# IndaPlus22/bwidman-raytracer

Hardware: AMD Instinct MI355X
Metric: Msamples/sec (W*H*spp*bounces/t), 1920x1080 8spp 4-bounce, 07_specular_BRDF (higher is better)
Workload: dtype f32; 1 GPU; 07_specular_BRDF 1920x1080 8spp 4-bounce (BASELINE configs[2]); scene=07, width=1920, height=1080, spp=8, max_bounces=4, parallelism=pixel-rows/1

## Files before the change

bwidman-raytracer_amd/bwrt/abi.py:

```python
from __future__ import annotations

import ctypes as C
import os
import re

PKG_DIR = os.path.dirname(os.path.dirname(os.path.abspath(__file__)))
REPO_DIR = os.path.dirname(PKG_DIR)
LIB_PATH = os.path.join(PKG_DIR, "lib", "libbwrt.so")
HEADER_PATH = os.path.join(REPO_DIR, "include", "rt_abi.h")


class Vec3(C.Structure):
    _fields_ = [("x", C.c_float), ("y", C.c_float), ("z", C.c_float)]

    def tolist(self):
        return [self.x, self.y, self.z]


class Material(C.Structure):
    _fields_ = [("albedo", Vec3), ("emittance", C.c_float), ("roughness", C.c_float),
                ("refractive_index", C.c_float)]


class Sphere(C.Structure):
    _fields_ = [("position", Vec3), ("radius", C.c_float), ("mat", Material)]


class Plane(C.Structure):
    _fields_ = [("origin", Vec3), ("directions", Vec3 * 2), ("mat", Material)]


class Triangle(C.Structure):
    _fields_ = [("vertices", Vec3 * 3), ("mat", Material)]


class Quad(C.Structure):
    _fields_ = [("vertices", Vec3 * 4), ("mat", Material)]


class Camera(C.Structure):
    _fields_ = [("position", Vec3), ("angle", C.c_float * 2), ("fov", C.c_float)]


class SceneStruct(C.Structure):
    _fields_ = [("camera", Camera),
                ("spheres", C.POINTER(Sphere)), ("sphere_count", C.c_int),
                ("planes", C.POINTER(Plane)), ("plane_count", C.c_int),
                ("triangles", C.POINTER(Triangle)), ("triangle_count", C.c_int),
                ("quads", C.POINTER(Quad)), ("quad_count", C.c_int)]


class RenderParams(C.Structure):
    _fields_ = [("width", C.c_int), ("height", C.c_int), ("samples", C.c_int),
                ("max_bounces", C.c_int), ("first_frame", C.c_uint),
                ("row_offset", C.c_int), ("row_stride", C.c_int)]


class DenoiseParams(C.Structure):
    _fields_ = [("iterations", C.c_int), ("sigma_color", C.c_float), ("sigma_normal", C.c_float),
                ("sigma_plane", C.c_float)]


class DenoiseVarParams(C.Structure):
    _fields_ = [("iterations", C.c_int), ("sigma_lum", C.c_float), ("sigma_normal", C.c_float),
                ("sigma_plane", C.c_float), ("min_batches", C.c_int)]


class TemporalParams(C.Structure):
    _fields_ = [("max_history", C.c_float), ("normal_cos_min", C.c_float), ("plane_tol", C.c_float)]


RT_OK = 0
RT_ERR_INVALID_ARGUMENT = -1
RT_ERR_NO_DEVICE = -2
RT_ERR_NO_SCENE = -5
RT_ERR_UNSUPPORTED = -6
RT_DENOISE_MAX_ITERATIONS = 6
RT_MAX_BOUNCES = 32
RT_DEFAULT_MAX_BOUNCES = 5
RT_PRECISION_EXACT = 0
RT_PRECISION_REFERENCE_FAST = 1

_lib = None


def _proto(lib):
    P = C.POINTER
    vp = C.c_void_p
    sigs = {
        "rt_version": (C.c_char_p, []),
        "rt_material_default": (Material, []),
        "rt_device_count": (C.c_int, []),
        "rt_create": (C.c_int, [C.c_int, P(vp)]),
        "rt_destroy": (None, [vp]),
        "rt_cpu_threads": (C.c_int, []),
        "rt_create_cpu": (C.c_int, [C.c_int, P(vp)]),
        "rt_context_threads": (C.c_int, [vp]),
        "rt_render_cpu": (C.c_int, [vp, P(RenderParams), C.c_int, vp, vp]),
        "rt_set_scene": (C.c_int, [vp, P(SceneStruct)]),
        "rt_set_camera": (C.c_int, [vp, P(Camera)]),
        "rt_reset_accumulation": (C.c_int, [vp]),
        "rt_frame_counter": (C.c_uint, [vp]),
        "rt_set_max_bounces": (C.c_int, [vp, C.c_int]),
        "rt_set_background": (C.c_int, [vp, C.c_float, C.c_float, C.c_float]),
        "rt_set_precision": (C.c_int, [vp, C.c_int]),
        "rt_get_precision": (C.c_int, [vp]),
        "rt_set_samples_per_pixel": (C.c_int, [vp, C.c_int]),
        "rt_get_camera": (C.c_int, [vp, P(Camera)]),
        "rt_apply_controls": (C.c_int, [P(Camera), C.c_uint, C.c_float]),
        "rt_controls": (C.c_int, [vp, C.c_uint, C.c_float]),
        "rt_init_rand": (C.c_int, [vp, C.c_int, C.c_int, C.c_int, C.c_int]),
        "rt_render": (C.c_int, [vp, C.c_int, C.c_int, C.c_int, vp]),
        "rt_render_ex": (C.c_int, [vp, P(RenderParams), vp, vp]),
        "rt_render_device": (C.c_int, [vp, P(RenderParams), vp, vp]),
        "rt_synchronize": (C.c_int, [vp]),
        "rt_get_stream": (vp, [vp]),
        "rt_render_multi": (C.c_int, [P(vp), C.c_int, C.c_int, C.c_int, C.c_int, vp]),
        "rt_last_kernel_ms": (C.c_float, [vp]),
        "rt_set_kernel_timing": (C.c_int, [vp, C.c_int]),
        "rt_shard_rows": (C.c_int, [C.c_int, C.c_int, C.c_int]),
        "rt_deinterleave_rows_device": (C.c_int, [vp, vp, vp, C.c_int, C.c_int, C.c_int,
                                                  C.c_int, vp]),
        "rt_get_state": (C.c_int, [vp, vp, vp]),
        "rt_set_state": (C.c_int, [vp, vp, vp, C.c_uint]),
        "rt_render_aov": (C.c_int, [vp, P(RenderParams), vp, vp, vp, vp]),
        "rt_denoise_params_default": (DenoiseParams, []),
        "rt_denoise": (C.c_int, [vp, P(DenoiseParams), vp, vp]),
        "rt_denoise_device": (C.c_int, [vp, P(DenoiseParams), vp, vp]),
        "rt_last_denoise_ms": (C.c_float, [vp]),
        "rt_denoise_var_params_default": (DenoiseVarParams, []),
        "rt_denoise_var": (C.c_int, [vp, P(DenoiseVarParams), vp, vp, vp]),
        "rt_denoise_var_device": (C.c_int, [vp, P(DenoiseVarParams), vp, vp]),
        "rt_last_denoise_var_ms": (C.c_float, [vp]),
        "rt_temporal_params_default": (TemporalParams, []),
        "rt_temporal": (C.c_int, [vp, P(TemporalParams), P(DenoiseParams), vp, vp, vp]),
        "rt_temporal_device": (C.c_int, [vp, P(TemporalParams), P(DenoiseParams), vp, vp]),
        "rt_temporal_reset": (C.c_int, [vp]),
        "rt_last_temporal_ms": (C.c_float, [vp]),
        "rt_set_moments": (C.c_int, [vp, C.c_int]),
        "rt_get_moments": (C.c_int, [vp]),
        "rt_moments_batches": (C.c_int, [vp]),
        "rt_get_variance": (C.c_int, [vp, vp, vp]),
        "rt_error_string": (C.c_char_p, [C.c_int]),
        "rt_last_error": (C.c_char_p, [vp]),
        "rt_last_kernel_name": (C.c_char_p, [vp]),
    }
    for name, (res, args) in sigs.items():
        fn = getattr(lib, name)
        fn.restype = res
        fn.argtypes = args
    return lib


def declared_functions(header: str = HEADER_PATH):
    with open(header) as f:
        text = f.read()
    return sorted(set(re.findall(r"RT_API[^;(]*?\b(rt_\w+)\s*\(", text)))


def load(path: str | None = None):
    global _lib
    if _lib is not None and path is None:
        return _lib
    p = path or os.environ.get("BWRT_LIB", LIB_PATH)
    if not os.path.exists(p):
        raise RuntimeError(
            f"libbwrt.so not found at {p}: build it with `python -c 'import __graft_entry__ as g; g.build()'`"
            " (the HIP library is the product; nothing runs without it)")
    lib = _proto(C.CDLL(p))
    if path is None:
        _lib = lib
    return lib


KEYS = {"W": 1 << 0, "A": 1 << 1, "S": 1 << 2, "D": 1 << 3, "SPACE": 1 << 4, "LEFT_SHIFT": 1 << 5,
        "LEFT": 1 << 6, "RIGHT": 1 << 7, "UP": 1 << 8, "DOWN": 1 << 9, "ESCAPE": 1 << 10}
CONTROLS_MOVED = 1
CONTROLS_QUIT = 2


class RTError(RuntimeError):
    pass


def check(lib, status, ctx=None):
    if status != RT_OK:
        msg = lib.rt_error_string(status).decode()
        if ctx:
            last = lib.rt_last_error(ctx)
            if last:
                msg += ": " + last.decode()
        raise RTError(f"rt status {status}: {msg}")
    return status
```

bwidman-raytracer_amd/bwrt/renderer.py:

```python
from __future__ import annotations

import ctypes as C

import numpy as np

from . import abi


class Renderer:
    def __init__(self, device: int = 0, lib=None, _cpu_threads=None):
        self.lib = lib or abi.load()
        self.ctx = C.c_void_p()
        if _cpu_threads is None:
            abi.check(self.lib, self.lib.rt_create(device, C.byref(self.ctx)))
        else:
            abi.check(self.lib, self.lib.rt_create_cpu(_cpu_threads, C.byref(self.ctx)))
        self.device = device if _cpu_threads is None else -1
        self.scene = None

    @classmethod
    def cpu(cls, threads: int = 0, lib=None) -> "Renderer":
        return cls(-1, lib=lib, _cpu_threads=threads)

    @property
    def is_cpu(self) -> bool:
        return self.device < 0

    @property
    def threads(self) -> int:
        return self.lib.rt_context_threads(self.ctx)

    def close(self):
        if self.ctx:
            self.lib.rt_destroy(self.ctx)
            self.ctx = C.c_void_p()

    def __enter__(self):
        return self

    def __exit__(self, *exc):
        self.close()

    def __del__(self):
        try:
            self.close()
        except Exception:
            pass

    def _check(self, status):
        return abi.check(self.lib, status, self.ctx)

    def set_scene(self, scene):
        self.scene = scene
        self._check(self.lib.rt_set_scene(self.ctx, C.byref(scene.struct)))

    def set_camera(self, camera):
        self._check(self.lib.rt_set_camera(self.ctx, C.byref(camera)))

    def reset_accumulation(self):
        self._check(self.lib.rt_reset_accumulation(self.ctx))

    @property
    def frame_counter(self) -> int:
        return self.lib.rt_frame_counter(self.ctx)

    def set_max_bounces(self, mb: int):
        self._check(self.lib.rt_set_max_bounces(self.ctx, mb))

    def set_background(self, r: float, g: float, b: float):
        self._check(self.lib.rt_set_background(self.ctx, r, g, b))

    _PRECISIONS = {"exact": abi.RT_PRECISION_EXACT, "fast": abi.RT_PRECISION_REFERENCE_FAST}

    def set_precision(self, mode: str):
        if mode not in self._PRECISIONS:
            raise ValueError(f"precision {mode!r}: expected 'exact' or 'fast'")
        self._check(self.lib.rt_set_precision(self.ctx, self._PRECISIONS[mode]))

    @property
    def precision(self) -> str:
        return "fast" if self.lib.rt_get_precision(self.ctx) == abi.RT_PRECISION_REFERENCE_FAST else "exact"

    def set_samples_per_pixel(self, n: int):
        self._check(self.lib.rt_set_samples_per_pixel(self.ctx, n))

    def get_camera(self):
        from .abi import Camera
        cam = Camera()
        self._check(self.lib.rt_get_camera(self.ctx, C.byref(cam)))
        return cam

    def controls(self, keys, delta_time: float) -> int:
        from .abi import KEYS
        if not isinstance(keys, int):
            keys = sum(KEYS[k] for k in keys)
        flags = self.lib.rt_controls(self.ctx, keys, delta_time)
        if flags < 0:
            self._check(flags)
        return flags

    def init_rand(self, width, height, row_offset=0, row_stride=1):
        self._check(self.lib.rt_init_rand(self.ctx, width, height, row_offset, row_stride))

    @staticmethod
    def params(width, height, samples, max_bounces, first_frame=0, row_offset=0, row_stride=1):
        return abi.RenderParams(width, height, samples, max_bounces, first_frame, row_offset,
                                row_stride)

    def render_simple(self, width: int, height: int, samples: int) -> np.ndarray:
        out = np.empty((height, width, 4), dtype=np.uint8)
        self._check(self.lib.rt_render(self.ctx, width, height, samples, out.ctypes.data))
        return out

    def render(self, width, height, samples, max_bounces=abi.RT_DEFAULT_MAX_BOUNCES, first_frame=0,
               row_offset=0, row_stride=1, want_accum=False):
        rows = self.lib.rt_shard_rows(height, row_offset, row_stride)
        out = np.empty((rows, width, 4), dtype=np.uint8)
        acc = np.empty((rows, width, 3), dtype=np.float32) if want_accum else None
        p = self.params(width, height, samples, max_bounces, first_frame, row_offset, row_stride)
        self._check(self.lib.rt_render_ex(self.ctx, C.byref(p), out.ctypes.data,
                                          acc.ctypes.data if acc is not None else None))
        return (out, acc) if want_accum else out

    def render_cpu(self, width, height, samples, max_bounces=abi.RT_DEFAULT_MAX_BOUNCES, first_frame=0,
                   row_offset=0, row_stride=1, threads=0, want_accum=False):
        rows = self.lib.rt_shard_rows(height, row_offset, row_stride)
        out = np.empty((rows, width, 4), dtype=np.uint8)
        acc = np.empty((rows, width, 3), dtype=np.float32) if want_accum else None
        p = self.params(width, height, samples, max_bounces, first_frame, row_offset, row_stride)
        self._check(self.lib.rt_render_cpu(self.ctx, C.byref(p), threads, out.ctypes.data,
                                           acc.ctypes.data if acc is not None else None))
        return (out, acc) if want_accum else out

    def render_device(self, params: abi.RenderParams, rgba_ptr: int, stream_ptr: int | None = None):
        self._check(self.lib.rt_render_device(self.ctx, C.byref(params), rgba_ptr, stream_ptr))

    def synchronize(self):
        self._check(self.lib.rt_synchronize(self.ctx))

    def stream_handle(self) -> int:
        return self.lib.rt_get_stream(self.ctx) or 0

    def last_kernel_ms(self) -> float:
        return self.lib.rt_last_kernel_ms(self.ctx)

    def last_kernel_name(self) -> str:
        return self.lib.rt_last_kernel_name(self.ctx).decode()

    def set_kernel_timing(self, enable: bool):
        self._check(self.lib.rt_set_kernel_timing(self.ctx, int(bool(enable))))

    def deinterleave_device(self, gathered_ptr, image_ptr, width, height, shards, rows_per_shard,
                            stream_ptr=None):
        self._check(self.lib.rt_deinterleave_rows_device(self.ctx, gathered_ptr, image_ptr, width,
                                                         height, shards, rows_per_shard,
                                                         stream_ptr))

    def render_aov(self, width, height, row_offset=0, row_stride=1):
        rows = self.lib.rt_shard_rows(height, row_offset, row_stride)
        out = {"albedo": np.empty((rows, width, 3), np.float32), "normal": np.empty((rows, width, 3), np.float32),
               "depth": np.empty((rows, width), np.float32), "prim": np.empty((rows, width), np.int32)}
        p = self.params(width, height, 1, 0, 0, row_offset, row_stride)
        self._check(self.lib.rt_render_aov(self.ctx, C.byref(p), out["albedo"].ctypes.data,
                                           out["normal"].ctypes.data, out["depth"].ctypes.data,
                                           out["prim"].ctypes.data))
        return out

    def denoise_params(self, iterations=None, sigma_color=None, sigma_normal=None, sigma_plane=None):
        d = self.lib.rt_denoise_params_default()
        for name, v in (("iterations", iterations), ("sigma_color", sigma_color),
                        ("sigma_normal", sigma_normal), ("sigma_plane", sigma_plane)):
            if v is not None:
                setattr(d, name, v)
        return d

    def denoise(self, width, height, iterations=None, sigma_color=None, sigma_normal=None, sigma_plane=None,
                want_color=False):
        d = self.denoise_params(iterations, sigma_color, sigma_normal, sigma_plane)
        out = np.empty((height, width, 4), np.uint8)
        col = np.empty((height, width, 3), np.float32) if want_color else None
        self._check(self.lib.rt_denoise(self.ctx, C.byref(d), out.ctypes.data,
                                        col.ctypes.data if col is not None else None))
        return (out, col) if want_color else out

    def denoise_device(self, rgba_ptr: int, stream_ptr: int | None = None, iterations=None, sigma_color=None,
                       sigma_normal=None, sigma_plane=None):
        d = self.denoise_params(iterations, sigma_color, sigma_normal, sigma_plane)
        self._check(self.lib.rt_denoise_device(self.ctx, C.byref(d), rgba_ptr, stream_ptr))

    def last_denoise_ms(self) -> float:
        return self.lib.rt_last_denoise_ms(self.ctx)

    def denoise_var_params(self, iterations=None, sigma_lum=None, sigma_normal=None, sigma_plane=None,
                           min_batches=None):
        d = self.lib.rt_denoise_var_params_default()
        for name, v in (("iterations", iterations), ("sigma_lum", sigma_lum), ("sigma_normal", sigma_normal),
                        ("sigma_plane", sigma_plane), ("min_batches", min_batches)):
            if v is not None:
                setattr(d, name, v)
        return d

    def denoise_var(self, width, height, want_color=False, want_var=False, **params):
        d = self.denoise_var_params(**params)
        out = np.empty((height, width, 4), np.uint8)
        col = np.empty((height, width, 3), np.float32) if want_color else None
        var = np.empty((height, width), np.float32) if want_var else None
        self._check(self.lib.rt_denoise_var(self.ctx, C.byref(d), out.ctypes.data,
                                            col.ctypes.data if col is not None else None,
                                            var.ctypes.data if var is not None else None))
        res = (out,) + ((col,) if want_color else ()) + ((var,) if want_var else ())
        return res if len(res) > 1 else out

    def denoise_var_device(self, rgba_ptr: int, stream_ptr: int | None = None, **params):
        d = self.denoise_var_params(**params)
        self._check(self.lib.rt_denoise_var_device(self.ctx, C.byref(d), rgba_ptr, stream_ptr))

    def last_denoise_var_ms(self) -> float:
        return self.lib.rt_last_denoise_var_ms(self.ctx)

    def temporal_params(self, max_history=None, normal_cos_min=None, plane_tol=None):
        t = self.lib.rt_temporal_params_default()
        for name, v in (("max_history", max_history), ("normal_cos_min", normal_cos_min), ("plane_tol", plane_tol)):
            if v is not None:
                setattr(t, name, v)
        return t

    def _dn(self, denoise):
        return None if denoise is None else C.byref(self.denoise_params(**denoise))

    def temporal(self, width, height, max_history=None, normal_cos_min=None, plane_tol=None, denoise=None,
                 want_color=False, want_length=False):
        t = self.temporal_params(max_history, normal_cos_min, plane_tol)
        out = np.empty((height, width, 4), np.uint8)
        col = np.empty((height, width, 3), np.float32) if want_color else None
        ln = np.empty((height, width), np.float32) if want_length else None
        self._check(self.lib.rt_temporal(self.ctx, C.byref(t), self._dn(denoise), out.ctypes.data,
                                         col.ctypes.data if col is not None else None,
                                         ln.ctypes.data if ln is not None else None))
        res = (out,) + ((col,) if want_color else ()) + ((ln,) if want_length else ())
        return res if len(res) > 1 else out

    def temporal_device(self, rgba_ptr: int, stream_ptr: int | None = None, max_history=None, normal_cos_min=None,
                        plane_tol=None, denoise=None):
        t = self.temporal_params(max_history, normal_cos_min, plane_tol)
        self._check(self.lib.rt_temporal_device(self.ctx, C.byref(t), self._dn(denoise), rgba_ptr, stream_ptr))

    def temporal_reset(self):
        self._check(self.lib.rt_temporal_reset(self.ctx))

    def last_temporal_ms(self) -> float:
        return self.lib.rt_last_temporal_ms(self.ctx)

    def set_moments(self, enable: bool = True):
        self._check(self.lib.rt_set_moments(self.ctx, int(bool(enable))))

    @property
    def moments(self) -> bool:
        return bool(self.lib.rt_get_moments(self.ctx))

    @property
    def moments_batches(self) -> int:
        return self.lib.rt_moments_batches(self.ctx)

    def variance(self, rows, width, want_lum=False):
        var = np.empty((rows, width), np.float32)
        lum = np.empty((rows, width), np.float32) if want_lum else None
        self._check(self.lib.rt_get_variance(self.ctx, var.ctypes.data, lum.ctypes.data if want_lum else None))
        return (var, lum) if want_lum else var

    def get_state(self, rows, width):
        rng = np.empty((6, rows, width), dtype=np.uint32)
        acc = np.empty((rows, width, 3), dtype=np.float32)
        self._check(self.lib.rt_get_state(self.ctx, rng.ctypes.data, acc.ctypes.data))
        return rng, acc

    def set_state(self, rng, acc, frame_counter):
        rng = np.ascontiguousarray(rng, dtype=np.uint32)
        acc = np.ascontiguousarray(acc, dtype=np.float32)
        self._check(self.lib.rt_set_state(self.ctx, rng.ctypes.data, acc.ctypes.data,
                                          frame_counter))


def shard_rows(height: int, row_offset: int, row_stride: int) -> int:
    return len(range(row_offset, height, row_stride)) if row_stride > 0 else 0


def render_multi(renderers, width: int, height: int, samples: int) -> np.ndarray:
    lib = renderers[0].lib
    arr = (C.c_void_p * len(renderers))(*[r.ctx.value for r in renderers])
    out = np.empty((height, width, 4), np.uint8)
    rc = lib.rt_render_multi(arr, len(renderers), width, height, samples, out.ctypes.data)
    if rc != abi.RT_OK:
        renderers[0]._check(rc)
    return out
```

bwidman-raytracer_amd/csrc/rt_context.cpp:

```cpp
#include <sched.h>

#include <algorithm>
#include <cmath>
#include <cstdarg>
#include <cstddef>
#include <thread>

#include "rt_context.h"

static_assert(sizeof(rt_vec3) == 12, "vec3d layout (Math.cuh:35-39)");
static_assert(sizeof(rt_material) == 24, "material layout (WorldTypes.cuh:15-20)");
static_assert(sizeof(rt_sphere) == 40 && offsetof(rt_sphere, mat) == 16, "sphere layout");
static_assert(sizeof(rt_plane) == 60 && offsetof(rt_plane, mat) == 36, "plane layout");
static_assert(sizeof(rt_triangle) == 60 && offsetof(rt_triangle, mat) == 36, "triangle layout");
static_assert(sizeof(rt_quad) == 72 && offsetof(rt_quad, mat) == 48, "quad layout");
static_assert(sizeof(rt_camera) == 24, "camera layout (WorldTypes.cuh:9-13)");
static_assert(sizeof(rt_scene) == 88 && offsetof(rt_scene, spheres) == 24 &&
                  offsetof(rt_scene, sphere_count) == 32 && offsetof(rt_scene, planes) == 40 &&
                  offsetof(rt_scene, triangles) == 56 && offsetof(rt_scene, quads) == 72 &&
                  offsetof(rt_scene, quad_count) == 80,
              "scene layout (WorldTypes.cuh:44-53)");

const char* tuning_env(const char* name) {
    const char* t = std::getenv("BWRT_TUNING");
    return t && std::strcmp(t, "1") == 0 ? std::getenv(name) : nullptr;
}

int fail(rt_context* c, int code, const char* fmt, ...) {
    if (c) {
        char buf[512];
        va_list ap;
        va_start(ap, fmt);
        vsnprintf(buf, sizeof buf, fmt, ap);
        va_end(ap);
        c->err = buf;
    }
    return code;
}

int hip_fail(rt_context* c, hipError_t e, const char* what) {
    return fail(c, e == hipErrorOutOfMemory ? RT_ERR_OUT_OF_MEMORY : RT_ERR_HIP, "%s: %s", what,
                hipGetErrorString(e));
}

int quiesce(rt_context* c) {
    if (c->cpu) return RT_OK;
    HIP_TRY(c, c->render.flush());
    for (Pass* p : {&c->denoise, &c->temporal, &c->denoise_var, &c->render}) HIP_TRY(c, p->sync());
    return RT_OK;
}

int order_after_all(rt_context* c, hipStream_t s) {
    for (Pass* p : {&c->render, &c->denoise, &c->temporal, &c->denoise_var}) HIP_TRY(c, p->wait_on(s));
    return RT_OK;
}

int ensure_buf(rt_context* c, Buf& b, size_t bytes, const char* host_oom, size_t n) {
    if (b.bytes >= bytes && b.p) return RT_OK;
    if (b.p && !c->cpu) {
        int rc = quiesce(c);
        if (rc) return rc;
        HIP_TRY(c, hipStreamSynchronize(c->stream));
    }
    b.release();
    if (bytes == 0) return RT_OK;
    if (c->cpu) {
        if (!(b.p = std::calloc(bytes, 1))) return fail(c, RT_ERR_OUT_OF_MEMORY, host_oom, n);
        b.host = true;
    } else {
        HIP_TRY(c, hipMalloc(&b.p, bytes));
    }
    b.bytes = bytes;
    return RT_OK;
}

int shard_rows(int height, int row_offset, int row_stride) {
    if (height <= 0 || row_offset < 0 || row_stride <= 0 || row_offset >= height) return 0;
    return (height - row_offset + row_stride - 1) / row_stride;
}

int shard_check(rt_context* c, int width, int height, int row_offset, int row_stride) {
    if (width <= 0 || height <= 0 || row_offset < 0 || row_stride < 0 || row_offset >= height)
        return fail(c, RT_ERR_INVALID_ARGUMENT, "bad shard %dx%d offset %d stride %d", width, height,
                    row_offset, row_stride);
    if ((long long)width * height > (1ll << 31))
        return fail(c, RT_ERR_UNSUPPORTED, "image larger than 2^31 pixels");
    return RT_OK;
}

extern "C" {

const char* rt_version(void) { return "0.3.0"; }

rt_material rt_material_default(void) {
    rt_material m;
    m.albedo = {0.0f, 0.0f, 0.0f};
    m.emittance = 0.0f;
    m.roughness = 1.0f;
    m.refractive_index = 1.05f;
    return m;
}

int rt_device_count(void) {
    int n = 0;
    if (hipGetDeviceCount(&n) != hipSuccess) return 0;
    return n;
}

int rt_create(int device, rt_context** out) {
    if (!out) return RT_ERR_INVALID_ARGUMENT;
    *out = nullptr;
    int n = 0;
    if (hipGetDeviceCount(&n) != hipSuccess || n <= 0) return RT_ERR_NO_DEVICE;
    if (device < 0 || device >= n) return RT_ERR_INVALID_ARGUMENT;
    rt_context* c = new rt_context();
    c->device = device;
    int prio_lo = 0, prio_hi = 0;
    const char* sp = tuning_env("BWRT_STREAM_PRIO");
    const bool high = !(sp && std::atoi(sp) == 0) && hipSetDevice(device) == hipSuccess &&
                      hipDeviceGetStreamPriorityRange(&prio_lo, &prio_hi) == hipSuccess;
    if (hipSetDevice(device) != hipSuccess ||
        (high ? hipStreamCreateWithPriority(&c->stream, hipStreamNonBlocking, prio_hi)
              : hipStreamCreateWithFlags(&c->stream, hipStreamNonBlocking)) != hipSuccess ||
        c->render.create(true) != hipSuccess || c->aux.create(false) != hipSuccess ||
        c->denoise.create(true) != hipSuccess) {
        rt_destroy(c);
        return RT_ERR_HIP;
    }
    c->render.home = c->stream;
    hipDeviceProp_t prop;
    if (hipGetDeviceProperties(&prop, device) == hipSuccess && prop.multiProcessorCount > 0)
        c->num_cus = prop.multiProcessorCount;
    if (const char* gm = tuning_env("BWRT_GRID_MULT")) c->grid_mult = std::atoi(gm);
    if (const char* db = tuning_env("BWRT_DEINT_BLOCKS")) c->deint_blocks = std::max(std::atoi(db), 0);
    if (const char* kk = tuning_env("BWRT_KERNEL")) c->simple = std::strcmp(kk, "simple") == 0;
    if (const char* bk = tuning_env("BWRT_BLOCK")) c->block = std::atoi(bk);
    if (const char* tw = tuning_env("BWRT_TILE")) {
        const int t = std::atoi(tw);
        if (t >= 0 && t <= 64 && (t & (t - 1)) == 0) c->tile_w = t;
    }
    if (const char* g = tuning_env("BWRT_TILE_SQ")) c->tile_sq = std::atoi(g) != 0;
    if (const char* g = tuning_env("BWRT_GREC")) c->grec = std::atoi(g) ? 1 : 0;
    if (const char* g = tuning_env("BWRT_LEAF_BATCH")) c->leaf_batch = std::min(std::max(std::atoi(g), 1), 64);
    if (const char* g = tuning_env("BWRT_REFILL")) c->refill = std::min(std::max(std::atoi(g), 1), 64);
    if (const char* g = tuning_env("BWRT_SPREAD")) c->spread = std::atoi(g) ? 1 : 0;
    if (const char* g = tuning_env("BWRT_ORDER")) c->order_feedback = std::atoi(g) != 0;
    if (const char* g = tuning_env("BWRT_ORDER_PERIOD")) c->order_period = std::max(std::atoi(g), 1);
    if (const char* g = tuning_env("BWRT_DENOISE_KERNEL"))
        c->dn_kernel = std::strcmp(g, "tiled") == 0 ? 1 : std::strcmp(g, "direct") == 0 ? 0 : -1;
    if (const char* g = tuning_env("BWRT_PRECISION"))
        c->precision = std::strcmp(g, "fast") == 0 ? RT_PRECISION_REFERENCE_FAST : RT_PRECISION_EXACT;
    *out = c;
    return RT_OK;
}

int rt_create_cpu(int threads, rt_context** out) {
    if (!out) return RT_ERR_INVALID_ARGUMENT;
    *out = nullptr;
    if (threads < 0) return RT_ERR_INVALID_ARGUMENT;
    if (!rt_cpu_supported()) return RT_ERR_UNSUPPORTED;
    rt_context* c = new rt_context();
    c->cpu = true;
    c->render.host = c->denoise.host = c->temporal.host = c->denoise_var.host = true;
    c->device = -1;
    c->threads = threads > 0 ? threads : rt_cpu_threads();
    *out = c;
    return RT_OK;
}

int rt_cpu_threads(void) {
    int n = 0;
    cpu_set_t set;
    if (sched_getaffinity(0, sizeof set, &set) == 0) n = CPU_COUNT(&set);
    if (n <= 0) n = (int)std::thread::hardware_concurrency();
    if (n <= 0) n = 1;
    if (FILE* f = std::fopen("/sys/fs/cgroup/cpu.max", "r")) {
        char quota[32] = {0};
        long period = 0;
        if (std::fscanf(f, "%31s %ld", quota, &period) == 2 && std::strcmp(quota, "max") != 0 && period > 0) {
            const long q = std::atol(quota);
            const int share = (int)((q + period - 1) / period);
            if (share > 0 && share < n) n = share;
        }
        std::fclose(f);
    }
    return n;
}

void rt_destroy(rt_context* c) {
    if (!c) return;
    if (!c->cpu) {
        (void)hipSetDevice(c->device);
        if (c->stream) (void)hipStreamSynchronize(c->stream);
        c->render.pending = false;
        for (Pass* p : {&c->render, &c->aux, &c->denoise, &c->temporal, &c->denoise_var}) {
            (void)p->sync();
            p->destroy();
        }
        if (c->host_rgba) (void)hipHostFree(c->host_rgba);
        if (c->stream) (void)hipStreamDestroy(c->stream);
    }
    delete c;
}

int rt_set_scene(rt_context* c, const rt_scene* s) {
    const HostFpEnv fp;
    if (!c || !s) return fail(c, RT_ERR_INVALID_ARGUMENT, "null argument");
    if (s->sphere_count < 0 || s->plane_count < 0 || s->triangle_count < 0 || s->quad_count < 0)
        return fail(c, RT_ERR_INVALID_ARGUMENT, "negative primitive count");
    if ((s->sphere_count && !s->spheres) || (s->plane_count && !s->planes) ||
        (s->triangle_count && !s->triangles) || (s->quad_count && !s->quads))
        return fail(c, RT_ERR_INVALID_ARGUMENT, "null primitive array with non-zero count");
    if (!c->cpu) HIP_TRY(c, hipSetDevice(c->device));
    rt_scene_options opt;
    for (const char* name : rt_scene_option_names)
        if (const char* v = tuning_env(name)) rt_scene_option_set(opt, name, v);
    rt_compiled_scene cs;
    std::string err;
    if (const int rc = rt_compile_scene(*s, opt, cs, err)) return fail(c, rc, "%s", err.c_str());
    const size_t bytes = cs.data.size() * sizeof(float);
    int rc = quiesce(c);
    if (!rc) rc = ensure_buf(c, c->scene_buf, bytes, "host scene of %zu bytes", bytes);
    if (rc) {
        if (!c->scene_buf.p) c->has_scene = false;
        return rc;
    }
    if (c->cpu) {
        std::memcpy(c->scene_buf.p, cs.data.data(), bytes);
    } else {
        HIP_TRY(c, hipMemcpyAsync(c->scene_buf.p, cs.data.data(), bytes, hipMemcpyHostToDevice, c->stream));
        HIP_TRY(c, hipStreamSynchronize(c->stream));
    }
    std::vector<float>().swap(cs.data);
    c->scene = std::move(cs);
    c->camera = s->camera;
    c->has_scene = true;
    c->frame = 1;
    c->order_stale = true;
    c->new_view();
    c->tp_has_hist = c->tp_has_pending = false;
    return RT_OK;
}

int rt_set_camera(rt_context* c, const rt_camera* cam) {
    if (!c || !cam) return fail(c, RT_ERR_INVALID_ARGUMENT, "null argument");
    c->camera = *cam;
    c->frame = 1;
    c->order_stale = true;
    c->new_view();
    return RT_OK;
}

int rt_set_background(rt_context* c, float r, float g, float b) {
    if (!c) return RT_ERR_INVALID_ARGUMENT;
    c->background[0] = r;
    c->background[1] = g;
    c->background[2] = b;
    return RT_OK;
}

int rt_set_precision(rt_context* c, int precision) {
    if (!c) return RT_ERR_INVALID_ARGUMENT;
    if (precision != RT_PRECISION_EXACT && precision != RT_PRECISION_REFERENCE_FAST)
        return fail(c, RT_ERR_INVALID_ARGUMENT, "rt_set_precision: unknown precision %d", precision);
    if (c->cpu && precision != RT_PRECISION_EXACT)
        return fail(c, RT_ERR_UNSUPPORTED,
                    "rt_set_precision: RT_PRECISION_REFERENCE_FAST is not supported on a CPU context "
                    "(the CPU fallback is bit-identical to the exact kernels)");
    c->precision = precision;
    return RT_OK;
}

int rt_get_precision(const rt_context* c) { return c ? c->precision : RT_PRECISION_EXACT; }

int rt_get_camera(const rt_context* c, rt_camera* cam) {
    if (!c || !cam) return RT_ERR_INVALID_ARGUMENT;
    *cam = c->camera;
    return RT_OK;
}

int rt_apply_controls(rt_camera* cam, unsigned keys, float dt) {
    if (!cam) return RT_ERR_INVALID_ARGUMENT;
    const HostFpEnv fp;
    struct V3 {
        float x, y, z;
    };
    const float move = 5 * dt;
    const float rot = 2 * dt;
    const float cy = cosf(cam->angle[0]), sy = sinf(cam->angle[0]);
    const float cx = cosf(cam->angle[1]), sx = sinf(cam->angle[1]);
    const float L[3][3] = {{cy, 0, sy}, {0, 1, 0}, {-sy, 0, cy}};
    const float U[3][3] = {{1, 0, 0}, {0, cx, -sx}, {0, sx, cx}};
    float M[3][3];
    for (int i = 0; i < 3; i++)
        for (int j = 0; j < 3; j++) M[i][j] = L[i][0] * U[0][j] + L[i][1] * U[1][j] + L[i][2] * U[2][j];
    auto mul = [&](float x, float y, float z) {
        return V3{M[0][0] * x + M[0][1] * y + M[0][2] * z, M[1][0] * x + M[1][1] * y + M[1][2] * z,
                  M[2][0] * x + M[2][1] * y + M[2][2] * z};
    };
    const V3 front = mul(0, 0, -1), right = mul(1, 0, 0);
    rt_vec3& p = cam->position;
    int flags = 0;
    auto add = [&](float k, V3 v, float sign) {
        const V3 kv{k * v.x, k * v.y, k * v.z};
        if (sign > 0) {
            p.x = p.x + kv.x;
            p.y = p.y + kv.y;
            p.z = p.z + kv.z;
        } else {
            p.x = p.x - kv.x;
            p.y = p.y - kv.y;
            p.z = p.z - kv.z;
        }
        flags |= RT_CONTROLS_MOVED;
    };
    if (keys & RT_KEY_W) add(move, front, +1);
    if (keys & RT_KEY_A) add(move, right, -1);
    if (keys & RT_KEY_S) add(move, front, -1);
    if (keys & RT_KEY_D) add(move, right, +1);
    if (keys & RT_KEY_SPACE) {
        p.y += move;
        flags |= RT_CONTROLS_MOVED;
    }
    if (keys & RT_KEY_LEFT_SHIFT) {
        p.y -= move;
        flags |= RT_CONTROLS_MOVED;
    }
    if (keys & RT_KEY_LEFT) {
        cam->angle[0] += rot;
        flags |= RT_CONTROLS_MOVED;
    }
    if (keys & RT_KEY_RIGHT) {
        cam->angle[0] -= rot;
        flags |= RT_CONTROLS_MOVED;
    }
    if (keys & RT_KEY_UP) {
        cam->angle[1] += rot;
        flags |= RT_CONTROLS_MOVED;
    }
    if (keys & RT_KEY_DOWN) {
        cam->angle[1] -= rot;
        flags |= RT_CONTROLS_MOVED;
    }
    if (keys & RT_KEY_ESCAPE) flags |= RT_CONTROLS_QUIT;
    return flags;
}

int rt_controls(rt_context* c, unsigned keys, float dt) {
    if (!c) return RT_ERR_INVALID_ARGUMENT;
    const int flags = rt_apply_controls(&c->camera, keys, dt);
    if (flags > 0 && (flags & RT_CONTROLS_MOVED)) {
        c->frame = 1;
        c->order_stale = true;
        c->new_view();
    }
    return flags;
}

int rt_reset_accumulation(rt_context* c) {
    if (!c) return RT_ERR_INVALID_ARGUMENT;
    c->frame = 1;
    return RT_OK;
}

unsigned rt_frame_counter(const rt_context* c) { return c ? c->frame : 0u; }

int rt_set_max_bounces(rt_context* c, int mb) {
    if (!c) return RT_ERR_INVALID_ARGUMENT;
    if (mb < 0) return fail(c, RT_ERR_INVALID_ARGUMENT, "max_bounces < 0");
    if (mb > RT_MAX_BOUNCES) return fail(c, RT_ERR_UNSUPPORTED, "max_bounces > %d", RT_MAX_BOUNCES);
    c->max_bounces = mb;
    return RT_OK;
}

int rt_set_samples_per_pixel(rt_context* c, int n) {
    if (!c) return RT_ERR_INVALID_ARGUMENT;
    if (n < 1) return fail(c, RT_ERR_INVALID_ARGUMENT, "samples per pixel < 1");
    if (n > RT_MAX_SAMPLES_PER_PIXEL)
        return fail(c, RT_ERR_UNSUPPORTED, "samples per pixel > %d", RT_MAX_SAMPLES_PER_PIXEL);
    c->spp_inner = n;
    return RT_OK;
}

int rt_set_kernel_timing(rt_context* c, int enable) {
    if (!c) return RT_ERR_INVALID_ARGUMENT;
    c->ktiming = enable != 0;
    if (!c->ktiming) c->render.timed = false;
    return RT_OK;
}

int rt_shard_rows(int height, int row_offset, int row_stride) {
    return shard_rows(height, row_offset, row_stride == 0 ? 1 : row_stride);
}

int rt_init_rand(rt_context* c, int width, int height, int row_offset, int row_stride) {
    if (!c) return RT_ERR_INVALID_ARGUMENT;
    if (row_stride == 0) row_stride = 1;
    if (const int rc = shard_check(c, width, height, row_offset, row_stride)) return rc;
    const int rows = shard_rows(height, row_offset, row_stride);
    const size_t npix = (size_t)rows * width;
    c->new_view();
    c->mom_drop();
    if (width != c->tp_w || height != c->tp_h) c->tp_has_hist = c->tp_has_pending = false;
    if (!c->cpu) HIP_TRY(c, hipSetDevice(c->device));
    int rc = quiesce(c);
    const char* oom = "host state for %zu pixels";
    if (!rc) rc = ensure_buf(c, c->rng, npix * 6 * sizeof(unsigned), oom, npix);
    if (!rc) rc = ensure_buf(c, c->accum, npix * 3 * sizeof(float), oom, npix);
    if (!rc && c->cpu) rc = ensure_buf(c, c->rgba, npix * 4, oom, npix);
    if (rc) return rc;
    if (c->cpu) {
        std::memset(c->rng.p, 0, npix * 6 * sizeof(unsigned));
        std::memset(c->accum.p, 0, npix * 3 * sizeof(float));
        std::memset(c->rgba.p, 0, npix * 4);
        rt_cpu_init_rand(c->rng.as<unsigned>(), width, rows, row_offset, row_stride);
    } else {
        HIP_TRY(c, hipMemsetAsync(c->accum.p, 0, npix * 3 * sizeof(float), c->stream));
        HIP_TRY(c, rt_launch_init_rand(c->rng.as<unsigned>(), width, rows, row_offset, row_stride, c->stream));
        HIP_TRY(c, hipStreamSynchronize(c->stream));
    }
    c->width = width;
    c->height = height;
    c->row_offset = row_offset;
    c->row_stride = row_stride;
    c->rows = rows;
    c->frame = 1;
    c->order_stale = true;
    return RT_OK;
}

int rt_synchronize(rt_context* c) {
    if (!c) return RT_ERR_INVALID_ARGUMENT;
    if (c->cpu) return RT_OK;
    HIP_TRY(c, hipSetDevice(c->device));
    HIP_TRY(c, c->render.flush());
    HIP_TRY(c, hipStreamSynchronize(c->stream));
    for (Pass* p : {&c->render, &c->aux, &c->denoise, &c->temporal, &c->denoise_var}) HIP_TRY(c, p->sync());
    return RT_OK;
}

void* rt_get_stream(rt_context* c) { return c && !c->cpu ? (void*)c->stream : nullptr; }

float rt_last_kernel_ms(rt_context* c) { return c ? c->render.elapsed_ms() : -1.0f; }

int rt_get_state(rt_context* c, uint32_t* rng, float* accum) {
    if (!c) return RT_ERR_INVALID_ARGUMENT;
    const size_t npix = (size_t)c->rows * c->width;
    if (!c->rng.p) return fail(c, RT_ERR_INVALID_ARGUMENT, "no shard state (render or rt_init_rand first)");
    if (c->cpu) {
        if (rng) std::memcpy(rng, c->rng.p, npix * 6 * sizeof(unsigned));
        if (accum) planes_to_rgb(c->accum.as<float>(), npix, accum);
        return RT_OK;
    }
    HIP_TRY(c, hipSetDevice(c->device));
    HIP_TRY(c, hipStreamSynchronize(c->stream));
    const int qrc = quiesce(c);
    if (qrc) return qrc;
    if (rng) HIP_TRY(c, hipMemcpy(rng, c->rng.p, npix * 6 * sizeof(unsigned), hipMemcpyDeviceToHost));
    if (accum) {
        std::vector<float> planes(npix * 3);
        HIP_TRY(c, hipMemcpy(planes.data(), c->accum.p, npix * 3 * sizeof(float), hipMemcpyDeviceToHost));
        planes_to_rgb(planes.data(), npix, accum);
    }
    return RT_OK;
}

int rt_set_state(rt_context* c, const uint32_t* rng, const float* accum, unsigned frame_counter) {
    if (!c) return RT_ERR_INVALID_ARGUMENT;
    if (!c->rng.p) return fail(c, RT_ERR_INVALID_ARGUMENT, "no shard state (rt_init_rand first)");
    if (frame_counter == 0) return fail(c, RT_ERR_INVALID_ARGUMENT, "frame_counter must be >= 1");
    const size_t npix = (size_t)c->rows * c->width;
    if (c->cpu) {
        if (rng) std::memcpy(c->rng.p, rng, npix * 6 * sizeof(unsigned));
        if (accum) rgb_to_planes(accum, npix, c->accum.as<float>());
        c->frame = frame_counter;
        c->mom_drop();
        return RT_OK;
    }
    HIP_TRY(c, hipSetDevice(c->device));
    const int rc = quiesce(c);
    if (rc) return rc;
    std::vector<float> planes;
    if (rng)
        HIP_TRY(c, hipMemcpyAsync(c->rng.p, rng, npix * 6 * sizeof(unsigned), hipMemcpyHostToDevice, c->stream));
    if (accum) {
        planes.resize(npix * 3);
        rgb_to_planes(accum, npix, planes.data());
        HIP_TRY(c, hipMemcpyAsync(c->accum.p, planes.data(), npix * 3 * sizeof(float), hipMemcpyHostToDevice,
                                  c->stream));
    }
    HIP_TRY(c, hipStreamSynchronize(c->stream));
    c->frame = frame_counter;
    c->mom_drop();
    return RT_OK;
}

const char* rt_error_string(int status) {
    switch (status) {
        case RT_OK: return "ok";
        case RT_ERR_INVALID_ARGUMENT: return "invalid argument";
        case RT_ERR_NO_DEVICE: return "no HIP device";
        case RT_ERR_HIP: return "HIP runtime error";
        case RT_ERR_OUT_OF_MEMORY: return "out of device memory";
        case RT_ERR_NO_SCENE: return "no scene";
        case RT_ERR_UNSUPPORTED: return "unsupported";
        default: return "unknown status";
    }
}

const char* rt_last_error(const rt_context* c) { return c ? c->err.c_str() : ""; }

const char* rt_last_kernel_name(const rt_context* c) { return c ? c->kernel_name.c_str() : ""; }

int rt_context_threads(const rt_context* c) { return c && c->cpu ? c->threads : 0; }

}
```

bwidman-raytracer_amd/csrc/rt_context.h:

```cpp
#pragma once

#include <hip/hip_runtime.h>

#include <chrono>
#include <cstdint>
#include <cstdio>
#include <cstdlib>
#include <cstring>
#include <string>
#include <vector>
#include <xmmintrin.h>

#include "../../include/rt_abi.h"
#include "rt_layout.h"
#include "rt_scene.h"

size_t rt_render_rec_floats(const rt_kparams& K);
bool rt_render_wants_global_records(const rt_kparams& K, int num_cus);
hipError_t rt_launch_render(const rt_kparams& K, int num_cus, int grid_mult, bool simple, int block_req,
                            hipStream_t stream, int pair_req);
hipError_t rt_launch_init_rand(unsigned* rng, int width, int rows, int row_offset, int row_stride,
                               hipStream_t stream);
namespace rt_fast {
bool rt_render_wants_global_records(const rt_kparams& K, int num_cus);
hipError_t rt_launch_render(const rt_kparams& K, int num_cus, int grid_mult, bool simple, int block_req,
                            hipStream_t stream, int pair_req);
}
extern thread_local long rt_order_groups_last;
extern thread_local char rt_launched_kernel[96];
hipError_t rt_launch_deinterleave(const unsigned* gathered, unsigned* image, int width, int height,
                                  int shards, int rows_per_shard, int max_blocks, hipStream_t stream);
int rt_cpu_render(const rt_kparams& K, int threads);
void rt_cpu_init_rand(unsigned* rng, int width, int rows, int row_offset, int row_stride);
bool rt_cpu_supported();
void rt_cpu_aov(const rt_kparams& K, int threads, float4* ga, float4* gb, float4* alb);
void rt_cpu_denoise_level(const rt_dn_level& L, int threads);
void rt_cpu_temporal(const rt_tp_args& T, int threads);
void rt_cpu_moments(const rt_mom_args& A, int threads);
void rt_cpu_denoise_var(const rt_dv_args& A, int stage, int threads);
hipError_t rt_launch_aov(const rt_kparams& K, float4* ga, float4* gb, float4* alb, hipStream_t stream);
hipError_t rt_launch_aov_bvh(const rt_kparams& K, float4* ga, float4* gb, float4* alb, hipStream_t stream);
hipError_t rt_launch_denoise_level(const rt_dn_level& L, bool tiled, hipStream_t stream);
hipError_t rt_launch_temporal(const rt_tp_args& T, hipStream_t stream);
hipError_t rt_launch_moments(const rt_mom_args& A, hipStream_t stream);
hipError_t rt_launch_denoise_var(const rt_dv_args& A, int stage, bool tiled, hipStream_t stream);

struct Buf {
    void* p = nullptr;
    size_t bytes = 0;
    bool host = false;
    Buf() = default;
    Buf(const Buf&) = delete;
    Buf& operator=(const Buf&) = delete;
    ~Buf() { release(); }
    void release() {
        if (p) host ? std::free(p) : (void)hipFree(p);
        p = nullptr;
        bytes = 0;
    }
    template <class T>
    T* as() const {
        return static_cast<T*>(p);
    }
};

struct Pass {
    hipEvent_t ev0 = nullptr, ev1 = nullptr;
    hipStream_t stream = nullptr;
    hipStream_t home = nullptr;
    bool host = false;
    bool recorded = false;
    bool pending = false;
    bool timed = false;
    bool marked = false;
    float cpu_ms = -1.0f;
    std::chrono::steady_clock::time_point t0;

    hipError_t create(bool timing) {
        hipError_t e = hipSuccess;
        if (timing && !ev0) e = hipEventCreate(&ev0);
        if (e == hipSuccess && !ev1) e = timing ? hipEventCreate(&ev1) : hipEventCreateWithFlags(&ev1, hipEventDisableTiming);
        return e;
    }
    hipError_t begin(hipStream_t s, bool with_marker) {
        marked = with_marker;
        if (host) t0 = std::chrono::steady_clock::now();
        return !host && with_marker ? hipEventRecord(ev0, s) : hipSuccess;
    }
    hipError_t end(hipStream_t s) {
        stream = s;
        if (host) {
            cpu_ms = std::chrono::duration<float, std::milli>(std::chrono::steady_clock::now() - t0).count();
        } else if (home && s == home && !marked) {
            pending = true;
        } else {
            pending = false;
            const hipError_t e = hipEventRecord(ev1, s);
            if (e != hipSuccess) return e;
            recorded = true;
        }
        timed = marked;
        return hipSuccess;
    }
    hipError_t flush() {
        if (!pending) return hipSuccess;
        pending = false;
        const hipError_t e = hipEventRecord(ev1, home);
        if (e == hipSuccess) recorded = true;
        return e;
    }
    hipError_t wait_on(hipStream_t s) {
        if (!(recorded || pending) || stream == s) return hipSuccess;
        const hipError_t e = flush();
        return e != hipSuccess ? e : hipStreamWaitEvent(s, ev1, 0);
    }
    hipError_t sync() { return recorded ? hipEventSynchronize(ev1) : hipSuccess; }
    float elapsed_ms() {
        if (host) return cpu_ms;
        float ms = -1.0f;
        if (!timed || hipEventSynchronize(ev1) != hipSuccess || hipEventElapsedTime(&ms, ev0, ev1) != hipSuccess)
            return -1.0f;
        return ms;
    }
    void destroy() {
        if (ev0) (void)hipEventDestroy(ev0);
        if (ev1) (void)hipEventDestroy(ev1);
        ev0 = ev1 = nullptr;
    }
};

struct rt_context {
    int device = 0;
    int num_cus = 256;
    bool simple = false;
    int grid_mult = 0;
    hipStream_t stream = nullptr;
    Pass render, aux, denoise, temporal, denoise_var;
    bool cpu = false;
    int threads = 1;
    bool ktiming = true;
    std::string err;

    bool has_scene = false;
    rt_camera camera{};
    float background[3] = {0.0f, 0.0f, 0.0f};
    rt_compiled_scene scene;
    Buf scene_buf;

    int width = 0, height = 0, row_offset = 0, row_stride = 1, rows = 0;
    Buf rng, accum, rgba;
    Buf rec;
    Buf gcost, gorder;
    long order_n = 0;
    int order_period = 16;
    bool order_stale = true;
    unsigned long long launches = 0;
    bool order_feedback = true;
    int grec = -1;
    void* host_rgba = nullptr;
    size_t host_rgba_bytes = 0;
    int block = 0;
    int tile_w = -1;
    int tile_sq = 0;
    int leaf_batch = -1;
    int refill = -1;
    int spread = -1;
    int deint_blocks = 0;
    std::string kernel_name;
    int precision = RT_PRECISION_EXACT;
    unsigned frame = 1;
    int max_bounces = RT_DEFAULT_MAX_BOUNCES;
    int spp_inner = 1;

    Buf guide_a, guide_b, dn_col[2], dn_rgba;
    Buf dn_rs;
    Buf aov_a, aov_b, aov_alb;
    bool guides_valid = false;
    int dn_kernel = -1;

    struct TpSet {
        Buf col, ga, gb;
        float cam_pos[3] = {}, rot[9] = {}, screen_z = 0.0f;
    };
    unsigned long long view = 1;
    TpSet tp[2];
    int tp_hist = 0;
    bool tp_has_hist = false, tp_has_pending = false;
    unsigned long long tp_pending_view = 0;
    int tp_w = 0, tp_h = 0;

    bool mom_on = false, mom_live = false;
    unsigned mom_batches = 0, mom_next = 0;
    Buf mom_prev, mom_m;
    void mom_drop() {
        mom_live = false;
        mom_batches = 0;
    }

    void new_view() {
        guides_valid = false;
        view++;
    }
};

struct HostFpEnv {
    unsigned saved;
    HostFpEnv() : saved(_mm_getcsr()) {
        _mm_setcsr((saved & ~(_MM_ROUND_MASK | _MM_FLUSH_ZERO_MASK | 0x0040u)) | _MM_ROUND_NEAREST);
    }
    ~HostFpEnv() { _mm_setcsr(saved); }
};

const char* tuning_env(const char* name);

int fail(rt_context* c, int code, const char* fmt, ...);
int hip_fail(rt_context* c, hipError_t e, const char* what);

#define HIP_TRY(ctx, expr)                                  \
    do {                                                    \
        hipError_t _e = (expr);                             \
        if (_e != hipSuccess) return hip_fail(ctx, _e, #expr); \
    } while (0)

int quiesce(rt_context* c);
int order_after_all(rt_context* c, hipStream_t s);
int ensure_buf(rt_context* c, Buf& b, size_t bytes, const char* host_oom = "host buffer (%zu)", size_t n = 0);
int shard_rows(int height, int row_offset, int row_stride);
int shard_check(rt_context* c, int width, int height, int row_offset, int row_stride);
void fill_view(rt_context* c, int width, int height, int row_offset, int stride, int rows, rt_kparams& K);

inline void planes_to_rgb(const float* planes, size_t npix, float* out) {
    for (size_t i = 0; i < npix; i++)
        for (int ch = 0; ch < 3; ch++) out[3 * i + ch] = planes[ch * npix + i];
}
inline void rgb_to_planes(const float* rgb, size_t npix, float* planes) {
    for (size_t i = 0; i < npix; i++)
        for (int ch = 0; ch < 3; ch++) planes[ch * npix + i] = rgb[3 * i + ch];
}
inline void xyz_of(const float4* v, size_t npix, float* out) {
    for (size_t i = 0; i < npix; i++) {
        out[3 * i + 0] = v[i].x;
        out[3 * i + 1] = v[i].y;
        out[3 * i + 2] = v[i].z;
    }
}
inline void w_of(const float4* v, size_t npix, void* out) {
    for (size_t i = 0; i < npix; i++) std::memcpy(static_cast<char*>(out) + 4 * i, &v[i].w, 4);
}
```

bwidman-raytracer_amd/csrc/rt_kernels.hip:

```cpp
#include <hip/hip_runtime.h>

#include <cstdio>
#include <type_traits>

#include "rt_diag.h"
#include "rt_layout.h"
#include "rt_path.h"

#ifdef RT_FAST
#define RT_MODE_BEGIN namespace rt_fast {
#define RT_MODE_END }
#define RT_MODE_TAG ",fast"
#else
#define RT_MODE_BEGIN
#define RT_MODE_END
#define RT_MODE_TAG ""
#endif
#if !defined(RT_TU_BVH) && !defined(RT_FAST)
#define RT_TU_SHARED
#endif

namespace {
__device__ __forceinline__ void closest_hit_bvh(const rt_kparams& K, f3 o, f3 d, float& best_t, int& best_id) {
    if (!bvh_safe(K, o, d)) {
        closest_hit_brute(K, o, d, best_t, best_id);
        return;
    }
    const float a = dot(d, d);
    const float a4 = 4.0f * a;
    const float a2 = 2.0f * a;
    best_t = INFINITY;
    best_id = -1;
    int best_key = -1;
    planes_first(K, o, d, best_t, best_id, best_key);
    const SlabRay sr = slab_ray(o, d);
    const float* nodes = K.bvh_nodes + (size_t)ray_octant(K, d) * K.bvh_order_stride;
    int node = 0;
    while (true) {
        int leaf = -1;
        while (true) {
            bool stalled = false;
            if (node >= 0) {
                RT_BRANCH_COUNT(K, 5);
                const float4 lo = *reinterpret_cast<const float4*>(nodes + 8 * node);
                const float4 hi = *reinterpret_cast<const float4*>(nodes + 8 * node + 4);
                const bool hit = slab_enter(lo.x, lo.y, lo.z, hi.x, hi.y, hi.z, sr, best_t);
                const int miss = __float_as_int(lo.w);
                const int lf = __float_as_int(hi.w);
                if (!hit) {
                    node = miss;
                } else if (lf < 0) {
                    node = node + 1;
                } else if (leaf < 0) {
                    leaf = lf;
                    node = miss;
                } else {
                    stalled = true;
                }
            }
            if (__all(leaf >= 0 || node < 0 || stalled)) break;
        }
        if (!__any(leaf >= 0)) break;
        if (leaf >= 0) {
            const int first = leaf & 0xffffff, count = leaf >> 24;
            for (int k = 0; k < count; k++) {
                RT_BRANCH_COUNT(K, 6);
                leaf_test(K, K.bvh_leafrec + (size_t)RT_LEAF_FLOATS * (first + k), o, d, a2, a4, best_t, best_id,
                          best_key);
            }
        }
    }
}

template <bool BVH, bool QUADS = true>
__device__ __forceinline__ void closest_hit(const rt_kparams& K, f3 o, f3 d, float& best_t, int& best_id) {
    if (BVH)
        closest_hit_bvh(K, o, d, best_t, best_id);
    else
        closest_hit_brute<QUADS>(K, o, d, best_t, best_id);
}

#ifndef RT_NT_PIXEL
#define RT_NT_PIXEL 3
#endif
#ifndef RT_NT_GREC
#define RT_NT_GREC 0
#endif
template <typename T>
__device__ __forceinline__ T px_ld(const T* a) {
    if (RT_NT_PIXEL & 1) return __builtin_nontemporal_load(a);
    return *a;
}
template <typename T>
__device__ __forceinline__ void px_st(T* a, T v) {
    if (RT_NT_PIXEL & 2) __builtin_nontemporal_store(v, a);
    else *a = v;
}
struct PixelState {
    long w;
    long p;
    bool valid;
    Xorwow rs;
    float ax, ay, az;
    f3 d0;
    int passes_left;
    unsigned frame;
};

__device__ __forceinline__ void load_pixel(const rt_kparams& K, long npix, long p, PixelState& s) {
    s.p = p;
    s.valid = p < npix;
    s.passes_left = 0;
    s.frame = K.first_frame;
    if (!s.valid) return;
    const int j = (int)(p / K.width);
    const int x = (int)(p - (long)j * K.width);
    const int y = K.row_offset + j * K.row_stride;
    s.rs.d = px_ld(&K.rng[0 * npix + p]);
    s.rs.v0 = px_ld(&K.rng[1 * npix + p]);
    s.rs.v1 = px_ld(&K.rng[2 * npix + p]);
    s.rs.v2 = px_ld(&K.rng[3 * npix + p]);
    s.rs.v3 = px_ld(&K.rng[4 * npix + p]);
    s.rs.v4 = px_ld(&K.rng[5 * npix + p]);
    s.ax = s.ay = s.az = 0.0f;
    if (K.first_frame != 1u) {
        s.ax = px_ld(&K.accum[0 * npix + p]);
        s.ay = px_ld(&K.accum[1 * npix + p]);
        s.az = px_ld(&K.accum[2 * npix + p]);
    }
    s.d0 = primary_dir(K, x, y);
    s.passes_left = K.samples;
}

__host__ __device__ inline long launch_items(const rt_kparams& K) {
    if (K.tile_w <= 0) return (long)K.rows * K.width;
    const int tw = K.tile_w, th = 64 / K.tile_w;
    long tiles_x = (K.width + tw - 1) / tw, tiles_y = (K.rows + th - 1) / th;
    if (K.tile_sq) {
        tiles_x += tiles_x & 1;
        tiles_y += tiles_y & 1;
    }
    return tiles_x * tiles_y * 64;
}

__device__ __forceinline__ long items_of(const rt_kparams& K, long npix) {
    return K.tile_w <= 0 ? npix : launch_items(K);
}

__device__ __forceinline__ long item_to_pixel(const rt_kparams& K, long npix, long w) {
    if (K.tile_w <= 0) return w < npix ? w : npix;
    const int tw = K.tile_w, th = 64 / K.tile_w;
    const long tiles_x = (K.width + tw - 1) / tw;
    const long wave = w >> 6;
    const int l = (int)(w & 63);
    long tx, ty;
    if (K.tile_sq) {
        const long sx = (tiles_x + 1) >> 1, sw = wave >> 2;
        tx = (sw % sx) * 2 + (wave & 1);
        ty = (sw / sx) * 2 + ((wave >> 1) & 1);
    } else {
        tx = wave % tiles_x;
        ty = wave / tiles_x;
    }
    const long x = tx * tw + (l % tw);
    const long j = ty * th + (l / tw);
    if (x >= K.width || j >= K.rows) return npix;
    return j * K.width + x;
}

__device__ __forceinline__ void load_item(const rt_kparams& K, long npix, long nitems, long w, PixelState& s) {
    load_pixel(K, npix, w < nitems ? item_to_pixel(K, npix, w) : npix, s);
    s.w = w;
}

__device__ __forceinline__ void store_pixel(const rt_kparams& K, long npix, const PixelState& s) {
    const long p = s.p;
    px_st(&K.rng[0 * npix + p], s.rs.d);
    px_st(&K.rng[1 * npix + p], s.rs.v0);
    px_st(&K.rng[2 * npix + p], s.rs.v1);
    px_st(&K.rng[3 * npix + p], s.rs.v2);
    px_st(&K.rng[4 * npix + p], s.rs.v3);
    px_st(&K.rng[5 * npix + p], s.rs.v4);
    px_st(&K.accum[0 * npix + p], s.ax);
    px_st(&K.accum[1 * npix + p], s.ay);
    px_st(&K.accum[2 * npix + p], s.az);
#if RT_NT_PIXEL & 2
    if (K.rgba) px_st(&K.rgba[p], tone_map(s.ax, s.ay, s.az, s.frame - 1u));
#else
    if (K.rgba) K.rgba[p] = tone_map(s.ax, s.ay, s.az, s.frame - 1u);
#endif
}

typedef __attribute__((address_space(3))) float lds_float;

__device__ __forceinline__ int lanes_below(unsigned long long mask) {
    return (int)__builtin_amdgcn_mbcnt_hi((unsigned)(mask >> 32),
                                          __builtin_amdgcn_mbcnt_lo((unsigned)mask, 0u));
}

__device__ __forceinline__ int prim_key(const rt_kparams& K, int id) {
    const int e_pln = K.n_sph, e_tri = e_pln + K.n_pln, e_quad = e_tri + K.n_tri;
    return id < 0 ? -1
                  : id < e_pln ? RT_KEY(0, id)
                               : id < e_tri ? RT_KEY(1, id - e_pln)
                                            : id < e_quad ? RT_KEY(2, id - e_tri) : RT_KEY(3, id - e_quad);
}

}

#ifndef RT_WAVES_PER_EU
#define RT_WAVES_PER_EU 1
#endif
#ifndef RT_GREC_WAVES
#define RT_GREC_WAVES 7
#endif
#ifndef RT_GREC_LDS_LEVELS
#define RT_GREC_LDS_LEVELS 2
#endif
#ifndef RT_SPEC_PRIO
#define RT_SPEC_PRIO 3
#endif
#ifndef RT_PAIR_WAVES
#define RT_PAIR_WAVES 7
#endif

RT_MODE_BEGIN
template <int BLOCK, bool HIT_LDS, bool BVH>
__global__ void __launch_bounds__(BLOCK) __attribute__((amdgpu_waves_per_eu(RT_WAVES_PER_EU)))
rt_render_kernel(rt_kparams K) {
    extern __shared__ float smem[];
    const int tid = threadIdx.x;
    const int n_prim = K.n_sph + K.n_pln + K.n_tri + K.n_quad;
    const float* hit_tab = K.hit;
    float* rec_base = smem;
    if (HIT_LDS) {
        for (int i = tid; i < n_prim * RT_HIT_FLOATS; i += BLOCK) smem[i] = K.hit[i];
        __syncthreads();
        hit_tab = smem;
        rec_base = smem + ((n_prim * RT_HIT_FLOATS + 3) & ~3);
    }
    int* rec_code = reinterpret_cast<int*>(rec_base) + tid;
    float* rec_k = rec_base + (K.max_bounces + 1) * BLOCK + tid;
    float* rec_c = rec_base + 2 * (K.max_bounces + 1) * BLOCK + tid;

    const long npix = (long)K.rows * K.width;
    const long T = (long)gridDim.x * BLOCK;
    const long nitems = items_of(K, npix);
    PixelState px;
    load_item(K, npix, nitems, (long)blockIdx.x * BLOCK + tid, px);

    f3 o = mk(0.0f, 0.0f, 0.0f), d = mk(0.0f, 0.0f, 1.0f);
    int depth = -1;
    const f3 cam = mk(K.cam_pos[0], K.cam_pos[1], K.cam_pos[2]);
    f3 dcam = d;
    int inner = 1;

    while (true) {
        if (depth < 0 && px.passes_left > 0) {
            f3 jit = random_direction(px.rs, px.d0);
            d = normalize3(add(px.d0, scale(K.jitter, jit)));
            o = cam;
            depth = 0;
            dcam = d;
            inner = K.spp_inner;
        }
        const bool active = depth >= 0;
        if (__ballot(active) == 0ull) break;
        if (active) {
            float t;
            int id;
            closest_hit<BVH>(K, o, d, t, id);

            bool finished = true;
            if (id >= 0) {
                const float* h = hit_tab + RT_HIT_FLOATS * id;
                const float4 h0 = *reinterpret_cast<const float4*>(h);
                const float4 h1 = *reinterpret_cast<const float4*>(h + 4);
                const float4 h2 = *reinterpret_cast<const float4*>(h + 8);
                const f3 P = add(o, scale(t, d));
                f3 n = mk(h0.x, h0.y, h0.z);
                if (h0.w != 0.0f) n = normalize3(sub(P, n));
                const f3 albedo = mk(h1.x, h1.y, h1.z);
                const float rough = h2.x, ior2m1 = h2.y, rough2 = h2.z;

                f3 scatter;
                int code = id;
                float kspec = 0.0f;
                const float choice = rand_range(px.rs, 1.0f);
                if (choice < RT_SPECULAR_CHANCE) {
                    const float e1 = rand_range(px.rs, 1.0f);
                    const float e2 = rand_range(px.rs, 1.0f);
                    const float theta = atan_nn(rt_div(rough * rt_sqrt(e1), rt_sqrt(1.0f - e1)));
                    const float phi = 2.0f * RT_PI * e2;
                    float st, ct, sp, cp;
                    rt_sincos(theta, st, ct);
                    rt_sincos(phi, sp, cp);
                    const f3 mloc = mk(st * cp, st * sp, ct);
                    f3 some = mk(1.0f, 0.0f, 0.0f);
                    if (fabsf(dot(n, some)) < 1.0f - RT_NEAR_ZERO) some = mk(0.0f, 1.0f, 0.0f);
                    const f3 t1 = cross(n, some);
                    const f3 t2 = cross(n, t1);
                    const f3 m = mk(dot(mk(t1.x, t2.x, n.x), mloc), dot(mk(t1.y, t2.y, n.y), mloc),
                                    dot(mk(t1.z, t2.z, n.z), mloc));
                    scatter = sub(d, scale(2.0f * dot(d, m), m));
                    const f3 inc = scale(-1.0f, d);
                    const float fr = fresnel(inc, m, ior2m1);
                    const float sw = specular_weight(inc, scatter, n, m, rough2);
                    kspec = rt_div_spec_chance(sw * fr);
                    code = ~id;
                } else {
                    scatter = random_direction(px.rs, n);
                }
                (void)albedo;
                rec_code[depth * BLOCK] = code;
                rec_k[depth * BLOCK] = kspec;
                rec_c[depth * BLOCK] = dot(scatter, n);
                depth++;
                o = P;
                d = scatter;
                finished = depth > K.max_bounces;
            }
            if (finished) {
                float lx = K.bg[0], ly = K.bg[1], lz = K.bg[2];
                for (int l = depth - 1; l >= 0; --l)
                    fold_level(rec_code[l * BLOCK], rec_k[l * BLOCK], rec_c[l * BLOCK], hit_tab, lx, ly, lz);
                if (inner > 1) {
                    inner--;
                    o = cam;
                    d = dcam;
                    depth = 0;
                    continue;
                }
                if (K.spp_inner != 1) {
                    const float k = rt_div(1.0f, (float)K.spp_inner);
                    lx = k * lx;
                    ly = k * ly;
                    lz = k * lz;
                }
                if (px.frame == 1u) {
                    px.ax = 0.0f;
                    px.ay = 0.0f;
                    px.az = 0.0f;
                }
                px.ax = px.ax + lx;
                px.ay = px.ay + ly;
                px.az = px.az + lz;
                px.frame++;
                px.passes_left--;
                depth = -1;
                if (px.passes_left == 0) {
                    store_pixel(K, npix, px);
                    load_item(K, npix, nitems, px.w + T, px);
                }
            }
        }
    }
}
RT_MODE_END

#ifdef RT_TU_SHARED
__device__ __forceinline__ int order_bucket(unsigned cost) {
    const int k = (int)(__float_as_uint((float)cost + 1.0f) >> 19) - (127 << 4);
    return 511 - min(k, 511);
}

__global__ void __launch_bounds__(1024) rt_order_groups_kernel(const unsigned* __restrict__ cost,
                                                               int* __restrict__ order, int n) {
    __shared__ unsigned hist[512];
    __shared__ unsigned wsum[8];
    const int tid = threadIdx.x;
    if (tid < 512) hist[tid] = 0;
    __syncthreads();
    for (int i = tid; i < n; i += 1024) atomicAdd(&hist[order_bucket(cost[i])], 1u);
    __syncthreads();
    unsigned v = 0, incl = 0;
    if (tid < 512) {
        v = hist[tid];
        incl = v;
        for (int m = 1; m < 64; m <<= 1) {
            const unsigned u = __shfl_up(incl, m);
            if ((tid & 63) >= m) incl += u;
        }
        if ((tid & 63) == 63) wsum[tid >> 6] = incl;
    }
    __syncthreads();
    if (tid < 512) {
        unsigned base = 0;
        for (int w = 0; w < (tid >> 6); w++) base += wsum[w];
        hist[tid] = base + incl - v;
    }
    __syncthreads();
    for (int i = tid; i < n; i += 1024) order[atomicAdd(&hist[order_bucket(cost[i])], 1u)] = i;
}

__global__ void __launch_bounds__(256) rt_init_rand_kernel(unsigned* rng, int width, int rows,
                                                           int row_offset, int row_stride) {
    const long npix = (long)rows * width;
    const long p = (long)blockIdx.x * blockDim.x + threadIdx.x;
    if (p >= npix) return;
    const int j = (int)(p / width);
    const int x = (int)(p - (long)j * width);
    const int y = row_offset + j * row_stride;
    const Xorwow s = xorwow_seed(pixel_seed(x, y, width));
    rng[0 * npix + p] = s.d;
    rng[1 * npix + p] = s.v0;
    rng[2 * npix + p] = s.v1;
    rng[3 * npix + p] = s.v2;
    rng[4 * npix + p] = s.v3;
    rng[5 * npix + p] = s.v4;
}

template <int VEC>
__global__ void __launch_bounds__(256) rt_deinterleave_kernel(const unsigned* __restrict__ gathered,
                                                              unsigned* __restrict__ image, int width,
                                                              int height, int shards, int rows_per_shard) {
    typedef typename std::conditional<VEC == 4, uint4, unsigned>::type word;
    const int wv = width / VEC;
    const long n = (long)height * wv;
    for (long q = (long)blockIdx.x * blockDim.x + threadIdx.x; q < n; q += (long)gridDim.x * blockDim.x) {
        const int y = (int)(q / wv);
        const int x = (int)(q - (long)y * wv);
        const int r = y % shards;
        const int j = y / shards;
        reinterpret_cast<word*>(image)[q] = reinterpret_cast<const word*>(gathered)[((long)r * rows_per_shard + j) * wv + x];
    }
}
#endif

enum { T_NONE = 0, T_REGEN = 1, T_DIFF = 2, T_SPEC = 3 };

RT_MODE_BEGIN
template <int BLOCK, bool HIT_LDS, bool GREC, bool ORDER = false, bool QUADS = true>
__global__ void __launch_bounds__(BLOCK) __attribute__((amdgpu_waves_per_eu(GREC ? RT_GREC_WAVES : RT_WAVES_PER_EU)))
rt_render_sorted_kernel(rt_kparams K) {
    extern __shared__ float smem[];
    const int tid = threadIdx.x;
    const int lane = tid & 63;
    const int n_prim = K.n_sph + K.n_pln + K.n_tri + K.n_quad;
    const float* hit_tab = K.hit;
    float* rec_base = smem;
    if (HIT_LDS) {
        for (int i = tid; i < n_prim * RT_HIT_FLOATS; i += BLOCK) smem[i] = K.hit[i];
        hit_tab = smem;
        rec_base = smem + ((n_prim * RT_HIT_FLOATS + 3) & ~3);
    }
    const int levels = K.max_bounces;
    const int LL = GREC ? (levels < RT_GREC_LDS_LEVELS ? levels : RT_GREC_LDS_LEVELS) : levels;
    lds_float* rec = (lds_float*)(rec_base + tid);
    const int GL = levels - LL;
    float* grec = GREC ? K.rec + (long)blockIdx.x * 3 * GL * BLOCK + tid : rec_base;
    float* slots = rec_base + 3 * LL * BLOCK;
    int* counters = reinterpret_cast<int*>(slots + 13 * BLOCK);
    const long npix = (long)K.rows * K.width;
    const long nitems = items_of(K, npix);
    if (tid < 4) counters[tid] = 0;
    diag_group_start(K);
    __syncthreads();
#define SLOT(f, i) slots[(f) * BLOCK + (i)]
#define RES(f, i) slots[((f) < 4 ? (f) : (f) + 3) * BLOCK + (i)]

    const long group = ORDER && K.group_order ? (long)K.group_order[blockIdx.x] : (long)blockIdx.x;
    if (ORDER && tid == 0) K.group_cost[group] = (unsigned)__builtin_amdgcn_s_memrealtime();
    PixelState px;
    load_item(K, npix, nitems, tid < BLOCK ? group * BLOCK + tid : nitems, px);
    int mode = px.passes_left > 0 ? T_REGEN : T_NONE;

    f3 o = mk(0.0f, 0.0f, 0.0f), d = mk(0.0f, 0.0f, 1.0f);
    f3 hn = o;
    int hid = 0, depth = 0;
    bool has_ray = false;
    int parity = 0;
    const f3 cam = mk(K.cam_pos[0], K.cam_pos[1], K.cam_pos[2]);

    auto finish_path = [&](int slot) {
        auto fold_path = [&](auto x, float& lx, float& ly, float& lz) {
            if (depth > K.max_bounces)
                fold_level(__float_as_int(x(SLOT(6, slot))), x(SLOT(4, slot)), x(SLOT(5, slot)), hit_tab, lx, ly, lz);
            const int nrec = depth > K.max_bounces ? K.max_bounces : depth;
            if (GREC)
                for (int l = nrec - 1; l >= LL; --l) {
                    const float* r = grec + 3 * (l - LL) * BLOCK;
#if RT_NT_GREC
                    fold_level(__float_as_int(x(__builtin_nontemporal_load(&r[0]))), x(__builtin_nontemporal_load(&r[BLOCK])),
                               x(__builtin_nontemporal_load(&r[2 * BLOCK])), hit_tab, lx, ly, lz);
#else
                    fold_level(__float_as_int(x(r[0])), x(r[BLOCK]), x(r[2 * BLOCK]), hit_tab, lx, ly, lz);
#endif
                }
            for (int l = (nrec < LL ? nrec : LL) - 1; l >= 0; --l) {
                const lds_float* r = rec + 3 * l * BLOCK;
                fold_level(__float_as_int(x(r[0])), x(r[BLOCK]), x(r[2 * BLOCK]), hit_tab, lx, ly, lz);
            }
        };
        float lx = K.bg[0], ly = K.bg[1], lz = K.bg[2];
        fold_path(DiagIdent(), lx, ly, lz);
        RT_TWICE_FOLD(K, fold_path);
        if (px.frame == 1u) {
            px.ax = 0.0f;
            px.ay = 0.0f;
            px.az = 0.0f;
        }
        px.ax = px.ax + lx;
        px.ay = px.ay + ly;
        px.az = px.az + lz;
        px.frame++;
        px.passes_left--;
        mode = px.passes_left > 0 ? T_REGEN : T_NONE;
    };
    bool ended = false;

    SortedStamps dg;
    while (true) {
        const int task = mode;
        dg.stamp(7);
        __syncthreads();
        dg.stamp(0);

        int* cnt = counters + 2 * parity;
        const bool front = task == T_REGEN || task == T_DIFF;
        const unsigned long long mf = __ballot(front);
        const unsigned long long mbk = __ballot(task == T_SPEC);
        int base_f = 0, base_b = 0;
        if (lane == 0) {
            if (mf) base_f = atomicAdd(&cnt[0], __popcll(mf));
            if (mbk) base_b = atomicAdd(&cnt[1], __popcll(mbk));
        }
        base_f = __builtin_amdgcn_readfirstlane(base_f);
        base_b = __builtin_amdgcn_readfirstlane(base_b);
        int slot = -1;
        if (front) slot = base_f + lanes_below(mf);
        if (task == T_SPEC) slot = BLOCK - 1 - (base_b + lanes_below(mbk));
        if (slot >= 0) {
            const f3 nrm = task == T_REGEN ? px.d0 : hn;
            SLOT(0, slot) = nrm.x;
            SLOT(1, slot) = nrm.y;
            SLOT(2, slot) = nrm.z;
            SLOT(3, slot) = d.x;
            SLOT(4, slot) = d.y;
            SLOT(5, slot) = d.z;
            SLOT(6, slot) = __int_as_float(task == T_REGEN ? -1 : hid);
            SLOT(7, slot) = __uint_as_float(px.rs.d);
            SLOT(8, slot) = __uint_as_float(px.rs.v0);
            SLOT(9, slot) = __uint_as_float(px.rs.v1);
            SLOT(10, slot) = __uint_as_float(px.rs.v2);
            SLOT(11, slot) = __uint_as_float(px.rs.v3);
            SLOT(12, slot) = __uint_as_float(px.rs.v4);
        }
        dg.stamp(1);
        __syncthreads();
        dg.stamp(2);
        const int nf = cnt[0], nb = cnt[1];
        if (nf + nb == 0) break;

        {
            const bool do_front = tid < nf;
            const bool do_spec = tid >= BLOCK - nb;
#if RT_SPEC_PRIO
            const int wave_first = (int)__builtin_amdgcn_readfirstlane((unsigned)(tid & ~63));
            const bool spec_wave = wave_first + 63 >= BLOCK - nb;
            if (spec_wave) __builtin_amdgcn_s_setprio(RT_SPEC_PRIO);
#endif
            if (do_front || do_spec) {
                Xorwow rs;
                rs.d = __float_as_uint(SLOT(7, tid));
                rs.v0 = __float_as_uint(SLOT(8, tid));
                rs.v1 = __float_as_uint(SLOT(9, tid));
                rs.v2 = __float_as_uint(SLOT(10, tid));
                rs.v3 = __float_as_uint(SLOT(11, tid));
                rs.v4 = __float_as_uint(SLOT(12, tid));
                const f3 nrm = mk(SLOT(0, tid), SLOT(1, tid), SLOT(2, tid));
                const int code = __float_as_int(SLOT(6, tid));
                f3 r;
                if (do_front) {
                    RT_TWICE_RANDDIR(rs, nrm);
                    r = random_direction(rs, nrm, dg.rej_ptr());
                    if (code < 0) r = normalize3(add(nrm, scale(K.jitter, r)));
                } else {
                    const f3 dd = mk(SLOT(3, tid), SLOT(4, tid), SLOT(5, tid));
                    const float4 h2 = *reinterpret_cast<const float4*>(hit_tab + RT_HIT_FLOATS * code + 8);
                    float kspec;
                    RT_TWICE_SPEC(rs, dd, nrm, h2);
                    r = specular_scatter(rs, dd, nrm, h2.x, h2.z, h2.y, kspec);
                    RES(3, tid) = kspec;
                }
                RES(0, tid) = r.x;
                RES(1, tid) = r.y;
                RES(2, tid) = r.z;
                RES(4, tid) = __uint_as_float(rs.d);
                RES(5, tid) = __uint_as_float(rs.v0);
                RES(6, tid) = __uint_as_float(rs.v1);
                RES(7, tid) = __uint_as_float(rs.v2);
                RES(8, tid) = __uint_as_float(rs.v3);
                RES(9, tid) = __uint_as_float(rs.v4);
            }
            dg.exec(do_front, do_spec);
        }
        dg.stamp(3);
#if RT_SPEC_PRIO
        __builtin_amdgcn_s_setprio(0);
#endif
        __syncthreads();
        dg.stamp(4);
        if (tid == 0) {
            counters[2 * (parity ^ 1)] = 0;
            counters[2 * (parity ^ 1) + 1] = 0;
        }
        parity ^= 1;

        if (slot >= 0) {
            d = mk(RES(0, slot), RES(1, slot), RES(2, slot));
            px.rs.d = __float_as_uint(RES(4, slot));
            px.rs.v0 = __float_as_uint(RES(5, slot));
            px.rs.v1 = __float_as_uint(RES(6, slot));
            px.rs.v2 = __float_as_uint(RES(7, slot));
            px.rs.v3 = __float_as_uint(RES(8, slot));
            px.rs.v4 = __float_as_uint(RES(9, slot));
            mode = T_NONE;
            if (task == T_REGEN) {
                o = cam;
                depth = 0;
                has_ray = true;
            } else {
                const int code = task == T_SPEC ? ~hid : hid;
                const float kspec = task == T_SPEC ? RES(3, slot) : 0.0f;
                const float cosang = dot(d, hn);
                if (depth < K.max_bounces) {
                    if (!GREC || depth < LL) {
                        lds_float* r = rec + 3 * depth * BLOCK;
                        r[0] = __int_as_float(code);
                        r[BLOCK] = kspec;
                        r[2 * BLOCK] = cosang;
                    } else {
                        float* r = grec + 3 * (depth - LL) * BLOCK;
                        r[0] = __int_as_float(code);
                        r[BLOCK] = kspec;
                        r[2 * BLOCK] = cosang;
                    }
                    has_ray = true;
                } else {
                    SLOT(4, slot) = kspec;
                    SLOT(5, slot) = cosang;
                    SLOT(6, slot) = __int_as_float(code);
                    ended = true;
                }
                depth++;
            }
        }

        dg.stamp(5);
        dg.rays(has_ray);
        float t = INFINITY;
        int id = -1;
        if (has_ray) {
            RT_TWICE_HIT(QUADS, K, o, d);
            closest_hit_brute<QUADS>(K, o, d, t, id);
        }
        if (has_ray) {
            has_ray = false;
            if (id >= 0) {
                const float4 h0 = *reinterpret_cast<const float4*>(hit_tab + RT_HIT_FLOATS * id);
                o = add(o, scale(t, d));
                hn = mk(h0.x, h0.y, h0.z);
                if (h0.w != 0.0f) hn = normalize3(sub(o, hn));
                hid = id;
                mode = rand_range(px.rs, 1.0f) < RT_SPECULAR_CHANCE ? T_SPEC : T_DIFF;
            } else {
                ended = true;
            }
        }
        if (ended) {
            ended = false;
            finish_path(slot);
        }
        dg.stamp(6);
    }
    if (px.valid && px.passes_left == 0 && px.frame != K.first_frame) store_pixel(K, npix, px);
    if (ORDER && tid == 0) {
        const volatile __attribute__((address_space(4))) rt_kparams* kp =
            (const volatile __attribute__((address_space(4))) rt_kparams*)__builtin_amdgcn_kernarg_segment_ptr();
        int* const ord = kp->group_order;
        unsigned* const cost = kp->group_cost;
        const long g = ord ? (long)__builtin_nontemporal_load(&ord[blockIdx.x]) : (long)blockIdx.x;
        cost[g] = (unsigned)__builtin_amdgcn_s_memrealtime() - cost[g];
    }
    diag_group_end<true>(K);
    dg.flush(K);
#undef SLOT
#undef RES
}

#define RT_PAIR_FIELDS 25
template <bool HIT_LDS, bool ORDER, bool QUADS>
__global__ void __launch_bounds__(128) __attribute__((amdgpu_waves_per_eu(RT_PAIR_WAVES)))
rt_render_pair_kernel(rt_kparams K) {
    extern __shared__ float smem[];
    const int tid = threadIdx.x;
    const int j = tid & 63;
    const bool owner = tid < 64;
    const int n_prim = K.n_sph + K.n_pln + K.n_tri + K.n_quad;
    const float* hit_tab = K.hit;
    float* rec_base = smem;
    if (HIT_LDS) {
        for (int i = tid; i < n_prim * RT_HIT_FLOATS; i += 128) smem[i] = K.hit[i];
        hit_tab = smem;
        rec_base = smem + ((n_prim * RT_HIT_FLOATS + 3) & ~3);
    }
    const int levels = K.max_bounces;
    lds_float* rec = (lds_float*)(rec_base + j);
    lds_float* xb = (lds_float*)(rec_base + 3 * levels * 64) + j;
#define XF(f) xb[(f) * 64]
    int* live_flag = reinterpret_cast<int*>(rec_base + 3 * levels * 64 + RT_PAIR_FIELDS * 64);
    const long npix = (long)K.rows * K.width;
    const long nitems = items_of(K, npix);
    diag_group_start(K);
    const long group = ORDER && K.group_order ? (long)K.group_order[blockIdx.x] : (long)blockIdx.x;
    if (ORDER && tid == 0) K.group_cost[group] = (unsigned)__builtin_amdgcn_s_memrealtime();
    PixelState px;
    load_item(K, npix, nitems, owner ? group * 64 + j : nitems, px);
    int mode = px.passes_left > 0 ? T_REGEN : T_NONE;
    f3 o = mk(0.0f, 0.0f, 0.0f), d = mk(0.0f, 0.0f, 1.0f), hn = o;
    int hid = 0, depth = 0;
    bool hit = false;
    int hflag = 0;
    const f3 cam = mk(K.cam_pos[0], K.cam_pos[1], K.cam_pos[2]);
    if (owner) XF(22) = __int_as_float(0);
    __syncthreads();

    bool fold = false;
    while (true) {
        bool has_ray = false, ended = false;
        int dcode = 0;
        float dk = 0.0f, dc = 0.0f;
        if (owner) {
            if (fold) {
                fold = false;
                float lx = K.bg[0], ly = K.bg[1], lz = K.bg[2];
                if (depth > K.max_bounces)
                    fold_level(__float_as_int(XF(6)), XF(7), XF(8), hit_tab, lx, ly, lz);
                const int nrec = depth > K.max_bounces ? K.max_bounces : depth;
                for (int l = nrec - 1; l >= 0; --l) {
                    const lds_float* q = rec + 3 * l * 64;
                    fold_level(__float_as_int(q[0]), q[64], q[128], hit_tab, lx, ly, lz);
                }
                if (px.frame == 1u) {
                    px.ax = 0.0f;
                    px.ay = 0.0f;
                    px.az = 0.0f;
                }
                px.ax = px.ax + lx;
                px.ay = px.ay + ly;
                px.az = px.az + lz;
                px.frame++;
                px.passes_left--;
            }
            if (hit) {
                hit = false;
                o = mk(XF(0), XF(1), XF(2));
                hn = mk(XF(9), XF(10), XF(11));
            }
            if (mode == T_REGEN || mode == T_DIFF) {
                f3 r = random_direction(px.rs, mode == T_REGEN ? px.d0 : hn);
                if (mode == T_REGEN) {
                    d = normalize3(add(px.d0, scale(K.jitter, r)));
                    o = cam;
                    depth = 0;
                    has_ray = true;
                } else {
                    const float cosang = dot(r, hn);
                    if (depth < K.max_bounces) {
                        lds_float* q = rec + 3 * depth * 64;
                        q[0] = __int_as_float(hid);
                        q[64] = 0.0f;
                        q[128] = cosang;
                        d = r;
                        has_ray = true;
                    } else {
                        dcode = hid;
                        dc = cosang;
                        ended = true;
                    }
                    depth++;
                }
            }
            if (mode != T_SPEC) {
                const int flag = has_ray ? (bvh_safe(K, o, d) ? 1 : 2) : 0;
                XF(0) = o.x;
                XF(1) = o.y;
                XF(2) = o.z;
                XF(3) = d.x;
                XF(4) = d.y;
                XF(5) = d.z;
                XF(6) = __int_as_float(flag);
            }
        } else {
            const int sf = __float_as_int(XF(22));
            if (sf & 1) {
                Xorwow rs;
                rs.d = __float_as_uint(XF(16));
                rs.v0 = __float_as_uint(XF(17));
                rs.v1 = __float_as_uint(XF(18));
                rs.v2 = __float_as_uint(XF(19));
                rs.v3 = __float_as_uint(XF(20));
                rs.v4 = __float_as_uint(XF(21));
                const f3 nrm = mk(XF(9), XF(10), XF(11));
                const f3 dd = mk(XF(3), XF(4), XF(5));
                const float4 h2 = *reinterpret_cast<const float4*>(hit_tab + RT_HIT_FLOATS * hid + 8);
                float kspec;
                const f3 r = specular_scatter(rs, dd, nrm, h2.x, h2.z, h2.y, kspec);
                XF(12) = r.x;
                XF(13) = r.y;
                XF(14) = r.z;
                XF(15) = kspec;
                XF(16) = __uint_as_float(rs.d);
                XF(17) = __uint_as_float(rs.v0);
                XF(18) = __uint_as_float(rs.v1);
                XF(19) = __uint_as_float(rs.v2);
                XF(20) = __uint_as_float(rs.v3);
                XF(21) = __uint_as_float(rs.v4);
                int flag = 0;
                if (sf & 2) {
                    XF(3) = r.x;
                    XF(4) = r.y;
                    XF(5) = r.z;
                    flag = bvh_safe(K, mk(XF(0), XF(1), XF(2)), r) ? 1 : 2;
                }
                XF(6) = __int_as_float(flag);
            }
        }
        __syncthreads();

        float t = INFINITY;
        int id = -1;
        int rflag = 0;
        if (owner) {
            if (mode == T_SPEC) {
                const f3 r = mk(XF(12), XF(13), XF(14));
                const float kspec = XF(15);
                px.rs.d = __float_as_uint(XF(16));
                px.rs.v0 = __float_as_uint(XF(17));
                px.rs.v1 = __float_as_uint(XF(18));
                px.rs.v2 = __float_as_uint(XF(19));
                px.rs.v3 = __float_as_uint(XF(20));
                px.rs.v4 = __float_as_uint(XF(21));
                const float cosang = dot(r, hn);
                if (depth < K.max_bounces) {
                    lds_float* q = rec + 3 * depth * 64;
                    q[0] = __int_as_float(~hid);
                    q[64] = kspec;
                    q[128] = cosang;
                    d = r;
                    has_ray = true;
                } else {
                    dcode = ~hid;
                    dk = kspec;
                    dc = cosang;
                    ended = true;
                }
                depth++;
            }
            if (has_ray) {
                rflag = __float_as_int(XF(6));
                if (rflag == 1)
                    closest_hit_brute<QUADS, 2>(K, o, d, t, id, 1);
                else
                    closest_hit_brute<QUADS>(K, o, d, t, id);
                XF(23) = t;
                XF(24) = __int_as_float(id);
            }
        } else {
            hflag = __float_as_int(XF(6));
            if (hflag == 1) {
                closest_hit_brute<QUADS, 2>(K, mk(XF(0), XF(1), XF(2)), mk(XF(3), XF(4), XF(5)), t, id, 0);
                XF(7) = t;
                XF(8) = __int_as_float(id);
            }
        }
        __syncthreads();

        int live = 0;
        if (owner) {
            if (rflag == 1) {
                const float t2 = XF(7);
                const int id2 = __float_as_int(XF(8));
                if (id2 >= 0 && (t2 < t || (t2 == t && prim_key(K, id2) > prim_key(K, id)))) {
                    t = t2;
                    id = id2;
                }
            }
            mode = T_NONE;
            if (has_ray) {
                if (id >= 0) {
                    hid = id;
                    hit = true;
                    mode = rand_range(px.rs, 1.0f) < RT_SPECULAR_CHANCE ? T_SPEC : T_DIFF;
                } else {
                    ended = true;
                }
            }
            if (ended) {
                fold = true;
                XF(6) = __int_as_float(dcode);
                XF(7) = dk;
                XF(8) = dc;
                mode = px.passes_left > 1 ? T_REGEN : T_NONE;
            }
            int sf = 0;
            if (mode == T_SPEC) {
                XF(16) = __uint_as_float(px.rs.d);
                XF(17) = __uint_as_float(px.rs.v0);
                XF(18) = __uint_as_float(px.rs.v1);
                XF(19) = __uint_as_float(px.rs.v2);
                XF(20) = __uint_as_float(px.rs.v3);
                XF(21) = __uint_as_float(px.rs.v4);
                sf = depth < K.max_bounces ? 3 : 1;
            }
            XF(22) = __int_as_float(sf);
            live = __ballot(mode != T_NONE || fold) != 0ull;
            if (j == 0) *live_flag = live;
        } else if (hflag != 0) {
            float tt = XF(23);
            int ii = __float_as_int(XF(24));
            if (hflag == 1 && id >= 0 && (t < tt || (t == tt && prim_key(K, id) > prim_key(K, ii)))) {
                tt = t;
                ii = id;
            }
            if (ii >= 0) {
                const float4 h0 = *reinterpret_cast<const float4*>(hit_tab + RT_HIT_FLOATS * ii);
                const f3 hp = add(mk(XF(0), XF(1), XF(2)), scale(tt, mk(XF(3), XF(4), XF(5))));
                f3 nn = mk(h0.x, h0.y, h0.z);
                if (h0.w != 0.0f) nn = normalize3(sub(hp, nn));
                XF(0) = hp.x;
                XF(1) = hp.y;
                XF(2) = hp.z;
                XF(9) = nn.x;
                XF(10) = nn.y;
                XF(11) = nn.z;
                hid = ii;
            }
        }
        __syncthreads();
        if (!owner) live = *live_flag;
        if (!live) break;
    }
#undef XF
    if (px.valid && px.passes_left == 0 && px.frame != K.first_frame) store_pixel(K, npix, px);
    if (ORDER && tid == 0) {
        const volatile __attribute__((address_space(4))) rt_kparams* kp =
            (const volatile __attribute__((address_space(4))) rt_kparams*)__builtin_amdgcn_kernarg_segment_ptr();
        int* const ord = kp->group_order;
        unsigned* const cost = kp->group_cost;
        const long g = ord ? (long)__builtin_nontemporal_load(&ord[blockIdx.x]) : (long)blockIdx.x;
        cost[g] = (unsigned)__builtin_amdgcn_s_memrealtime() - cost[g];
    }
    diag_group_end<true>(K);
}
RT_MODE_END

#ifdef RT_TU_BVH
__device__ __forceinline__ float h2f(unsigned bits) {
    return (float)__builtin_bit_cast(_Float16, (unsigned short)(bits & 0xffffu));
}

#ifndef RT_REFILL_WAVES
#define RT_REFILL_WAVES 5
#endif
#ifndef RT_NODE_PAIR
#define RT_NODE_PAIR 1
#endif
RT_MODE_BEGIN
template <int BLOCK, bool N16, bool ORDER = false>
__global__ void __launch_bounds__(BLOCK) __attribute__((amdgpu_waves_per_eu(RT_REFILL_WAVES)))
rt_render_bvh_refill_kernel(rt_kparams K) {
    extern __shared__ float smem[];
    const int tid = threadIdx.x;
    const float* hit_tab = K.hit;
    int* rec_code = reinterpret_cast<int*>(smem) + tid;
    float* rec_k = smem + (K.max_bounces + 1) * BLOCK + tid;
    float* rec_c = smem + 2 * (K.max_bounces + 1) * BLOCK + tid;
    const long npix = (long)K.rows * K.width;
    const long T = (long)gridDim.x * BLOCK;
    const long nitems = items_of(K, npix);
    const long group = ORDER && K.group_order ? (long)K.group_order[blockIdx.x] : (long)blockIdx.x;
    if (ORDER && tid == 0) K.group_cost[group] = (unsigned)__builtin_amdgcn_s_memrealtime();
    PixelState px;
    load_item(K, npix, nitems, group * BLOCK + tid, px);
    const f3 cam = mk(K.cam_pos[0], K.cam_pos[1], K.cam_pos[2]);
    diag_group_start(K);
    LaneDone lane_done;

    f3 o = mk(0.0f, 0.0f, 0.0f), d = mk(0.0f, 0.0f, 1.0f);
    int depth = -1;
    bool walking = false;
    bool pending = false;
    bool idle = false;
    int node = -1, leaf = -1, leaf2 = -1;
    float best_t = INFINITY;
    int best_id = -1, best_key = -1;
    SlabRay sr;
    sr.inv = o;
    sr.oinv = o;
    sr.m = 0.0f;
    float a2 = 0.0f, a4 = 0.0f;
    const float* nodes = K.bvh_nodes;
    const unsigned* nodes16 = K.bvh_nodes16;
    const int nn = K.bvh_n_nodes;
#define NODE_LIVE(n) ((unsigned)(n) < (unsigned)nn)
    RefillStamps dg;
    while (true) {
        dg.count(3);
        while (!walking && !idle) {
            if (pending) {
                pending = false;
                diag_bvh_check(K, o, d, best_t, best_id, depth);
                bool finished = true;
                if (best_id >= 0) {
                    const float* h = hit_tab + RT_HIT_FLOATS * best_id;
                    const float4 h0 = *reinterpret_cast<const float4*>(h);
                    const float4 h2 = *reinterpret_cast<const float4*>(h + 8);
                    const f3 P = add(o, scale(best_t, d));
                    f3 n = mk(h0.x, h0.y, h0.z);
                    if (h0.w != 0.0f) n = normalize3(sub(P, n));
                    f3 scatter;
                    int code = best_id;
                    float kspec = 0.0f;
                    const float choice = rand_range(px.rs, 1.0f);
                    if (choice < RT_SPECULAR_CHANCE) {
                        scatter = specular_scatter(px.rs, d, n, h2.x, h2.z, h2.y, kspec);
                        code = ~best_id;
                    } else {
                        scatter = random_direction(px.rs, n);
                    }
                    rec_code[depth * BLOCK] = code;
                    rec_k[depth * BLOCK] = kspec;
                    rec_c[depth * BLOCK] = dot(scatter, n);
                    depth++;
                    o = P;
                    d = scatter;
                    finished = depth > K.max_bounces;
                }
                if (finished) {
                    float lx = K.bg[0], ly = K.bg[1], lz = K.bg[2];
                    for (int l = depth - 1; l >= 0; --l)
                        fold_level(rec_code[l * BLOCK], rec_k[l * BLOCK], rec_c[l * BLOCK], hit_tab, lx, ly, lz);
                    if (px.frame == 1u) {
                        px.ax = 0.0f;
                        px.ay = 0.0f;
                        px.az = 0.0f;
                    }
                    px.ax = px.ax + lx;
                    px.ay = px.ay + ly;
                    px.az = px.az + lz;
                    px.frame++;
                    px.passes_left--;
                    depth = -1;
                    if (px.passes_left == 0) {
                        store_pixel(K, npix, px);
                        load_item(K, npix, nitems, px.w + T, px);
                    }
                }
            }
            if (depth < 0) {
                if (px.passes_left <= 0) {
                    idle = true;
                    lane_done.mark(K);
                    break;
                }
                const f3 jit = random_direction(px.rs, px.d0);
                d = normalize3(add(px.d0, scale(K.jitter, jit)));
                o = cam;
                depth = 0;
            }
            best_t = INFINITY;
            best_id = -1;
            best_key = -1;
            if (!bvh_safe(K, o, d)) {
                closest_hit_brute(K, o, d, best_t, best_id);
                pending = true;
                continue;
            }
            const float a = dot(d, d);
            a4 = 4.0f * a;
            a2 = 2.0f * a;
            planes_first(K, o, d, best_t, best_id, best_key);
            sr = slab_ray(o, d);
            const int order = ray_octant(K, d);
            if (N16)
                nodes16 = K.bvh_nodes16 + (size_t)order * nn * 4;
            else
                nodes = K.bvh_nodes + (size_t)order * K.bvh_order_stride;
            node = 0;
            leaf = -1;
            leaf2 = -1;
            walking = true;
        }
        dg.stamp(0);
        if (__ballot(walking) == 0ull) break;

        while (true) {
            while (true) {
                bool stalled = false;
                if (NODE_LIVE(node)) {
                    RT_BRANCH_COUNT(K, 5);
                    if (N16) {
#define RT_N16_STEP(q)                                                                                        \
    do {                                                                                                      \
        const int w = (int)(q).w;         \
        const bool lnode = w < -1;                                                                            \
        const bool hit = slab_enter(h2f((q).x), h2f((q).x >> 16), h2f((q).y), h2f((q).y >> 16), h2f((q).z), \
                                    h2f((q).z >> 16), sr, best_t);                                            \
        const bool is_leaf = hit && lnode;                                                                    \
        const bool park = is_leaf && leaf2 < 0;                                                               \
        stalled = is_leaf != park;                                                                            \
        const bool first = park && leaf < 0;                                                                  \
        leaf2 = park != first ? ~w : leaf2;                                                                   \
        leaf = first ? ~w : leaf;                                                                             \
        node = !hit && !lnode ? w : (stalled ? node : node + 1);                                              \
    } while (0)
                        const uint4* nq = reinterpret_cast<const uint4*>(nodes16);
                        const uint4 q = nq[(unsigned)node];
#if RT_NODE_PAIR
                        const int node0 = node;
                        const uint4 q1 = nq[min((unsigned)node + 1u, (unsigned)nn - 1u)];
                        RT_N16_STEP(q);
                        asm volatile("" ::"v"(q1.x), "v"(q1.y), "v"(q1.z), "v"(q1.w));
                        if (node == node0 + 1 && NODE_LIVE(node)) RT_N16_STEP(q1);
#else
                        RT_N16_STEP(q);
#endif
#undef RT_N16_STEP
                    } else {
                        const float4 lo = *reinterpret_cast<const float4*>(nodes + 8 * node);
                        const float4 hi = *reinterpret_cast<const float4*>(nodes + 8 * node + 4);
                        const bool hit = slab_enter(lo.x, lo.y, lo.z, hi.x, hi.y, hi.z, sr, best_t);
                        const int miss = __float_as_int(lo.w);
                        const int lf = __float_as_int(hi.w);
                        const bool is_leaf = hit && lf >= 0;
                        const bool park = is_leaf && leaf2 < 0;
                        stalled = is_leaf != park;
                        const bool first = park && leaf < 0;
                        leaf2 = park != first ? lf : leaf2;
                        leaf = first ? lf : leaf;
                        node = !hit || park ? miss : (is_leaf ? node : node + 1);
                    }
                }
                dg.count(4);
                if (__popcll(__ballot(leaf >= 0) | __ballot(!NODE_LIVE(node))) >= K.leaf_batch) break;
            }
            dg.stamp(1);
            dg.count(5);
            if (leaf >= 0) {
                const int first = leaf & 0xffffff, count = leaf >> 24;
                for (int k = 0; k < count; k++) {
                    RT_BRANCH_COUNT(K, 6);
                    leaf_test<true>(K, K.bvh_leafvtx + (size_t)RT_LEAF_VFLOATS * (first + k), o, d, a2, a4, best_t,
                                    best_id, best_key);
                }
                leaf = -1;
            }
            if (leaf2 >= 0) {
                const int first = leaf2 & 0xffffff, count = leaf2 >> 24;
                for (int k = 0; k < count; k++)
                    leaf_test<true>(K, K.bvh_leafvtx + (size_t)RT_LEAF_VFLOATS * (first + k), o, d, a2, a4, best_t,
                                    best_id, best_key);
                leaf2 = -1;
            }
            dg.stamp(2);
            if (walking && !NODE_LIVE(node)) {
                walking = false;
                pending = true;
            }
            const unsigned long long w = __ballot(walking);
            const unsigned long long live = ~__ballot(idle);
            if (w == 0ull || 64 * __popcll(~w & live) >= K.refill * __popcll(live)) break;
        }
    }
    if (ORDER && tid == 0) {
        const long g = K.group_order ? (long)K.group_order[blockIdx.x] : (long)blockIdx.x;
        K.group_cost[g] = (unsigned)__builtin_amdgcn_s_memrealtime() - K.group_cost[g];
    }
    diag_group_end<false>(K);
    dg.flush(K);
#undef NODE_LIVE
}
RT_MODE_END
#endif

#ifndef RT_ORDER_MIN_GEN
#define RT_ORDER_MIN_GEN 1.1
#endif
extern thread_local long rt_order_groups_last;
extern thread_local char rt_launched_kernel[96];
hipError_t rt_launch_order_groups(const unsigned* cost, int* order, long n, hipStream_t stream);
size_t rt_render_lds_bytes(const rt_kparams& K, int block, bool hit_lds, bool sorted);
size_t rt_pair_lds_bytes(const rt_kparams& K);

RT_MODE_BEGIN
namespace {
enum { K_SIMPLE = 0, K_SORTED = 1, K_PAIR = 2 };

template <int KIND, int BLOCK, bool HIT_LDS, bool BVH = false, bool GREC = false, bool ORDER = false, bool QUADS = true>
void* kernel_ptr() {
    if constexpr (KIND == K_PAIR) return reinterpret_cast<void*>(&rt_render_pair_kernel<HIT_LDS, ORDER, QUADS>);
    if constexpr (KIND == K_SORTED)
        return reinterpret_cast<void*>(&rt_render_sorted_kernel<BLOCK, HIT_LDS, GREC, ORDER, QUADS>);
    return reinterpret_cast<void*>(&rt_render_kernel<BLOCK, HIT_LDS, BVH>);
}

template <int KIND, int BLOCK, bool HIT_LDS, bool GREC, bool ORDER, bool QUADS>
void launch_kind(const rt_kparams& K, long grid, size_t lds, hipStream_t stream) {
    if constexpr (KIND == K_PAIR)
        hipLaunchKernelGGL((rt_render_pair_kernel<HIT_LDS, ORDER, QUADS>), dim3((unsigned)grid), dim3(128), lds, stream, K);
    else
        hipLaunchKernelGGL((rt_render_sorted_kernel<BLOCK, HIT_LDS, GREC, ORDER, QUADS>), dim3((unsigned)grid),
                           dim3(BLOCK), lds, stream, K);
}

template <int KIND, int BLOCK, bool HIT_LDS, bool BVH = false, bool GREC = false>
hipError_t launch_render(const rt_kparams& K0, size_t lds, int grid_mult, int num_cus, hipStream_t stream) {
    static_assert(KIND != K_PAIR || (BLOCK == 128 && HIT_LDS && !BVH && !GREC), "pair launches: 128 lanes, 64 pixels");
    static_assert(KIND == K_SIMPLE || !BVH, "BVH scenes: the ray-refill kernel");
    constexpr int OWN = KIND == K_PAIR ? 64 : BLOCK;
    rt_kparams K = K0;
    const long nitems = launch_items(K);
    long grid = (nitems + OWN - 1) / OWN;
    if (grid_mult > 0 && KIND == K_SIMPLE) {
        int per_cu = 0;
        if (hipOccupancyMaxActiveBlocksPerMultiprocessor(&per_cu, kernel_ptr<KIND, BLOCK, HIT_LDS, BVH>(), BLOCK, lds) ==
                hipSuccess &&
            per_cu > 0) {
            const long cap = (long)per_cu * num_cus * grid_mult;
            if (grid > cap) grid = cap;
        }
    }
    if (grid < 1) grid = 1;
    K.rec_stride = (int)(grid * OWN);
    bool feedback = KIND != K_SIMPLE && K.group_cost && K.group_order && grid <= K.order_cap;
    if (feedback) {
        int per_cu = 0;
        if (hipOccupancyMaxActiveBlocksPerMultiprocessor(&per_cu, kernel_ptr<KIND, BLOCK, HIT_LDS, BVH, GREC>(), BLOCK,
                                                         lds) != hipSuccess ||
            per_cu <= 0)
            per_cu = 1;
        feedback = KIND == K_PAIR || (double)grid > RT_ORDER_MIN_GEN * (double)per_cu * num_cus;
    }
    if (!feedback) {
        K.group_cost = nullptr;
        K.group_order = nullptr;
    } else if (K.order_n != grid) {
        K.group_order = nullptr;
    }
    const bool quads = BVH || K.n_quad > 0;
    if constexpr (KIND == K_SIMPLE) {
        hipLaunchKernelGGL((rt_render_kernel<BLOCK, HIT_LDS, BVH>), dim3((unsigned)grid), dim3(BLOCK), lds, stream, K);
    } else {
        if (feedback && quads)
            launch_kind<KIND, BLOCK, HIT_LDS, GREC, true, true>(K, grid, lds, stream);
        else if (feedback)
            launch_kind<KIND, BLOCK, HIT_LDS, GREC, true, false>(K, grid, lds, stream);
        else if (quads)
            launch_kind<KIND, BLOCK, HIT_LDS, GREC, false, true>(K, grid, lds, stream);
        else
            launch_kind<KIND, BLOCK, HIT_LDS, GREC, false, false>(K, grid, lds, stream);
    }
    std::snprintf(rt_launched_kernel, sizeof rt_launched_kernel, "%s<%d%s%s%s%s>%s",
                  KIND == K_PAIR ? "rt_render_pair_kernel" : KIND == K_SORTED ? "rt_render_sorted_kernel" : "rt_render_kernel",
                  KIND == K_PAIR ? 128 : BLOCK, HIT_LDS ? "" : ",hit_global", GREC ? ",grec" : "", BVH ? ",bvh" : "",
                  RT_MODE_TAG, feedback ? "+order" : "");
    hipError_t e = hipGetLastError();
    if (e == hipSuccess && feedback && (K0.order_sort || K0.order_n != grid)) {
        e = rt_launch_order_groups(K0.group_cost, K0.group_order, grid, stream);
        if (e == hipSuccess) rt_order_groups_last = grid;
    }
    return e;
}

}

#ifdef RT_TU_BVH
hipError_t rt_launch_render_bvh_refill(const rt_kparams& K0, int num_cus, hipStream_t s) {
    constexpr int BLOCK = 64;
    rt_kparams K = K0;
    const long nitems = launch_items(K);
    const long grid = (nitems + BLOCK - 1) / BLOCK < 1 ? 1 : (nitems + BLOCK - 1) / BLOCK;
    const size_t lds = (size_t)3 * (K.max_bounces + 1) * BLOCK * sizeof(float);
    bool feedback = K.group_cost && K.group_order && grid <= K.order_cap;
    if (feedback) {
        int per_cu = 0;
        const void* kp = K.bvh_nodes16 ? reinterpret_cast<const void*>(&rt_render_bvh_refill_kernel<BLOCK, true, true>)
                                       : reinterpret_cast<const void*>(&rt_render_bvh_refill_kernel<BLOCK, false, true>);
        if (hipOccupancyMaxActiveBlocksPerMultiprocessor(&per_cu, kp, BLOCK, lds) != hipSuccess || per_cu <= 0)
            per_cu = 1;
        feedback = (double)grid > RT_ORDER_MIN_GEN * (double)per_cu * num_cus;
    }
    if (!feedback) {
        K.group_cost = nullptr;
        K.group_order = nullptr;
    } else if (K.order_n != grid) {
        K.group_order = nullptr;
    }
    const bool n16 = K.bvh_nodes16 != nullptr;
    if (feedback && n16)
        hipLaunchKernelGGL((rt_render_bvh_refill_kernel<BLOCK, true, true>), dim3((unsigned)grid), dim3(BLOCK), lds, s, K);
    else if (feedback)
        hipLaunchKernelGGL((rt_render_bvh_refill_kernel<BLOCK, false, true>), dim3((unsigned)grid), dim3(BLOCK), lds, s, K);
    else if (n16)
        hipLaunchKernelGGL((rt_render_bvh_refill_kernel<BLOCK, true>), dim3((unsigned)grid), dim3(BLOCK), lds, s, K);
    else
        hipLaunchKernelGGL((rt_render_bvh_refill_kernel<BLOCK, false>), dim3((unsigned)grid), dim3(BLOCK), lds, s, K);
    std::snprintf(rt_launched_kernel, sizeof rt_launched_kernel, "rt_render_bvh_refill_kernel<64%s%s>%s",
                  n16 ? ",n16" : "", RT_MODE_TAG, feedback ? "+order" : "");
    hipError_t e = hipGetLastError();
    if (e == hipSuccess && feedback && (K0.order_sort || K0.order_n != grid)) {
        e = rt_launch_order_groups(K0.group_cost, K0.group_order, grid, s);
        if (e == hipSuccess) rt_order_groups_last = grid;
    }
    return e;
}

hipError_t rt_launch_render_bvh_simple(const rt_kparams& K, int block, size_t lds, int grid_mult, int num_cus,
                                       hipStream_t s) {
    return block == 64 ? launch_render<K_SIMPLE, 64, false, true>(K, lds, grid_mult, num_cus, s)
                       : launch_render<K_SIMPLE, 256, false, true>(K, lds, grid_mult, num_cus, s);
}
RT_MODE_END
#else
hipError_t rt_launch_render_bvh_simple(const rt_kparams& K, int block, size_t lds, int grid_mult, int num_cus,
                                       hipStream_t s);
hipError_t rt_launch_render_bvh_refill(const rt_kparams& K, int num_cus, hipStream_t s);

namespace {
template <int BLOCK, int KIND>
hipError_t launch_block(const rt_kparams& K, bool hit_lds, size_t lds, int grid_mult, int num_cus, hipStream_t s) {
    if constexpr (KIND == K_SIMPLE) {
        if (K.bvh_nodes)
            return rt_launch_render_bvh_simple(K, BLOCK, lds, grid_mult, num_cus, s);
    }
    if (KIND == K_SORTED && K.rec)
        return hit_lds ? launch_render<KIND, BLOCK, true, false, true>(K, lds, grid_mult, num_cus, s)
                       : launch_render<KIND, BLOCK, false, false, true>(K, lds, grid_mult, num_cus, s);
    return hit_lds ? launch_render<KIND, BLOCK, true>(K, lds, grid_mult, num_cus, s)
                   : launch_render<KIND, BLOCK, false>(K, lds, grid_mult, num_cus, s);
}
}

#ifndef RT_GREC_MIN_GEN
#define RT_GREC_MIN_GEN 1.4
#endif
bool rt_render_wants_global_records(const rt_kparams& K, int num_cus) {
    if (K.bvh_nodes || K.max_bounces <= 0) return false;
    const int n_prim = K.n_sph + K.n_pln + K.n_tri + K.n_quad;
    const bool hit_lds = (size_t)n_prim * RT_HIT_FLOATS * sizeof(float) <= 16384;
    rt_kparams L = K;
    L.rec = nullptr;
    const size_t lds = rt_render_lds_bytes(L, 256, hit_lds, true);
    const long groups = (long)(160 * 1024) / (long)(lds ? lds : 1);
    if (groups < RT_WAVES_PER_EU) return true;
    L.rec = reinterpret_cast<float*>(&L);
    const size_t lds_g = rt_render_lds_bytes(L, 256, hit_lds, true);
    int occ_l = 0, occ_g = 0;
    const void* kl = hit_lds ? kernel_ptr<K_SORTED, 256, true>() : kernel_ptr<K_SORTED, 256, false>();
    const void* kg = hit_lds ? kernel_ptr<K_SORTED, 256, true, false, true>() : kernel_ptr<K_SORTED, 256, false, false, true>();
    if (hipOccupancyMaxActiveBlocksPerMultiprocessor(&occ_l, kl, 256, lds) != hipSuccess ||
        hipOccupancyMaxActiveBlocksPerMultiprocessor(&occ_g, kg, 256, lds_g) != hipSuccess || occ_g <= occ_l)
        return false;
    const double gens = (double)((long)K.rows * K.width) / (256.0 * occ_g * (num_cus > 0 ? num_cus : 1));
    return gens >= RT_GREC_MIN_GEN;
}
RT_MODE_END

#ifdef RT_TU_SHARED
size_t rt_pair_lds_bytes(const rt_kparams& K) {
    const int n_prim = K.n_sph + K.n_pln + K.n_tri + K.n_quad;
    return (size_t)((n_prim * RT_HIT_FLOATS + 3) & ~3) * sizeof(float) +
           (size_t)(3 * (K.max_bounces > 0 ? K.max_bounces : 0) + RT_PAIR_FIELDS) * 64 * sizeof(float) + 4 * sizeof(int);
}

size_t rt_render_rec_floats(const rt_kparams& K) {
    const long nitems = launch_items(K);
    const int lds_levels = K.max_bounces < RT_GREC_LDS_LEVELS ? K.max_bounces : RT_GREC_LDS_LEVELS;
    const size_t planes = (size_t)3 * (K.max_bounces - lds_levels);
    return planes ? planes * (size_t)((nitems + 255) / 256 * 256) : 1;
}

size_t rt_render_lds_bytes(const rt_kparams& K, int block, bool hit_lds, bool sorted) {
    const int n_prim = K.n_sph + K.n_pln + K.n_tri + K.n_quad;
    const size_t hit = hit_lds ? (size_t)((n_prim * RT_HIT_FLOATS + 3) & ~3) * sizeof(float) : 0;
    const int lds_levels = sorted && K.rec ? (K.max_bounces < RT_GREC_LDS_LEVELS ? K.max_bounces : RT_GREC_LDS_LEVELS)
                                           : K.max_bounces + (sorted ? 0 : 1);
    size_t b = hit + (size_t)3 * (lds_levels > 0 ? lds_levels : 0) * block * sizeof(float);
    if (sorted) b += (size_t)13 * block * sizeof(float) + 8 * sizeof(int);
    return b;
}
#endif

#ifndef RT_SPREAD_PIX
#define RT_SPREAD_PIX 1400
#endif
#ifndef RT_PAIR_MIN_CHAIN
#define RT_PAIR_MIN_CHAIN 8
#endif
RT_MODE_BEGIN
hipError_t rt_launch_render(const rt_kparams& K, int num_cus, int grid_mult, bool simple, int block_req,
                            hipStream_t stream, int pair_req) {
    simple = simple || K.spp_inner > 1;
    if (K.bvh_nodes && !simple) return rt_launch_render_bvh_refill(K, num_cus, stream);
    const int n_prim = K.n_sph + K.n_pln + K.n_tri + K.n_quad;
#ifdef RT_NO_HIT_LDS
    const bool hit_lds = false;
#else
    const bool hit_lds = !K.bvh_nodes && (size_t)n_prim * RT_HIT_FLOATS * sizeof(float) <= 16384;
#endif
    const bool small_block = (size_t)3 * (K.max_bounces + 1) * 256 * sizeof(float) > 49152;
    const int block = small_block ? 64 : 256;
    const size_t lds = rt_render_lds_bytes(K, block, hit_lds, !simple);
    if (simple)
        return small_block ? launch_block<64, K_SIMPLE>(K, hit_lds, lds, grid_mult, num_cus, stream)
                           : launch_block<256, K_SIMPLE>(K, hit_lds, lds, grid_mult, num_cus, stream);
#ifndef RT_SORTED_BLOCK
#define RT_SORTED_BLOCK 256
#endif
    if (small_block) return launch_block<64, K_SORTED>(K, hit_lds, lds, grid_mult, num_cus, stream);
    const long items = (long)K.rows * K.width;
    const bool pair = hit_lds && !K.rec && (block_req == 0 || block_req == 128) &&
                      (pair_req > 0 || (pair_req < 0 && block_req == 0 && items <= (long)num_cus * RT_SPREAD_PIX &&
                                        (long)K.samples * (K.max_bounces + 1) >= RT_PAIR_MIN_CHAIN));
    if (pair)
        return launch_render<K_PAIR, 128, true>(K, rt_pair_lds_bytes(K), grid_mult, num_cus, stream);
    if (block_req == 64 || block_req == 128 || block_req == 256) {
        const size_t lds_r = rt_render_lds_bytes(K, block_req, hit_lds, true);
        if (lds_r <= 65536) {
            if (block_req == 64) return launch_block<64, K_SORTED>(K, hit_lds, lds_r, grid_mult, num_cus, stream);
            if (block_req == 128) return launch_block<128, K_SORTED>(K, hit_lds, lds_r, grid_mult, num_cus, stream);
            return launch_block<256, K_SORTED>(K, hit_lds, lds_r, grid_mult, num_cus, stream);
        }
    }
    const size_t lds_s = rt_render_lds_bytes(K, RT_SORTED_BLOCK, hit_lds, true);
    auto waves_per_cu = [](size_t lds_bytes, int block) {
        const long by_lds = (long)(160 * 1024 / (lds_bytes ? lds_bytes : 1)) * (block / 64);
        return by_lds < 4L * RT_WAVES_PER_EU ? by_lds : 4L * RT_WAVES_PER_EU;
    };
    const bool few_groups = items < (long)num_cus * 4 * RT_SORTED_BLOCK;
    if (RT_SORTED_BLOCK > 128 &&
        (few_groups ||
         waves_per_cu(rt_render_lds_bytes(K, 128, hit_lds, true), 128) > waves_per_cu(lds_s, RT_SORTED_BLOCK))) {
        const size_t lds_128 = rt_render_lds_bytes(K, 128, hit_lds, true);
        return launch_block<128, K_SORTED>(K, hit_lds, lds_128, grid_mult, num_cus, stream);
    }
    return launch_block<RT_SORTED_BLOCK, K_SORTED>(K, hit_lds, lds_s, grid_mult, num_cus, stream);
}
RT_MODE_END

#ifdef RT_TU_SHARED
thread_local long rt_order_groups_last = 0;
thread_local char rt_launched_kernel[96] = "";

hipError_t rt_launch_order_groups(const unsigned* cost, int* order, long n, hipStream_t stream) {
    hipLaunchKernelGGL(rt_order_groups_kernel, dim3(1), dim3(1024), 0, stream, cost, order, (int)n);
    return hipGetLastError();
}

hipError_t rt_launch_init_rand(unsigned* rng, int width, int rows, int row_offset, int row_stride,
                               hipStream_t stream) {
    const long npix = (long)rows * width;
    const unsigned grid = (unsigned)((npix + 255) / 256);
    hipLaunchKernelGGL(rt_init_rand_kernel, dim3(grid), dim3(256), 0, stream, rng, width, rows,
                       row_offset, row_stride);
    return hipGetLastError();
}

hipError_t rt_launch_deinterleave(const unsigned* gathered, unsigned* image, int width, int height,
                                  int shards, int rows_per_shard, int max_blocks, hipStream_t stream) {
    const bool vec = width % 4 == 0 && ((reinterpret_cast<uintptr_t>(gathered) | reinterpret_cast<uintptr_t>(image)) & 15) == 0;
    const long n = (long)height * (vec ? width / 4 : width);
    long grid = (n + 255) / 256;
    if (max_blocks > 0 && grid > max_blocks) grid = max_blocks;
    if (vec)
        hipLaunchKernelGGL(rt_deinterleave_kernel<4>, dim3((unsigned)grid), dim3(256), 0, stream, gathered, image,
                           width, height, shards, rows_per_shard);
    else
        hipLaunchKernelGGL(rt_deinterleave_kernel<1>, dim3((unsigned)grid), dim3(256), 0, stream, gathered, image,
                           width, height, shards, rows_per_shard);
    return hipGetLastError();
}
#endif
#endif

template <bool BVH>
__global__ void __launch_bounds__(256) rt_aov_kernel(const rt_kparams K, float4* __restrict__ ga,
                                                     float4* __restrict__ gb, float4* __restrict__ alb) {
    const long npix = (long)K.rows * K.width;
    const long i = (long)blockIdx.x * 256 + threadIdx.x;
    const bool valid = i < npix;
    const long p = valid ? i : npix - 1;
    const int j = (int)(p / K.width);
    const int x = (int)(p - (long)j * K.width);
    const int y = K.row_offset + j * K.row_stride;
    const f3 o = mk(K.cam_pos[0], K.cam_pos[1], K.cam_pos[2]);
    const f3 d = primary_dir(K, x, y);
    float t;
    int id;
    closest_hit<BVH>(K, o, d, t, id);
    const AovHit a = aov_shade(K, o, d, t, id);
    if (valid) {
        ga[p] = make_float4(a.n.x, a.n.y, a.n.z, __int_as_float(a.prim));
        gb[p] = make_float4(a.P.x, a.P.y, a.P.z, a.depth);
        if (alb) alb[p] = make_float4(a.albedo.x, a.albedo.y, a.albedo.z, 0.0f);
    }
}

#if defined(RT_TU_SHARED) || (defined(RT_TU_BVH) && !defined(RT_FAST))
#ifdef RT_TU_SHARED
hipError_t rt_launch_aov(const rt_kparams& K, float4* ga, float4* gb, float4* alb, hipStream_t stream) {
    constexpr bool kBvh = false;
#else
hipError_t rt_launch_aov_bvh(const rt_kparams& K, float4* ga, float4* gb, float4* alb, hipStream_t stream) {
    constexpr bool kBvh = true;
#endif
    const long npix = (long)K.rows * K.width;
    if (npix <= 0) return hipErrorInvalidValue;
    hipLaunchKernelGGL(rt_aov_kernel<kBvh>, dim3((unsigned)((npix + 255) / 256)), dim3(256), 0, stream, K, ga, gb, alb);
    return hipGetLastError();
}
#endif
```

bwidman-raytracer_amd/csrc/rt_layout.h:

```cpp
#pragma once

#define RT_SPH_FLOATS 4
#define RT_PLN_FLOATS 4
#define RT_TRI_FLOATS 28
#define RT_QUAD_FLOATS 32
#define RT_TRI_CULL 24
#define RT_QUAD_CULL 28
#define RT_POLY_EDGES 4
#define RT_LEAF_FLOATS 32
#define RT_LEAF_VFLOATS 16
#ifndef RT_HIT_FLOATS
#define RT_HIT_FLOATS 16
#endif

#define RT_NEAR_ZERO 0.0001f
#define RT_SPECULAR_CHANCE 0.5f
#define RT_PI 3.1415926535f
#define RT_MAX_LEVELS 33

#define RT_GTIMES_WORDS (1ull << 22)

struct rt_kparams {
    int width, height;
    int row_offset, row_stride;
    int rows;
    int samples;
    int max_bounces;
    unsigned first_frame;
    float cam_pos[3];
    float rot[9];
    float screen_z;
    float jitter;
    float bg[3];
    int n_sph, n_pln, n_tri, n_quad, n_max;
    const float* sph;
    const float* pln;
    const float* tri;
    const float* quad;
    const float* hit;
    unsigned* rng;
    float* accum;
    unsigned* rgba;
    unsigned long long* stamps;
    int tile_w;
    int tile_sq;
    const float* bvh_nodes;
    const float* bvh_leafrec;
    const float* bvh_leafvtx;
    int bvh_order_stride;
    int bvh_order_mask;
    const unsigned* bvh_nodes16;
    int bvh_n_nodes;
    float ovf_sc, ovf_nm, ovf_im;
    float cull_omax;
    float cull_dmax;
    float* rec;
    int rec_stride;
    int* group_order;
    unsigned* group_cost;
    long order_n;
    long order_cap;
    int order_sort;
    int leaf_batch;
    int refill;
    int spp_inner;
};

#ifndef RT_LEAF_BATCH
#define RT_LEAF_BATCH 60
#endif
#ifndef RT_LEAF_BATCH_SMALL
#define RT_LEAF_BATCH_SMALL 62
#endif
#ifndef RT_REFILL
#define RT_REFILL 40
#endif
#ifndef RT_REFILL_SMALL
#define RT_REFILL_SMALL 32
#endif

#define RT_KEY(kind, i) ((i) * 4 + (kind))

struct rt_dn_level {
    int width, height;
    int step;
    int first;
    int last;
    float ic, in, ip;
    float inv;
    const float* accum;
    const float4* src;
    float4* dst;
    unsigned* rgba;
    const float4* ga;
    const float4* gb;
};

struct rt_tp_args {
    int width, height;
    int has_history;
    float n;
    float inv;
    float max_history, normal_cos_min, plane_tol;
    float h_cam[3];
    float h_rot[9];
    float h_screen_z;
    const float* accum;
    const float4* ga;
    const float4* gb;
    const float4* h_col;
    const float4* h_ga;
    const float4* h_gb;
    float4* p_col;
    float4* p_ga;
    float4* p_gb;
    unsigned* rgba;
};

struct rt_mom_args {
    long npix;
    int first;
    float kf;
    float invk;
    float kw;
    const float* accum;
    float* prev;
    float2* mom;
};

struct rt_dv_args {
    int width, height;
    int step;
    int last;
    int tracked;
    float in, ip;
    float inv;
    float rd;
    float sigma_lum;
    const float* accum;
    const float2* mom;
    const float4* src;
    float4* dst;
    float* rs;
    unsigned* rgba;
    const float4* ga;
    const float4* gb;
};
```

bwidman-raytracer_amd/csrc/rt_path.h:

```cpp
#pragma once
#include <hip/hip_runtime.h>

#include <math.h>

#include "rt_layout.h"
#include "rt_sqrt.h"

#define RT_HD __host__ __device__ __forceinline__

#if defined(RT_FAST) && defined(__HIP_DEVICE_COMPILE__)
#define RT_FAST_DEVICE 1
#else
#define RT_FAST_DEVICE 0
#endif

namespace {

RT_HD float rt_sqrt(float x) {
#if RT_FAST_DEVICE
    return sqrt_hw(x);
#elif defined(__HIP_DEVICE_COMPILE__)
    return sqrt_cr(x);
#else
    return sqrtf(x);
#endif
}

RT_HD float rt_rcp(float x) {
#if RT_FAST_DEVICE
    return rcp_hw(x);
#elif defined(__HIP_DEVICE_COMPILE__)
    return rcp_cr(x);
#else
    return 1.0f / x;
#endif
}

RT_HD float rt_inv_len(float s) {
#if RT_FAST_DEVICE
    return inv_length_hw(s);
#elif defined(__HIP_DEVICE_COMPILE__)
    return inv_length_cr(s);
#else
    return 1.0f / sqrtf(s);
#endif
}

RT_HD float rt_div(float x, float y) {
#if RT_FAST_DEVICE
    return x * rcp_hw(y);
#else
    return x / y;
#endif
}

RT_HD float rt_div_spec_chance(float x) {
#if RT_FAST_DEVICE
    return x * (1.0f / RT_SPECULAR_CHANCE);
#else
    return x / RT_SPECULAR_CHANCE;
#endif
}

RT_HD unsigned rt_xor3(unsigned a, unsigned b, unsigned c) {
#if defined(__HIP_DEVICE_COMPILE__)
    return __builtin_amdgcn_bitop3_b32(a, b, c, 0x96);
#else
    return a ^ b ^ c;
#endif
}

#if defined(__HIP_DEVICE_COMPILE__)
typedef const __attribute__((address_space(4))) float* cfloat_ptr;
#else
typedef const float* cfloat_ptr;
#endif
RT_HD cfloat_ptr as_const(const float* p) { return (cfloat_ptr)p; }

RT_HD int rt_f2i(float x) { return __builtin_bit_cast(int, x); }
RT_HD float rt_i2f(int x) { return __builtin_bit_cast(float, x); }

#if defined(RT_STAMPS) && defined(RT_BRANCH_STATS) && defined(__HIP_DEVICE_COMPILE__)
#define RT_BRANCH_COUNT(K, k)                                                                          \
    do {                                                                                               \
        const unsigned long long _m = __ballot(1);                                                     \
        if (__builtin_amdgcn_mbcnt_hi((unsigned)(_m >> 32), __builtin_amdgcn_mbcnt_lo((unsigned)_m, 0u)) == 0 && \
            (K).stamps) {                                                                              \
            atomicAdd(&(K).stamps[17 + 2 * (k)], 1ull);                                                \
            atomicAdd(&(K).stamps[18 + 2 * (k)], (unsigned long long)__popcll(_m));                    \
        }                                                                                              \
    } while (0)
#else
#define RT_BRANCH_COUNT(K, k) \
    do {                      \
    } while (0)
#endif

struct f3 {
    float x, y, z;
};

RT_HD f3 mk(float x, float y, float z) {
    f3 r;
    r.x = x;
    r.y = y;
    r.z = z;
    return r;
}
RT_HD f3 add(f3 a, f3 b) { return mk(a.x + b.x, a.y + b.y, a.z + b.z); }
RT_HD f3 sub(f3 a, f3 b) { return mk(a.x - b.x, a.y - b.y, a.z - b.z); }
RT_HD f3 scale(float k, f3 v) { return mk(k * v.x, k * v.y, k * v.z); }
RT_HD float dot(f3 a, f3 b) { return a.x * b.x + a.y * b.y + a.z * b.z; }
RT_HD f3 cross(f3 a, f3 b) {
    float i = a.y * b.z - a.z * b.y;
    float j = -(a.x * b.z - a.z * b.x);
    float k = a.x * b.y - a.y * b.x;
    return mk(i, j, k);
}
RT_HD float length3(f3 v) { return rt_sqrt(v.x * v.x + v.y * v.y + v.z * v.z); }
RT_HD f3 normalize3(f3 v) { return scale(rt_inv_len(v.x * v.x + v.y * v.y + v.z * v.z), v); }
RT_HD float square(float x) { return x * x; }
RT_HD float chi(float x) { return (x > 0.0f) ? 1.0f : 0.0f; }

struct Xorwow {
    unsigned d, v0, v1, v2, v3, v4;
};

RT_HD Xorwow xorwow_seed(unsigned long long seed) {
    const unsigned s0 = (unsigned)seed ^ 0xaad26b49u;
    const unsigned s1 = (unsigned)(seed >> 32) ^ 0xf7dcefddu;
    const unsigned t0 = 1099087573u * s0;
    const unsigned t1 = 2591861531u * s1;
    Xorwow s;
    s.d = 6615241u + t1 + t0;
    s.v0 = 123456789u + t0;
    s.v1 = 362436069u ^ t0;
    s.v2 = 521288629u + t1;
    s.v3 = 88675123u ^ t1;
    s.v4 = 5783321u + t0;
    return s;
}

RT_HD unsigned long long pixel_seed(int x, int y, int width) { return (unsigned long long)(long long)(y * width + x); }

RT_HD unsigned next_u32(Xorwow& s) {
    unsigned t = s.v0 ^ (s.v0 >> 2);
    s.v0 = s.v1;
    s.v1 = s.v2;
    s.v2 = s.v3;
    s.v3 = s.v4;
    s.v4 = rt_xor3(s.v4, s.v4 << 4, t) ^ (t << 1);
    s.d += 362437u;
    return s.v4 + s.d;
}

RT_HD float rand_range(Xorwow& s, float max) {
    float u = (float)next_u32(s);
    return u * (2.3283064365386963e-10f * max);
}

RT_HD float rand_pm1(Xorwow& s) { return __builtin_fmaf((float)next_u32(s), 4.656612873077393e-10f, -1.0f); }

#define FOPI 1.27323954473516f
#define DP1 0.78515625f
#define DP2 2.4187564849853515625e-4f
#define DP3 3.77489497744594108e-8f

RT_HD float poly_sin(float r, float z) {
    float p = -1.9515295891e-4f * z;
    p = p + 8.3321608736e-3f;
    p = p * z;
    p = p - 1.6666654611e-1f;
    p = p * z;
    p = p * r;
    return p + r;
}

RT_HD float poly_cos(float z) {
    float p = 2.443315711809948e-5f * z;
    p = p - 1.388731625493765e-3f;
    p = p * z;
    p = p + 4.166664568298827e-2f;
    p = p * z;
    p = p * z;
    p = p - 0.5f * z;
    return p + 1.0f;
}

RT_HD float reduce_quadrant(float x, int& jout) {
    int j = (int)(x * FOPI);
    float y = (float)j;
    if (j & 1) {
        j += 1;
        y += 1.0f;
    }
    jout = j & 7;
    float r = x - y * DP1;
    r = r - y * DP2;
    r = r - y * DP3;
    return r;
}

RT_HD void sincos_nn(float x, float& s, float& c) {
    const bool xneg = x < 0.0f;
    if (xneg) x = -x;
    int j;
    float r = reduce_quadrant(x, j);
    int sneg = 0, cneg = 0;
    if (j > 3) {
        sneg = 1;
        cneg = 1;
        j -= 4;
    }
    if (j > 1) cneg = !cneg;
    float z = r * r;
    float ps = poly_sin(r, z);
    float pc = poly_cos(z);
    bool swap = (j == 1 || j == 2);
    float sv = swap ? pc : ps;
    float cv = swap ? ps : pc;
    if (xneg) sneg = !sneg;
    s = sneg ? -sv : sv;
    c = cneg ? -cv : cv;
}

RT_HD void rt_sincos(float x, float& s, float& c) {
#if RT_FAST_DEVICE
    sincos_hw(x, s, c);
#else
    sincos_nn(x, s, c);
#endif
}

RT_HD float atan_nn(float x) {
    const bool xneg = x < 0.0f;
    if (xneg) x = -x;
    float y;
    if (x > 2.414213562373095f) {
        y = 1.5707963267948966f;
        x = -rt_rcp(x);
    } else if (x > 0.4142135623730950f) {
        y = 0.7853981633974483f;
        x = rt_div(x - 1.0f, x + 1.0f);
    } else {
        y = 0.0f;
    }
    float z = x * x;
    float p = 8.05374449538e-2f * z;
    p = p - 1.38776856032e-1f;
    p = p * z;
    p = p + 1.99777106478e-1f;
    p = p * z;
    p = p - 3.33329491539e-1f;
    p = p * z;
    p = p * x;
    p = p + x;
    y = y + p;
    return xneg ? -y : y;
}

RT_HD float exp_nn(float x) {
    if (x < -87.0f) return 0.0f;
    const float fn = floorf(x * 1.44269504088896341f + 0.5f);
    float r = x - fn * 0.693359375f;
    r = r - fn * -2.12194440e-4f;
    const float z = r * r;
    float p = 1.9875691500e-4f * r;
    p = p + 1.3981999507e-3f;
    p = p * r;
    p = p + 8.3334519073e-3f;
    p = p * r;
    p = p + 4.1665795894e-2f;
    p = p * r;
    p = p + 1.6666665459e-1f;
    p = p * r;
    p = p + 5.0000001201e-1f;
    p = p * z;
    p = p + r;
    p = p + 1.0f;
    return rt_i2f(rt_f2i(p) + (int)((unsigned)(int)fn << 23));
}

RT_HD float shadowing_masking(f3 dir, f3 n, f3 m, float rough2) {
    float vdn = dot(dir, n);
    float tan_theta = fmaxf(rt_rcp(vdn * vdn) - 1.0f, 0.0f);
    return rt_div(chi(rt_div(dot(dir, m), vdn)) * 2.0f, 1.0f + rt_sqrt(1.0f + rough2 * tan_theta * tan_theta));
}

RT_HD float fresnel(f3 incident, f3 normal, float ior2m1) {
    float c = fabsf(dot(incident, normal));
    float g_root = ior2m1 + c * c;
    if (g_root < 0.0f) return 1.0f;
    float g = rt_sqrt(g_root);
    return rt_div(0.5f * square(g - c), square(g + c)) *
           (1.0f + rt_div(square(c * (g + c) - 1.0f), square(c * (g - c) + 1.0f)));
}

RT_HD float specular_weight(f3 i, f3 o, f3 n, f3 m, float rough2) {
    float g = shadowing_masking(i, n, m, rough2) * shadowing_masking(o, n, m, rough2);
    if (isnan(g)) return 1.0f;
    float den = fabsf(dot(i, n) * dot(m, n));
    if (den == 0.0f) den = RT_NEAR_ZERO;
    return rt_div(fabsf(dot(i, m)) * g, den);
}

RT_HD f3 random_direction(Xorwow& s, f3 normal, int* iters = nullptr) {
    f3 r;
    do {
        if (iters) ++*iters;
        float x = rand_pm1(s);
        float y = rand_pm1(s);
        float z = rand_pm1(s);
        r = mk(x, y, z);
    } while (r.x * r.x + r.y * r.y + r.z * r.z > 1.00000012f);
    r = normalize3(r);
    if (dot(normal, r) < 0.0f) r = sub(r, scale(2.0f * dot(r, normal), normal));
    return r;
}

RT_HD f3 specular_scatter(Xorwow& rs, f3 d, f3 n, float rough, float rough2, float ior2m1, float& kspec) {
    const float e1 = rand_range(rs, 1.0f);
    const float e2 = rand_range(rs, 1.0f);
    const float theta = atan_nn(rt_div(rough * rt_sqrt(e1), rt_sqrt(1.0f - e1)));
    const float phi = 2.0f * RT_PI * e2;
    float st, ct, sp, cp;
    rt_sincos(theta, st, ct);
    rt_sincos(phi, sp, cp);
    const f3 mloc = mk(st * cp, st * sp, ct);
    f3 some = mk(1.0f, 0.0f, 0.0f);
    if (fabsf(dot(n, some)) < 1.0f - RT_NEAR_ZERO) some = mk(0.0f, 1.0f, 0.0f);
    const f3 t1 = cross(n, some);
    const f3 t2 = cross(n, t1);
    const f3 m = mk(dot(mk(t1.x, t2.x, n.x), mloc), dot(mk(t1.y, t2.y, n.y), mloc), dot(mk(t1.z, t2.z, n.z), mloc));
    const f3 scatter = sub(d, scale(2.0f * dot(d, m), m));
    const f3 inc = scale(-1.0f, d);
    const float fr = fresnel(inc, m, ior2m1);
    const float sw = specular_weight(inc, scatter, n, m, rough2);
    kspec = rt_div_spec_chance(sw * fr);
    return scatter;
}

RT_HD bool polygon_edges(cfloat_ptr q, int nv, f3 P) {
    bool inside = true;
#pragma unroll
    for (int k = 0; k < 4; k++) {
        if (k < nv) {
            f3 v = mk(q[6 * k + 0], q[6 * k + 1], q[6 * k + 2]);
            f3 in = mk(q[6 * k + 3], q[6 * k + 4], q[6 * k + 5]);
            if (dot(in, sub(P, v)) < 0.0f) inside = false;
        }
    }
    return inside;
}

struct CullRay {
    float a, a_k;
    bool ok;
};

RT_HD CullRay cull_ray(const rt_kparams& K, f3 o, f3 d, float a) {
    CullRay c;
    c.a = a;
    c.a_k = a * (1.0f - 6.103515625e-05f);
    c.ok = fmaxf(fmaxf(fabsf(o.x), fabsf(o.y)), fabsf(o.z)) <= K.cull_omax &&
           fmaxf(fmaxf(fabsf(d.x), fabsf(d.y)), fabsf(d.z)) <= K.cull_dmax;
    return c;
}

RT_HD bool culled(cfloat_ptr cs, const CullRay& cr, f3 o, f3 d) {
    const float wx = cs[0] - o.x, wy = cs[1] - o.y, wz = cs[2] - o.z;
    const float ww = __builtin_fmaf(wx, wx, __builtin_fmaf(wy, wy, wz * wz));
    const float pj = __builtin_fmaf(wx, d.x, __builtin_fmaf(wy, d.y, wz * d.z));
    const float lhs = __builtin_fmaf(-pj, pj, ww * cr.a_k);
    return cr.ok && lhs > cs[3] * cr.a;
}

RT_HD void polygon_test(const rt_kparams& K, cfloat_ptr q, int nv, f3 o, f3 d, int id, const CullRay& cr,
                        float& best_t, int& best_id) {
    if (culled(q + (nv == 3 ? RT_TRI_CULL : RT_QUAD_CULL), cr, o, d)) return;
    RT_BRANCH_COUNT(K, 2);
    float nx = q[0], ny = q[1], nz = q[2], dd = q[3];
    float nd = nx * d.x + ny * d.y + nz * d.z;
    if (!(fabsf(nd) < RT_NEAR_ZERO)) {
        float t = rt_div(-((nx * o.x + ny * o.y + nz * o.z) + dd), nd);
        bool plane_hit = !(t <= RT_NEAR_ZERO || t > INFINITY);
        if (plane_hit && !(t <= RT_NEAR_ZERO || t > best_t)) {
            RT_BRANCH_COUNT(K, 3);
            f3 P = add(o, scale(t, d));
            if (polygon_edges(q + RT_POLY_EDGES, nv, P)) {
                best_t = t;
                best_id = id;
            }
        }
    }
}

#ifndef RT_HIT_UNROLL
#define RT_HIT_UNROLL 1
#endif
#define RT_PRAGMA(x) _Pragma(#x)
#define RT_PRAGMA_UNROLL(n) RT_PRAGMA(unroll n)
template <bool QUADS = true, int STEP = 1>
RT_HD void closest_hit_brute(const rt_kparams& K, f3 o, f3 d, float& best_t, int& best_id, int i0 = 0) {
    const float a = dot(d, d);
    const float a4 = 4.0f * a;
    const float a2 = 2.0f * a;
    best_t = INFINITY;
    best_id = -1;
    const int pln_base = K.n_sph;
    const int tri_base = K.n_sph + K.n_pln;
    const int quad_base = tri_base + K.n_tri;
    const CullRay cr = cull_ray(K, o, d, a);
    RT_BRANCH_COUNT(K, 4);
#if RT_HIT_UNROLL > 1
    RT_PRAGMA_UNROLL(RT_HIT_UNROLL)
#endif
    for (int i = i0; i < K.n_max; i += STEP) {
        if (i < K.n_sph) {
            const cfloat_ptr s = as_const(K.sph) + RT_SPH_FLOATS * i;
            f3 xp = mk(o.x - s[0], o.y - s[1], o.z - s[2]);
            float b = 2.0f * dot(xp, d);
            float c = dot(xp, xp) - s[3];
            float disc = b * b - a4 * c;
            if (!(disc < 0.0f) && !(b >= 0.0f && disc == disc && a2 > 0.0f)) {
                RT_BRANCH_COUNT(K, 0);
                float t = rt_div(-b - rt_sqrt(disc), a2);
                if (!(t <= RT_NEAR_ZERO || t > best_t)) {
                    best_t = t;
                    best_id = i;
                }
            }
        }
        if (i < K.n_pln) {
            const cfloat_ptr q = as_const(K.pln) + RT_PLN_FLOATS * i;
            float nx = q[0], ny = q[1], nz = q[2], dd = q[3];
            float nd = nx * d.x + ny * d.y + nz * d.z;
            if (!(fabsf(nd) < RT_NEAR_ZERO)) {
                float t = rt_div(-((nx * o.x + ny * o.y + nz * o.z) + dd), nd);
                if (!(t <= RT_NEAR_ZERO || t > best_t)) {
                    best_t = t;
                    best_id = pln_base + i;
                }
            }
        }
        if (i < K.n_tri) polygon_test(K, as_const(K.tri) + RT_TRI_FLOATS * i, 3, o, d, tri_base + i, cr, best_t, best_id);
        if (QUADS && i < K.n_quad)
            polygon_test(K, as_const(K.quad) + RT_QUAD_FLOATS * i, 4, o, d, quad_base + i, cr, best_t, best_id);
    }
}

RT_HD bool key_accept(float t, int key, float best_t, int best_key) {
    return !(t <= RT_NEAR_ZERO) && (t < best_t || (t == best_t && key > best_key));
}

RT_HD bool bvh_safe(const rt_kparams& K, f3 o, f3 d) {
    const float om = fmaxf(fmaxf(fabsf(o.x), fabsf(o.y)), fabsf(o.z));
    const float dm = fmaxf(fmaxf(fabsf(d.x), fabsf(d.y)), fabsf(d.z));
    if (!(om + K.ovf_sc < 1e18f && dm < 1e18f && dm > 1e-15f && dm * (om + K.ovf_sc) < 1e18f &&
          K.ovf_nm * dm < 1e36f && K.ovf_nm * (om + 3.0f * K.ovf_sc) < 1e33f))
        return false;
    const float pm = om + K.ovf_sc + 6e4f * dm * (K.ovf_nm * (om + 3.0f * K.ovf_sc));
    return pm < 1e37f && K.ovf_im * pm < 3e36f;
}

RT_HD void planes_first(const rt_kparams& K, f3 o, f3 d, float& best_t, int& best_id, int& best_key) {
    for (int i = 0; i < K.n_pln; i++) {
        const cfloat_ptr q = as_const(K.pln) + RT_PLN_FLOATS * i;
        const float nd = q[0] * d.x + q[1] * d.y + q[2] * d.z;
        if (!(fabsf(nd) < RT_NEAR_ZERO)) {
            const float t = rt_div(-((q[0] * o.x + q[1] * o.y + q[2] * o.z) + q[3]), nd);
            const int key = RT_KEY(1, i);
            if (key_accept(t, key, best_t, best_key)) {
                best_t = t;
                best_id = K.n_sph + i;
                best_key = key;
            }
        }
    }
}

struct SlabRay {
    f3 inv, oinv;
    float m;
};

RT_HD SlabRay slab_ray(f3 o, f3 d) {
    const float tiny = 1e-20f;
    const f3 dc = mk(fabsf(d.x) < tiny ? copysignf(tiny, d.x) : d.x, fabsf(d.y) < tiny ? copysignf(tiny, d.y) : d.y,
                     fabsf(d.z) < tiny ? copysignf(tiny, d.z) : d.z);
    SlabRay s;
    s.inv = mk(rt_rcp(dc.x), rt_rcp(dc.y), rt_rcp(dc.z));
    s.oinv = mk(o.x * s.inv.x, o.y * s.inv.y, o.z * s.inv.z);
    s.m = 1e-6f + 9.5367431640625e-07f * fmaxf(fmaxf(fabsf(s.oinv.x), fabsf(s.oinv.y)), fabsf(s.oinv.z));
    return s;
}

RT_HD int ray_octant(const rt_kparams& K, f3 d) {
    return ((d.x < 0.0f) | ((d.y < 0.0f) << 1) | ((d.z < 0.0f) << 2)) & K.bvh_order_mask;
}

RT_HD bool slab_test(float lx, float ly, float lz, float hx, float hy, float hz, const SlabRay& s, float best_t,
                     float& tmin, float& tmax) {
    const float tx0 = __builtin_fmaf(lx, s.inv.x, -s.oinv.x), tx1 = __builtin_fmaf(hx, s.inv.x, -s.oinv.x);
    const float ty0 = __builtin_fmaf(ly, s.inv.y, -s.oinv.y), ty1 = __builtin_fmaf(hy, s.inv.y, -s.oinv.y);
    const float tz0 = __builtin_fmaf(lz, s.inv.z, -s.oinv.z), tz1 = __builtin_fmaf(hz, s.inv.z, -s.oinv.z);
    tmin = fmaxf(fmaxf(fminf(tx0, tx1), fminf(ty0, ty1)), fmaxf(fminf(tz0, tz1), 0.0f));
    tmax = fminf(fminf(fmaxf(tx0, tx1), fmaxf(ty0, ty1)), fmaxf(tz0, tz1));
    return tmin <= tmax * (1.0f + 1e-5f) + s.m && tmin <= best_t * (1.0f + 1e-5f) + (1e-5f + s.m);
}

RT_HD bool slab_enter(float lx, float ly, float lz, float hx, float hy, float hz, const SlabRay& s, float best_t) {
    float tmin, tmax;
    return slab_test(lx, ly, lz, hx, hy, hz, s, best_t, tmin, tmax);
}

template <bool VTX = false>
RT_HD void leaf_test(const rt_kparams& K, const float* r, f3 o, f3 d, float a2, float a4, float& best_t, int& best_id,
                     int& best_key) {
    const float4 c0 = *reinterpret_cast<const float4*>(r);
    const float4 c1 = *reinterpret_cast<const float4*>(r + 4);
    const float4 c2 = *reinterpret_cast<const float4*>(r + 8);
#if defined(__HIP_DEVICE_COMPILE__)
    asm volatile("" ::"v"(c2.x), "v"(c2.y), "v"(c2.z), "v"(c2.w));
#endif
    const int key = rt_f2i(c0.x), kind = key & 3, idx = key >> 2;
    if (kind == 0) {
        const f3 xp = mk(o.x - c0.y, o.y - c0.z, o.z - c0.w);
        const float b = 2.0f * dot(xp, d);
        const float c = dot(xp, xp) - c1.x;
        const float disc = b * b - a4 * c;
        if (!(disc < 0.0f) && !(b >= 0.0f)) {
            const float t = rt_div(-b - rt_sqrt(disc), a2);
            if (key_accept(t, key, best_t, best_key)) {
                best_t = t;
                best_id = idx;
                best_key = key;
            }
        }
        return;
    }
    if (VTX) {
        const f3 v0 = mk(c0.y, c0.z, c0.w), v1 = mk(c1.x, c1.y, c1.z), v2 = mk(c1.w, c2.x, c2.y);
        const f3 n = cross(sub(v1, v0), sub(v2, v1));
        const float dd = -dot(n, v0);
        const float nd = n.x * d.x + n.y * d.y + n.z * d.z;
        if (fabsf(nd) < RT_NEAR_ZERO) return;
        const float t = rt_div(-((n.x * o.x + n.y * o.y + n.z * o.z) + dd), nd);
        if (!key_accept(t, key, best_t, best_key)) return;
        const f3 P = add(o, scale(t, d));
        if (dot(cross(n, sub(v1, v0)), sub(P, v0)) < 0.0f) return;
        if (dot(cross(n, sub(v2, v1)), sub(P, v1)) < 0.0f) return;
        if (kind == 2) {
            if (dot(cross(n, sub(v0, v2)), sub(P, v2)) < 0.0f) return;
        } else {
            const float4 c3 = *reinterpret_cast<const float4*>(r + 12);
            const f3 v3 = mk(c2.z, c2.w, c3.x);
            if (dot(cross(n, sub(v3, v2)), sub(P, v2)) < 0.0f) return;
            if (dot(cross(n, sub(v0, v3)), sub(P, v3)) < 0.0f) return;
        }
        best_t = t;
        best_id = (kind == 2 ? K.n_sph + K.n_pln : K.n_sph + K.n_pln + K.n_tri) + idx;
        best_key = key;
        return;
    }
    const float nd = c0.y * d.x + c0.z * d.y + c0.w * d.z;
    if (fabsf(nd) < RT_NEAR_ZERO) return;
    const float t = rt_div(-((c0.y * o.x + c0.z * o.y + c0.w * o.z) + c1.x), nd);
    if (!key_accept(t, key, best_t, best_key)) return;
    const f3 P = add(o, scale(t, d));
    if (dot(mk(c2.x, c2.y, c2.z), sub(P, mk(c1.y, c1.z, c1.w))) < 0.0f) return;
    const float4 c3 = *reinterpret_cast<const float4*>(r + 12);
    const float4 c4 = *reinterpret_cast<const float4*>(r + 16);
#if defined(__HIP_DEVICE_COMPILE__)
    asm volatile("" ::"v"(c4.y), "v"(c4.z), "v"(c4.w));
#endif
    if (dot(mk(c3.z, c3.w, c4.x), sub(P, mk(c2.w, c3.x, c3.y))) < 0.0f) return;
    const float4 c5 = *reinterpret_cast<const float4*>(r + 20);
    if (dot(mk(c5.x, c5.y, c5.z), sub(P, mk(c4.y, c4.z, c4.w))) < 0.0f) return;
    if (kind == 3) {
        const float4 c6 = *reinterpret_cast<const float4*>(r + 24);
        const float4 c7 = *reinterpret_cast<const float4*>(r + 28);
        if (dot(mk(c6.z, c6.w, c7.x), sub(P, mk(c5.w, c6.x, c6.y))) < 0.0f) return;
    }
    best_t = t;
    best_id = (kind == 2 ? K.n_sph + K.n_pln : K.n_sph + K.n_pln + K.n_tri) + idx;
    best_key = key;
}

RT_HD f3 primary_dir(const rt_kparams& K, int x, int y) {
    const f3 pix = mk((float)(x - K.width / 2), (float)(y - K.height / 2), K.screen_z);
    const f3 pr = mk(K.rot[0] * pix.x + K.rot[1] * pix.y + K.rot[2] * pix.z,
                     K.rot[3] * pix.x + K.rot[4] * pix.y + K.rot[5] * pix.z,
                     K.rot[6] * pix.x + K.rot[7] * pix.y + K.rot[8] * pix.z);
    return normalize3(pr);
}

struct AovHit {
    f3 albedo, n, P;
    float depth;
    int prim;
};

RT_HD AovHit aov_shade(const rt_kparams& K, f3 o, f3 d, float t, int id) {
    AovHit a;
    if (id < 0) {
        a.albedo = mk(K.bg[0], K.bg[1], K.bg[2]);
        a.n = mk(0.0f, 0.0f, 0.0f);
        a.P = mk(0.0f, 0.0f, 0.0f);
        a.depth = INFINITY;
        a.prim = -1;
        return a;
    }
    const float* h = K.hit + RT_HIT_FLOATS * id;
    a.P = add(o, scale(t, d));
    const f3 n = mk(h[0], h[1], h[2]);
    a.n = normalize3(h[3] != 0.0f ? sub(a.P, n) : n);
    a.albedo = mk(h[7], h[11], h[15]);
    a.depth = t;
    a.prim = id;
    return a;
}

RT_HD void fold_level(int c0, float k, float c, const float* hit_tab, float& lx, float& ly, float& lz) {
    const bool spec = c0 < 0;
    const float* h = hit_tab + RT_HIT_FLOATS * (spec ? ~c0 : c0);
    const float4 e = *reinterpret_cast<const float4*>(h + 4);
    const float4 da = *reinterpret_cast<const float4*>(h + 12);
    const float bx = spec ? k : da.x, by = spec ? k : da.y, bz = spec ? k : da.z;
    lx = e.x + (bx * lx) * c;
    ly = e.y + (by * ly) * c;
    lz = e.z + (bz * lz) * c;
}

RT_HD unsigned to_u8(float v) {
    float r = roundf(v);
    if (r != r) return 0u;
    if (r <= 0.0f) return 0u;
    if (r >= 255.0f) return 255u;
    return (unsigned)r;
}

RT_HD unsigned tone_map(float ax, float ay, float az, unsigned n) {
    const float inv = rt_div(1.0f, (float)n);
    float v[3] = {inv * ax, inv * ay, inv * az};
    unsigned px = 0xff000000u;
#pragma unroll
    for (int ch = 0; ch < 3; ch++) {
        float cc = 0.6f * v[ch];
        float num = cc * (2.51f * cc + 0.03f);
        float den = cc * (2.43f * cc + 0.59f) + 0.14f;
        float tm = fminf(rt_div(num, den), 1.0f);
        float g = rt_sqrt(tm) * 255.0f;
        px |= to_u8(g) << (8 * ch);
    }
    return px;
}

}
```

bwidman-raytracer_amd/csrc/rt_render.cpp:

```cpp
#include <cmath>

#include "rt_context.h"

static int prepare(rt_context* c, const rt_render_params* p, rt_kparams& K, unsigned& first) {
    const HostFpEnv fp;
    if (!c || !p) return fail(c, RT_ERR_INVALID_ARGUMENT, "null argument");
    if (!c->has_scene) return fail(c, RT_ERR_NO_SCENE, "rt_set_scene() not called");
    const int stride = p->row_stride == 0 ? 1 : p->row_stride;
    if (p->width <= 0 || p->height <= 0 || p->samples <= 0 || p->row_offset < 0 || stride < 0 ||
        p->row_offset >= p->height)
        return fail(c, RT_ERR_INVALID_ARGUMENT, "bad render params %dx%d samples %d shard %d/%d", p->width,
                    p->height, p->samples, p->row_offset, stride);
    if (p->max_bounces < 0) return fail(c, RT_ERR_INVALID_ARGUMENT, "max_bounces < 0");
    if (p->max_bounces > RT_MAX_BOUNCES)
        return fail(c, RT_ERR_UNSUPPORTED, "max_bounces %d > %d", p->max_bounces, RT_MAX_BOUNCES);
    if (c->width != p->width || c->height != p->height || c->row_offset != p->row_offset ||
        c->row_stride != stride || !c->rng.p) {
        int rc = rt_init_rand(c, p->width, p->height, p->row_offset, stride);
        if (rc) return rc;
    }
    first = p->first_frame ? p->first_frame : c->frame;
    if ((unsigned long long)first + (unsigned)p->samples > 0xffffffffull)
        return fail(c, RT_ERR_INVALID_ARGUMENT, "frame counter overflow");
    if (!c->cpu) HIP_TRY(c, hipSetDevice(c->device));

    fill_view(c, p->width, p->height, p->row_offset, stride, c->rows, K);
    K.samples = p->samples;
    K.max_bounces = p->max_bounces;
    K.first_frame = first;
    K.rng = c->rng.as<unsigned>();
    K.accum = c->accum.as<float>();
    return RT_OK;
}

void fill_view(rt_context* c, int width, int height, int row_offset, int stride, int rows, rt_kparams& K) {
    std::memset(&K, 0, sizeof K);
    K.width = width;
    K.height = height;
    K.row_offset = row_offset;
    K.row_stride = stride;
    K.rows = rows;
    const rt_camera& cam = c->camera;
    K.cam_pos[0] = cam.position.x;
    K.cam_pos[1] = cam.position.y;
    K.cam_pos[2] = cam.position.z;
    K.screen_z = -(float)(width / 2) / tanf(cam.fov / 2.0f);
    {
        const float cy = cosf(cam.angle[0]), sy = sinf(cam.angle[0]);
        const float cx = cosf(cam.angle[1]), sx = sinf(cam.angle[1]);
        const float L[3][3] = {{cy, 0, sy}, {0, 1, 0}, {-sy, 0, cy}};
        const float U[3][3] = {{1, 0, 0}, {0, cx, -sx}, {0, sx, cx}};
        for (int i = 0; i < 3; i++)
            for (int j = 0; j < 3; j++)
                K.rot[3 * i + j] = L[i][0] * U[0][j] + L[i][1] * U[1][j] + L[i][2] * U[2][j];
    }
    K.jitter = (float)(0.001 * (width / 1000));
    K.bg[0] = c->background[0];
    K.bg[1] = c->background[1];
    K.bg[2] = c->background[2];
    const rt_compiled_scene& sc = c->scene;
    K.n_sph = sc.n_sph;
    K.n_pln = sc.n_pln;
    K.n_tri = sc.n_tri;
    K.n_quad = sc.n_quad;
    K.cull_omax = sc.cull_omax;
    K.bvh_order_stride = sc.bvh_nodes_per_order * 8;
    K.bvh_order_mask = sc.bvh_order_mask;
    int nmax = sc.n_sph;
    if (sc.n_pln > nmax) nmax = sc.n_pln;
    if (sc.n_tri > nmax) nmax = sc.n_tri;
    if (sc.n_quad > nmax) nmax = sc.n_quad;
    K.n_max = nmax;
    const float* base = c->scene_buf.as<const float>();
    K.sph = base;
    K.pln = base + sc.off_pln;
    K.tri = base + sc.off_tri;
    K.quad = base + sc.off_quad;
    K.hit = base + sc.off_hit;
    K.bvh_nodes = sc.off_bvh ? base + sc.off_bvh : nullptr;
    K.bvh_leafrec = sc.off_bvh ? base + sc.off_bvh_prims : nullptr;
    K.bvh_leafvtx = sc.off_bvh ? base + sc.off_bvh_vtx : nullptr;
    K.bvh_nodes16 = sc.off_bvh && sc.off_bvh16 ? reinterpret_cast<const unsigned*>(base + sc.off_bvh16) : nullptr;
    K.bvh_n_nodes = sc.bvh_nodes_per_order;
    K.ovf_sc = sc.ovf_sc;
    K.ovf_nm = sc.ovf_nm;
    K.ovf_im = sc.ovf_im;
    K.cull_dmax = sc.cull_dmax;
    K.spp_inner = c->spp_inner;
}

static int moments_prepare(rt_context* c, unsigned first, int samples, rt_mom_args& A, bool& run) {
    run = c->mom_on && (first == 1u || (c->mom_live && first == c->mom_next));
    if (!run) {
        c->mom_drop();
        return RT_OK;
    }
    const size_t npix = (size_t)c->rows * c->width;
    const char* oom = "host moments for %zu pixels";
    int rc = ensure_buf(c, c->mom_prev, npix * 3 * sizeof(float), oom, npix);
    if (!rc) rc = ensure_buf(c, c->mom_m, npix * sizeof(float2), oom, npix);
    if (rc) {
        c->mom_drop();
        return rc;
    }
    const HostFpEnv fp;
    A.npix = (long)npix;
    A.first = first == 1u;
    A.kf = (float)samples;
    A.invk = 1.0f / A.kf;
    A.kw = A.kf / (float)(first - 1u + (unsigned)samples);
    A.accum = c->accum.as<float>();
    A.prev = c->mom_prev.as<float>();
    A.mom = c->mom_m.as<float2>();
    return RT_OK;
}

static void moments_commit(rt_context* c, unsigned first, int samples) {
    if (first == 1u) c->mom_batches = 0;
    c->mom_live = true;
    c->mom_batches++;
    c->mom_next = first + (unsigned)samples;
}

static int cpu_render(rt_context* c, const rt_render_params* p, int threads, uint8_t* rgba_out, float* accum_out) {
    rt_kparams K;
    unsigned first = 0;
    int rc = prepare(c, p, K, first);
    if (rc) return rc;
    const size_t npix = (size_t)c->rows * c->width;
    K.rgba = c->rgba.as<unsigned>();
    rt_mom_args MA;
    bool track = false;
    if ((rc = moments_prepare(c, first, p->samples, MA, track))) return rc;
    (void)c->render.begin(nullptr, true);
    rt_cpu_render(K, threads > 0 ? threads : c->threads);
    if (track) {
        rt_cpu_moments(MA, threads > 0 ? threads : c->threads);
        moments_commit(c, first, p->samples);
    }
    (void)c->render.end(nullptr);
    c->frame = first + (unsigned)p->samples;
    if (rgba_out) std::memcpy(rgba_out, c->rgba.p, npix * 4);
    if (accum_out) planes_to_rgb(c->accum.as<float>(), npix, accum_out);
    return RT_OK;
}

static int launch(rt_context* c, rt_kparams& K, hipStream_t s, unsigned first, int samples) {
    const bool small = (long)K.rows * K.width <= (long)c->num_cus * 1024;
    K.tile_w = c->tile_w >= 0 ? c->tile_w : K.bvh_nodes ? (small ? 4 : 8) : (small ? 32 : 8);
    K.tile_sq = c->tile_sq;
    K.leaf_batch = c->leaf_batch > 0 ? c->leaf_batch : small ? RT_LEAF_BATCH_SMALL : RT_LEAF_BATCH;
    K.refill = c->refill > 0 ? c->refill : small ? RT_REFILL_SMALL : RT_REFILL;
    K.rec = nullptr;
    const bool fast = c->precision == RT_PRECISION_REFERENCE_FAST;
    if (!c->simple && (c->grec == 1 || (c->grec < 0 && (fast ? rt_fast::rt_render_wants_global_records(K, c->num_cus)
                                                             : rt_render_wants_global_records(K, c->num_cus))))) {
        const int rc = ensure_buf(c, c->rec, rt_render_rec_floats(K) * sizeof(float));
        if (rc) return rc;
        K.rec = c->rec.as<float>();
    }
    unsigned long long* stamps = nullptr;
    const int NST = 40;
    if (tuning_env("BWRT_STAMPS")) {
        if (hipMalloc(&stamps, NST * sizeof(unsigned long long)) == hipSuccess)
            (void)hipMemsetAsync(stamps, 0, NST * sizeof(unsigned long long), s);
        K.stamps = stamps;
    }
    const char* gtimes = tuning_env("BWRT_GTIMES");
    const size_t NGT = (size_t)RT_GTIMES_WORDS;
    if (gtimes && !stamps) {
        if (hipMalloc(&stamps, NGT * sizeof(unsigned long long)) == hipSuccess)
            (void)hipMemsetAsync(stamps, 0, NGT * sizeof(unsigned long long), s);
        K.stamps = stamps;
    }
    if (c->order_feedback && !c->simple) {
        const size_t cap = ((size_t)K.width + 128) * ((size_t)K.rows + 128) / 64 + 1;
        const void* before = c->gorder.p;
        int rc = ensure_buf(c, c->gcost, cap * sizeof(unsigned));
        if (!rc) rc = ensure_buf(c, c->gorder, cap * sizeof(int));
        if (rc) return rc;
        if (c->gorder.p != before) c->order_n = 0;
        K.group_cost = c->gcost.as<unsigned>();
        K.group_order = c->gorder.as<int>();
        K.order_n = c->order_n;
        K.order_cap = (long)(c->gorder.bytes / sizeof(int));
        K.order_sort = K.bvh_nodes || c->order_stale || c->launches % (unsigned long long)c->order_period == 0;
        c->order_stale = false;
    }
    rt_mom_args MA;
    bool track = false;
    if (const int rc = moments_prepare(c, first, samples, MA, track)) return rc;
    int orc = order_after_all(c, s);
    if (orc) return orc;
    rt_order_groups_last = 0;
    rt_launched_kernel[0] = 0;
    HIP_TRY(c, c->render.begin(s, c->ktiming));
    hipError_t e = fast ? rt_fast::rt_launch_render(K, c->num_cus, c->grid_mult, c->simple, c->block, s, c->spread)
                        : rt_launch_render(K, c->num_cus, c->grid_mult, c->simple, c->block, s, c->spread);
    if (e == hipSuccess && rt_order_groups_last > 0) c->order_n = rt_order_groups_last;
    c->kernel_name = rt_launched_kernel;
    c->launches++;
    if (gtimes && stamps) {
        std::vector<unsigned long long> h(NGT);
        (void)hipMemcpyAsync(h.data(), stamps, NGT * sizeof(unsigned long long), hipMemcpyDeviceToHost, s);
        (void)hipStreamSynchronize(s);
        if (FILE* f = std::fopen(gtimes, "wb")) {
            std::fwrite(h.data(), sizeof(unsigned long long), NGT, f);
            std::fclose(f);
        }
        (void)hipFree(stamps);
        stamps = nullptr;
    }
    if (stamps) {
        unsigned long long h[NST] = {0};
        (void)hipMemcpyAsync(h, stamps, sizeof h, hipMemcpyDeviceToHost, s);
        (void)hipStreamSynchronize(s);
        std::fprintf(stderr, "stamps");
        for (int k = 0; k < NST; k++) std::fprintf(stderr, " %llu", h[k]);
        std::fprintf(stderr, "\n");
        (void)hipFree(stamps);
    }
    if (e != hipSuccess) {
        c->mom_drop();
        return hip_fail(c, e, "rt_render_kernel launch");
    }
    if (track) {
        e = rt_launch_moments(MA, s);
        if (e != hipSuccess) {
            c->mom_drop();
            return hip_fail(c, e, "rt_moments_kernel launch");
        }
        moments_commit(c, first, samples);
    }
    HIP_TRY(c, c->render.end(s));
    c->frame = first + (unsigned)samples;
    return RT_OK;
}

static rt_render_params next_frames(const rt_context* c, int width, int height, int samples, int row_offset,
                                    int row_stride) {
    rt_render_params p;
    p.width = width;
    p.height = height;
    p.samples = samples;
    p.max_bounces = c->max_bounces;
    p.first_frame = 0;
    p.row_offset = row_offset;
    p.row_stride = row_stride;
    return p;
}

extern "C" {

int rt_render_ex(rt_context* c, const rt_render_params* p, uint8_t* rgba_out, float* accum_out) {
    if (c && c->cpu) return cpu_render(c, p, 0, rgba_out, accum_out);
    rt_kparams K;
    unsigned first = 0;
    int rc = prepare(c, p, K, first);
    if (rc) return rc;
    const size_t npix = (size_t)c->rows * c->width;
    rc = ensure_buf(c, c->rgba, npix * 4);
    if (rc) return rc;
    K.rgba = c->rgba.as<unsigned>();
    rc = launch(c, K, c->stream, first, p->samples);
    if (rc) return rc;
    if (rgba_out) HIP_TRY(c, hipMemcpyAsync(rgba_out, c->rgba.p, npix * 4, hipMemcpyDeviceToHost, c->stream));
    if (accum_out) {
        std::vector<float> planes(npix * 3);
        HIP_TRY(c, hipMemcpyAsync(planes.data(), c->accum.p, npix * 3 * sizeof(float), hipMemcpyDeviceToHost,
                                  c->stream));
        HIP_TRY(c, hipStreamSynchronize(c->stream));
        planes_to_rgb(planes.data(), npix, accum_out);
    }
    HIP_TRY(c, hipStreamSynchronize(c->stream));
    return RT_OK;
}

int rt_render(rt_context* c, int width, int height, int samples, uint8_t* rgba_out) {
    if (!c) return RT_ERR_INVALID_ARGUMENT;
    const rt_render_params p = next_frames(c, width, height, samples, 0, 1);
    return rt_render_ex(c, &p, rgba_out, nullptr);
}

int rt_render_multi(rt_context* const* ctxs, int n, int width, int height, int samples, uint8_t* rgba_out) {
    if (!ctxs || n <= 0 || width <= 0 || height <= 0 || samples <= 0) return RT_ERR_INVALID_ARGUMENT;
    for (int i = 0; i < n; i++) {
        if (!ctxs[i]) return RT_ERR_INVALID_ARGUMENT;
        if (ctxs[i]->cpu) return fail(ctxs[i], RT_ERR_UNSUPPORTED, "rt_render_multi: CPU context");
        for (int j = 0; j < i; j++)
            if (ctxs[j] == ctxs[i]) return fail(ctxs[i], RT_ERR_INVALID_ARGUMENT, "context listed twice");
    }
    const int active = n < height ? n : height;
    auto drain = [&](int launched, int rc) {
        for (int j = 0; j < launched; j++) {
            (void)hipSetDevice(ctxs[j]->device);
            (void)hipStreamSynchronize(ctxs[j]->stream);
        }
        return rc;
    };
    for (int i = 0; i < active; i++) {
        rt_context* c = ctxs[i];
        const rt_render_params p = next_frames(c, width, height, samples, i, n);
        rt_kparams K;
        unsigned first = 0;
        int rc = prepare(c, &p, K, first);
        if (rc) return drain(i, rc);
        const size_t bytes = (size_t)c->rows * width * 4;
        rc = ensure_buf(c, c->rgba, bytes);
        if (rc) return drain(i, rc);
        if (c->host_rgba_bytes < bytes) {
            rc = quiesce(c);
            if (rc) return drain(i, rc);
            if (hipStreamSynchronize(c->stream) != hipSuccess) return drain(i, fail(c, RT_ERR_HIP, "stream sync"));
            if (c->host_rgba) (void)hipHostFree(c->host_rgba);
            c->host_rgba = nullptr;
            c->host_rgba_bytes = 0;
            const hipError_t e = hipHostMalloc(&c->host_rgba, bytes, hipHostMallocDefault);
            if (e != hipSuccess) return drain(i, hip_fail(c, e, "hipHostMalloc"));
            c->host_rgba_bytes = bytes;
        }
        K.rgba = c->rgba.as<unsigned>();
        rc = launch(c, K, c->stream, first, samples);
        if (rc) return drain(i + 1, rc);
        const hipError_t e = hipMemcpyAsync(c->host_rgba, c->rgba.p, bytes, hipMemcpyDeviceToHost, c->stream);
        if (e != hipSuccess) return drain(i + 1, hip_fail(c, e, "hipMemcpyAsync"));
    }
    for (int i = 0; i < active; i++) {
        rt_context* c = ctxs[i];
        HIP_TRY(c, hipSetDevice(c->device));
        HIP_TRY(c, hipStreamSynchronize(c->stream));
        if (!rgba_out) continue;
        const uint8_t* src = (const uint8_t*)c->host_rgba;
        for (int j = 0; j < c->rows; j++)
            std::memcpy(rgba_out + ((size_t)(i + j * n) * width) * 4, src + (size_t)j * width * 4, (size_t)width * 4);
    }
    return RT_OK;
}

int rt_render_device(rt_context* c, const rt_render_params* p, void* rgba_device, void* stream) {
    if (c && c->cpu) return fail(c, RT_ERR_UNSUPPORTED, "rt_render_device: CPU context");
    rt_kparams K;
    unsigned first = 0;
    int rc = prepare(c, p, K, first);
    if (rc) return rc;
    if (rgba_device && ((uintptr_t)rgba_device & 3u))
        return fail(c, RT_ERR_INVALID_ARGUMENT, "rgba_device not 4-byte aligned");
    K.rgba = (unsigned*)rgba_device;
    hipStream_t s = stream ? (hipStream_t)stream : c->stream;
    return launch(c, K, s, first, p->samples);
}

int rt_deinterleave_rows_device(rt_context* c, const void* gathered, void* image, int width, int height,
                                int shards, int rows_per_shard, void* stream) {
    if (!c || !gathered || !image) return fail(c, RT_ERR_INVALID_ARGUMENT, "null argument");
    if (width <= 0 || height <= 0 || shards <= 0 || rows_per_shard * shards < height)
        return fail(c, RT_ERR_INVALID_ARGUMENT, "bad deinterleave geometry");
    if (c->cpu) return fail(c, RT_ERR_UNSUPPORTED, "rt_deinterleave_rows_device: CPU context");
    HIP_TRY(c, hipSetDevice(c->device));
    hipStream_t s = stream ? (hipStream_t)stream : c->stream;
    HIP_TRY(c, rt_launch_deinterleave((const unsigned*)gathered, (unsigned*)image, width, height, shards,
                                      rows_per_shard, c->deint_blocks, s));
    HIP_TRY(c, c->aux.end(s));
    return RT_OK;
}

int rt_render_cpu(rt_context* c, const rt_render_params* p, int threads, uint8_t* rgba_out, float* accum_out) {
    if (!c) return RT_ERR_INVALID_ARGUMENT;
    if (!c->cpu) return fail(c, RT_ERR_INVALID_ARGUMENT, "rt_render_cpu: not a CPU context (rt_create_cpu)");
    if (threads < 0) return fail(c, RT_ERR_INVALID_ARGUMENT, "threads < 0");
    return cpu_render(c, p, threads, rgba_out, accum_out);
}

}
```

include/rt_abi.h:

```cpp
#ifndef RT_ABI_H
#define RT_ABI_H

#include <stddef.h>
#include <stdint.h>

#ifdef __cplusplus
extern "C" {
#endif

#if defined(__GNUC__)
#define RT_API __attribute__((visibility("default")))
#else
#define RT_API
#endif


typedef struct rt_vec3 {
    float x, y, z;
} rt_vec3;

typedef struct rt_material {
    rt_vec3 albedo;
    float emittance;
    float roughness;
    float refractive_index;
} rt_material;

typedef struct rt_sphere {
    rt_vec3 position;
    float radius;
    rt_material mat;
} rt_sphere;

typedef struct rt_plane {
    rt_vec3 origin;
    rt_vec3 directions[2];
    rt_material mat;
} rt_plane;

typedef struct rt_triangle {
    rt_vec3 vertices[3];
    rt_material mat;
} rt_triangle;

typedef struct rt_quad {
    rt_vec3 vertices[4];
    rt_material mat;
} rt_quad;

typedef struct rt_camera {
    rt_vec3 position;
    float angle[2];
    float fov;
} rt_camera;

typedef struct rt_scene {
    rt_camera camera;
    const rt_sphere* spheres;
    int sphere_count;
    const rt_plane* planes;
    int plane_count;
    const rt_triangle* triangles;
    int triangle_count;
    const rt_quad* quads;
    int quad_count;
} rt_scene;


typedef enum rt_status {
    RT_OK = 0,
    RT_ERR_INVALID_ARGUMENT = -1,
    RT_ERR_NO_DEVICE = -2,
    RT_ERR_HIP = -3,
    RT_ERR_OUT_OF_MEMORY = -4,
    RT_ERR_NO_SCENE = -5,
    RT_ERR_UNSUPPORTED = -6
} rt_status;

#define RT_MAX_BOUNCES 32
#define RT_DEFAULT_MAX_BOUNCES 5

typedef struct rt_render_params {
    int width;
    int height;
    int samples;
    int max_bounces;
    unsigned first_frame;
    int row_offset;
    int row_stride;
} rt_render_params;


typedef struct rt_context rt_context;

RT_API const char* rt_version(void);

RT_API rt_material rt_material_default(void);

RT_API int rt_device_count(void);

RT_API int rt_create(int device, rt_context** out);
RT_API void rt_destroy(rt_context* ctx);


RT_API int rt_cpu_threads(void);

RT_API int rt_create_cpu(int threads, rt_context** out);

RT_API int rt_context_threads(const rt_context* ctx);

RT_API int rt_render_cpu(rt_context* ctx, const rt_render_params* p, int threads,
                         uint8_t* rgba_out, float* accum_out);

RT_API int rt_set_scene(rt_context* ctx, const rt_scene* scene);

RT_API int rt_set_camera(rt_context* ctx, const rt_camera* camera);

RT_API int rt_reset_accumulation(rt_context* ctx);

RT_API unsigned rt_frame_counter(const rt_context* ctx);

RT_API int rt_set_max_bounces(rt_context* ctx, int max_bounces);

RT_API int rt_set_background(rt_context* ctx, float r, float g, float b);

typedef enum rt_precision { RT_PRECISION_EXACT = 0, RT_PRECISION_REFERENCE_FAST = 1 } rt_precision;
RT_API int rt_set_precision(rt_context* ctx, int precision);
RT_API int rt_get_precision(const rt_context* ctx);

#define RT_MAX_SAMPLES_PER_PIXEL 1024
RT_API int rt_set_samples_per_pixel(rt_context* ctx, int n);

RT_API int rt_get_camera(const rt_context* ctx, rt_camera* camera);

#define RT_KEY_W          (1u << 0)
#define RT_KEY_A          (1u << 1)
#define RT_KEY_S          (1u << 2)
#define RT_KEY_D          (1u << 3)
#define RT_KEY_SPACE      (1u << 4)
#define RT_KEY_LEFT_SHIFT (1u << 5)
#define RT_KEY_LEFT       (1u << 6)
#define RT_KEY_RIGHT      (1u << 7)
#define RT_KEY_UP         (1u << 8)
#define RT_KEY_DOWN       (1u << 9)
#define RT_KEY_ESCAPE     (1u << 10)
#define RT_CONTROLS_MOVED 1
#define RT_CONTROLS_QUIT 2

RT_API int rt_apply_controls(rt_camera* camera, unsigned keys, float delta_time);

RT_API int rt_controls(rt_context* ctx, unsigned keys, float delta_time);

RT_API int rt_init_rand(rt_context* ctx, int width, int height,
                        int row_offset, int row_stride);

RT_API int rt_render(rt_context* ctx, int width, int height, int samples,
                     uint8_t* rgba_out);

RT_API int rt_render_ex(rt_context* ctx, const rt_render_params* p,
                        uint8_t* rgba_out, float* accum_out);

RT_API int rt_render_device(rt_context* ctx, const rt_render_params* p,
                            void* rgba_device, void* stream);

RT_API void* rt_get_stream(rt_context* ctx);

RT_API int rt_synchronize(rt_context* ctx);

RT_API int rt_render_multi(rt_context* const* ctxs, int n, int width, int height, int samples,
                           uint8_t* rgba_out);

RT_API float rt_last_kernel_ms(rt_context* ctx);

RT_API const char* rt_last_kernel_name(const rt_context* ctx);

RT_API int rt_set_kernel_timing(rt_context* ctx, int enable);

RT_API int rt_shard_rows(int height, int row_offset, int row_stride);

RT_API int rt_deinterleave_rows_device(rt_context* ctx, const void* gathered,
                                       void* image, int width, int height,
                                       int shards, int rows_per_shard,
                                       void* stream);

RT_API int rt_get_state(rt_context* ctx, uint32_t* rng, float* accum);
RT_API int rt_set_state(rt_context* ctx, const uint32_t* rng,
                        const float* accum, unsigned frame_counter);


RT_API int rt_render_aov(rt_context* ctx, const rt_render_params* p,
                         float* albedo , float* normal ,
                         float* depth , int32_t* prim );

#define RT_DENOISE_MAX_ITERATIONS 6
typedef struct rt_denoise_params {
    int iterations;
    float sigma_color;
    float sigma_normal;
    float sigma_plane;
} rt_denoise_params;
RT_API rt_denoise_params rt_denoise_params_default(void);

RT_API int rt_denoise(rt_context* ctx, const rt_denoise_params* params,
                      uint8_t* rgba_out, float* color_out);
RT_API int rt_denoise_device(rt_context* ctx, const rt_denoise_params* params,
                             void* rgba_device, void* stream);
RT_API float rt_last_denoise_ms(rt_context* ctx);

typedef struct rt_temporal_params {
    float max_history;
    float normal_cos_min;
    float plane_tol;
} rt_temporal_params;
RT_API rt_temporal_params rt_temporal_params_default(void);

RT_API int rt_temporal(rt_context* ctx, const rt_temporal_params* params, const rt_denoise_params* dn,
                       uint8_t* rgba_out, float* color_out, float* length_out);
RT_API int rt_temporal_device(rt_context* ctx, const rt_temporal_params* params, const rt_denoise_params* dn,
                              void* rgba_device, void* stream);
RT_API int rt_temporal_reset(rt_context* ctx);
RT_API float rt_last_temporal_ms(rt_context* ctx);

RT_API int rt_set_moments(rt_context* ctx, int enable);
RT_API int rt_get_moments(const rt_context* ctx);
RT_API int rt_moments_batches(const rt_context* ctx);
RT_API int rt_get_variance(rt_context* ctx, float* var_out, float* lum_out);

typedef struct rt_denoise_var_params {
    int iterations;
    float sigma_lum;
    float sigma_normal;
    float sigma_plane;
    int min_batches;
} rt_denoise_var_params;
RT_API rt_denoise_var_params rt_denoise_var_params_default(void);
RT_API int rt_denoise_var(rt_context* ctx, const rt_denoise_var_params* params, uint8_t* rgba_out,
                          float* color_out, float* var_out);
RT_API int rt_denoise_var_device(rt_context* ctx, const rt_denoise_var_params* params, void* rgba_device,
                                 void* stream);
RT_API float rt_last_denoise_var_ms(rt_context* ctx);

RT_API const char* rt_error_string(int status);
RT_API const char* rt_last_error(const rt_context* ctx);

#ifdef __cplusplus
}
#endif

#endif
```

Baseline: 90080 Msamples/s.

## Skip full path tracing for tiles proven to see only sky

Adds a host-side conservative geometric test that classifies screen tiles whose primary rays, including jitter slack, cannot hit any primitive. It builds a bitmask keyed by the view, uploads it, and lets the sorted render kernel take a cheap path for blocks whose tiles are all sky: it accumulates the background colour while still consuming the RNG stream the same way. The table is cached per camera and scene generation. By default it is built only on the second launch with the same key. This adds host build cost, a branch at kernel entry and a risk of wrong pixels if the conservative bounds are ever off.

```diff
diff --git a/bwidman-raytracer_amd/bwrt/abi.py b/bwidman-raytracer_amd/bwrt/abi.py
--- a/bwidman-raytracer_amd/bwrt/abi.py
+++ b/bwidman-raytracer_amd/bwrt/abi.py
@@ -119,6 +119,8 @@
         "rt_last_kernel_ms": (C.c_float, [vp]),
         "rt_set_kernel_timing": (C.c_int, [vp, C.c_int]),
         "rt_shard_rows": (C.c_int, [C.c_int, C.c_int, C.c_int]),
+        "rt_sky_table": (C.c_int, [vp, P(RenderParams), C.c_int, C.c_int, vp, C.c_size_t, P(C.c_longlong),
+                                   P(C.c_ulonglong)]),
         "rt_deinterleave_rows_device": (C.c_int, [vp, vp, vp, C.c_int, C.c_int, C.c_int,
                                                   C.c_int, vp]),
         "rt_get_state": (C.c_int, [vp, vp, vp]),
diff --git a/bwidman-raytracer_amd/bwrt/renderer.py b/bwidman-raytracer_amd/bwrt/renderer.py
--- a/bwidman-raytracer_amd/bwrt/renderer.py
+++ b/bwidman-raytracer_amd/bwrt/renderer.py
@@ -140,6 +140,17 @@
 
     def stream_handle(self) -> int:
         return self.lib.rt_get_stream(self.ctx) or 0
+
+    def sky_table(self, width, height, row_offset=0, row_stride=1, tile_w=-1, tile_sq=False):
+        p = self.params(width, height, 1, 0, 0, row_offset, row_stride)
+        tiles, builds = C.c_longlong(), C.c_ulonglong()
+        self._check(self.lib.rt_sky_table(self.ctx, C.byref(p), tile_w, int(bool(tile_sq)), None, 0,
+                                          C.byref(tiles), C.byref(builds)))
+        words = np.zeros(tiles.value // 32 + 1, np.uint32)
+        self._check(self.lib.rt_sky_table(self.ctx, C.byref(p), tile_w, int(bool(tile_sq)), words.ctypes.data,
+                                          words.size, C.byref(tiles), C.byref(builds)))
+        bits = np.unpackbits(words.view(np.uint8), bitorder="little")[:tiles.value].astype(bool)
+        return bits, builds.value
 
     def last_kernel_ms(self) -> float:
         return self.lib.rt_last_kernel_ms(self.ctx)
diff --git a/bwidman-raytracer_amd/csrc/rt_context.cpp b/bwidman-raytracer_amd/csrc/rt_context.cpp
--- a/bwidman-raytracer_amd/csrc/rt_context.cpp
+++ b/bwidman-raytracer_amd/csrc/rt_context.cpp
@@ -145,6 +145,10 @@
     if (const char* g = tuning_env("BWRT_REFILL")) c->refill = std::min(std::max(std::atoi(g), 1), 64);
     if (const char* g = tuning_env("BWRT_SPREAD")) c->spread = std::atoi(g) ? 1 : 0;
     if (const char* g = tuning_env("BWRT_ORDER")) c->order_feedback = std::atoi(g) != 0;
+    if (const char* g = tuning_env("BWRT_SKY")) {
+        c->sky_on = std::atoi(g) != 0;
+        c->sky_eager = std::atoi(g) == 2;
+    }
     if (const char* g = tuning_env("BWRT_ORDER_PERIOD")) c->order_period = std::max(std::atoi(g), 1);
     if (const char* g = tuning_env("BWRT_DENOISE_KERNEL"))
         c->dn_kernel = std::strcmp(g, "tiled") == 0 ? 1 : std::strcmp(g, "direct") == 0 ? 0 : -1;
@@ -198,6 +202,10 @@
             p->destroy();
         }
         if (c->host_rgba) (void)hipHostFree(c->host_rgba);
+        if (c->sky_ev) {
+            (void)hipEventSynchronize(c->sky_ev);
+            (void)hipEventDestroy(c->sky_ev);
+        }
         if (c->stream) (void)hipStreamDestroy(c->stream);
     }
     delete c;
@@ -231,12 +239,14 @@
         HIP_TRY(c, hipMemcpyAsync(c->scene_buf.p, cs.data.data(), bytes, hipMemcpyHostToDevice, c->stream));
         HIP_TRY(c, hipStreamSynchronize(c->stream));
     }
+    rt_sky_collect(*s, cs, c->sky_prims);
     std::vector<float>().swap(cs.data);
     c->scene = std::move(cs);
     c->camera = s->camera;
     c->has_scene = true;
     c->frame = 1;
     c->order_stale = true;
+    c->sky_gen++;
     c->new_view();
     c->tp_has_hist = c->tp_has_pending = false;
     return RT_OK;
@@ -247,6 +257,7 @@
     c->camera = *cam;
     c->frame = 1;
     c->order_stale = true;
+    c->sky_gen++;
     c->new_view();
     return RT_OK;
 }
@@ -352,6 +363,7 @@
     if (flags > 0 && (flags & RT_CONTROLS_MOVED)) {
         c->frame = 1;
         c->order_stale = true;
+        c->sky_gen++;
         c->new_view();
     }
     return flags;
diff --git a/bwidman-raytracer_amd/csrc/rt_context.h b/bwidman-raytracer_amd/csrc/rt_context.h
--- a/bwidman-raytracer_amd/csrc/rt_context.h
+++ b/bwidman-raytracer_amd/csrc/rt_context.h
@@ -14,17 +14,20 @@
 #include "../../include/rt_abi.h"
 #include "rt_layout.h"
 #include "rt_scene.h"
+#include "rt_sky.h"
 
 size_t rt_render_rec_floats(const rt_kparams& K);
 bool rt_render_wants_global_records(const rt_kparams& K, int num_cus);
 hipError_t rt_launch_render(const rt_kparams& K, int num_cus, int grid_mult, bool simple, int block_req,
                             hipStream_t stream, int pair_req);
+bool rt_render_takes_sorted(const rt_kparams& K, int num_cus, bool simple, int block_req, int pair_req);
 hipError_t rt_launch_init_rand(unsigned* rng, int width, int rows, int row_offset, int row_stride,
                                hipStream_t stream);
 namespace rt_fast {
 bool rt_render_wants_global_records(const rt_kparams& K, int num_cus);
 hipError_t rt_launch_render(const rt_kparams& K, int num_cus, int grid_mult, bool simple, int block_req,
                             hipStream_t stream, int pair_req);
+bool rt_render_takes_sorted(const rt_kparams& K, int num_cus, bool simple, int block_req, int pair_req);
 }
 extern thread_local long rt_order_groups_last;
 extern thread_local char rt_launched_kernel[96];
@@ -197,6 +200,27 @@
         mom_batches = 0;
     }
 
+    struct SkyKey {
+        unsigned long long gen = 0;
+        int width = 0, height = 0, rows = 0, row_offset = 0, row_stride = 0, tile_w = 0, tile_sq = 0, spp_inner = 0;
+        float jitter = 0.0f;
+        bool operator==(const SkyKey& o) const {
+            return gen == o.gen && width == o.width && height == o.height && rows == o.rows &&
+                   row_offset == o.row_offset && row_stride == o.row_stride && tile_w == o.tile_w &&
+                   tile_sq == o.tile_sq && spp_inner == o.spp_inner && jitter == o.jitter;
+        }
+    };
+    bool sky_on = true, sky_eager = false;
+    unsigned long long sky_gen = 1, sky_builds = 0;
+    SkyKey sky_key;
+    SkyKey sky_seen;
+    bool sky_any = false;
+    bool sky_uploaded = false;
+    rt_sky_prims sky_prims;
+    std::vector<uint32_t> sky_bits;
+    Buf sky_buf;
+    hipEvent_t sky_ev = nullptr;
+
     void new_view() {
         guides_valid = false;
         view++;
@@ -228,6 +252,8 @@
 int shard_rows(int height, int row_offset, int row_stride);
 int shard_check(rt_context* c, int width, int height, int row_offset, int row_stride);
 void fill_view(rt_context* c, int width, int height, int row_offset, int stride, int rows, rt_kparams& K);
+void policy_tiles(const rt_context* c, rt_kparams& K);
+void sky_table(rt_context* c, const rt_kparams& K);
 
 inline void planes_to_rgb(const float* planes, size_t npix, float* out) {
     for (size_t i = 0; i < npix; i++)
diff --git a/bwidman-raytracer_amd/csrc/rt_kernels.hip b/bwidman-raytracer_amd/csrc/rt_kernels.hip
--- a/bwidman-raytracer_amd/csrc/rt_kernels.hip
+++ b/bwidman-raytracer_amd/csrc/rt_kernels.hip
@@ -429,6 +429,48 @@
 
 enum { T_NONE = 0, T_REGEN = 1, T_DIFF = 2, T_SPEC = 3 };
 
+namespace {
+template <int BLOCK, bool ORDER>
+__device__ __forceinline__ void render_sky_group(const rt_kparams& K, long group) {
+    const int tid = threadIdx.x;
+    unsigned t0 = 0u;
+    if (ORDER) t0 = (unsigned)__builtin_amdgcn_s_memrealtime();
+    const long npix = (long)K.rows * K.width;
+    const long nitems = items_of(K, npix);
+    PixelState px;
+    load_item(K, npix, nitems, group * BLOCK + tid, px);
+    const float lx = K.bg[0], ly = K.bg[1], lz = K.bg[2];
+    while (px.passes_left > 0) {
+        if (!ball_try(px.rs)) continue;
+        if (px.frame == 1u) {
+            px.ax = 0.0f;
+            px.ay = 0.0f;
+            px.az = 0.0f;
+        }
+        px.ax = px.ax + lx;
+        px.ay = px.ay + ly;
+        px.az = px.az + lz;
+        px.frame++;
+        px.passes_left--;
+    }
+    if (px.valid && px.frame != K.first_frame) store_pixel(K, npix, px);
+    if (ORDER && tid == 0) K.group_cost[group] = (unsigned)__builtin_amdgcn_s_memrealtime() - t0;
+}
+
+typedef const __attribute__((address_space(4))) rt_kparams* kparams_ptr;
+template <int BLOCK, bool ORDER>
+__device__ __attribute__((noinline)) void render_sky_group_call(kparams_ptr kp_v, int group_v) {
+#if defined(__HIP_DEVICE_COMPILE__)
+    const unsigned long long a = (unsigned long long)kp_v;
+    const unsigned lo = __builtin_amdgcn_readfirstlane((unsigned)a);
+    const unsigned hi = __builtin_amdgcn_readfirstlane((unsigned)(a >> 32));
+    const kparams_ptr kp = (kparams_ptr)(((unsigned long long)hi << 32) | lo);
+    const rt_kparams K = *kp;
+    render_sky_group<BLOCK, ORDER>(K, (long)__builtin_amdgcn_readfirstlane(group_v));
+#endif
+}
+}
+
 RT_MODE_BEGIN
 template <int BLOCK, bool HIT_LDS, bool GREC, bool ORDER = false, bool QUADS = true>
 __global__ void __launch_bounds__(BLOCK) __attribute__((amdgpu_waves_per_eu(GREC ? RT_GREC_WAVES : RT_WAVES_PER_EU)))
@@ -436,6 +478,15 @@
     extern __shared__ float smem[];
     const int tid = threadIdx.x;
     const int lane = tid & 63;
+    if (K.sky) {
+        constexpr unsigned WPB = BLOCK / 64, ALL = (1u << WPB) - 1u;
+        const long sgroup = ORDER && K.group_order ? (long)K.group_order[blockIdx.x] : (long)blockIdx.x;
+        const unsigned first = (unsigned)sgroup * WPB;
+        if (((K.sky[first >> 5] >> (first & 31)) & ALL) == ALL) {
+            render_sky_group_call<BLOCK, ORDER>((kparams_ptr)__builtin_amdgcn_kernarg_segment_ptr(), (int)sgroup);
+            return;
+        }
+    }
     const int n_prim = K.n_sph + K.n_pln + K.n_tri + K.n_quad;
     const float* hit_tab = K.hit;
     float* rec_base = smem;
@@ -1262,10 +1313,10 @@
         else
             launch_kind<KIND, BLOCK, HIT_LDS, GREC, false, false>(K, grid, lds, stream);
     }
-    std::snprintf(rt_launched_kernel, sizeof rt_launched_kernel, "%s<%d%s%s%s%s>%s",
+    std::snprintf(rt_launched_kernel, sizeof rt_launched_kernel, "%s<%d%s%s%s%s>%s%s",
                   KIND == K_PAIR ? "rt_render_pair_kernel" : KIND == K_SORTED ? "rt_render_sorted_kernel" : "rt_render_kernel",
                   KIND == K_PAIR ? 128 : BLOCK, HIT_LDS ? "" : ",hit_global", GREC ? ",grec" : "", BVH ? ",bvh" : "",
-                  RT_MODE_TAG, feedback ? "+order" : "");
+                  RT_MODE_TAG, feedback ? "+order" : "", KIND == K_SORTED && K.sky ? "+sky" : "");
     hipError_t e = hipGetLastError();
     if (e == hipSuccess && feedback && (K0.order_sort || K0.order_n != grid)) {
         e = rt_launch_order_groups(K0.group_cost, K0.group_order, grid, stream);
@@ -1400,6 +1451,27 @@
 #define RT_PAIR_MIN_CHAIN 8
 #endif
 RT_MODE_BEGIN
+namespace {
+bool takes_pair(const rt_kparams& K, bool hit_lds, int num_cus, int block_req, int pair_req) {
+    const long items = (long)K.rows * K.width;
+    return hit_lds && !K.rec && (block_req == 0 || block_req == 128) &&
+           (pair_req > 0 || (pair_req < 0 && block_req == 0 && items <= (long)num_cus * RT_SPREAD_PIX &&
+                             (long)K.samples * (K.max_bounces + 1) >= RT_PAIR_MIN_CHAIN));
+}
+}
+
+bool rt_render_takes_sorted(const rt_kparams& K, int num_cus, bool simple, int block_req, int pair_req) {
+    if (simple || K.spp_inner > 1 || K.bvh_nodes) return false;
+#ifdef RT_NO_HIT_LDS
+    const bool hit_lds = false;
+#else
+    const int n_prim = K.n_sph + K.n_pln + K.n_tri + K.n_quad;
+    const bool hit_lds = (size_t)n_prim * RT_HIT_FLOATS * sizeof(float) <= 16384;
+#endif
+    const bool small_block = (size_t)3 * (K.max_bounces + 1) * 256 * sizeof(float) > 49152;
+    return small_block || !takes_pair(K, hit_lds, num_cus, block_req, pair_req);
+}
+
 hipError_t rt_launch_render(const rt_kparams& K, int num_cus, int grid_mult, bool simple, int block_req,
                             hipStream_t stream, int pair_req) {
     simple = simple || K.spp_inner > 1;
@@ -1421,9 +1493,7 @@
 #endif
     if (small_block) return launch_block<64, K_SORTED>(K, hit_lds, lds, grid_mult, num_cus, stream);
     const long items = (long)K.rows * K.width;
-    const bool pair = hit_lds && !K.rec && (block_req == 0 || block_req == 128) &&
-                      (pair_req > 0 || (pair_req < 0 && block_req == 0 && items <= (long)num_cus * RT_SPREAD_PIX &&
-                                        (long)K.samples * (K.max_bounces + 1) >= RT_PAIR_MIN_CHAIN));
+    const bool pair = takes_pair(K, hit_lds, num_cus, block_req, pair_req);
     if (pair)
         return launch_render<K_PAIR, 128, true>(K, rt_pair_lds_bytes(K), grid_mult, num_cus, stream);
     if (block_req == 64 || block_req == 128 || block_req == 256) {
diff --git a/bwidman-raytracer_amd/csrc/rt_layout.h b/bwidman-raytracer_amd/csrc/rt_layout.h
--- a/bwidman-raytracer_amd/csrc/rt_layout.h
+++ b/bwidman-raytracer_amd/csrc/rt_layout.h
@@ -64,6 +64,7 @@
     int leaf_batch;
     int refill;
     int spp_inner;
+    const unsigned* sky;
 };
 
 #ifndef RT_LEAF_BATCH
diff --git a/bwidman-raytracer_amd/csrc/rt_path.h b/bwidman-raytracer_amd/csrc/rt_path.h
--- a/bwidman-raytracer_amd/csrc/rt_path.h
+++ b/bwidman-raytracer_amd/csrc/rt_path.h
@@ -316,6 +316,13 @@
     r = normalize3(r);
     if (dot(normal, r) < 0.0f) r = sub(r, scale(2.0f * dot(r, normal), normal));
     return r;
+}
+
+RT_HD bool ball_try(Xorwow& s) {
+    const float x = rand_pm1(s);
+    const float y = rand_pm1(s);
+    const float z = rand_pm1(s);
+    return !(x * x + y * y + z * z > 1.00000012f);
 }
 
 RT_HD f3 specular_scatter(Xorwow& rs, f3 d, f3 n, float rough, float rough2, float ior2m1, float& kspec) {
diff --git a/bwidman-raytracer_amd/csrc/rt_render.cpp b/bwidman-raytracer_amd/csrc/rt_render.cpp
--- a/bwidman-raytracer_amd/csrc/rt_render.cpp
+++ b/bwidman-raytracer_amd/csrc/rt_render.cpp
@@ -145,10 +145,42 @@
     return RT_OK;
 }
 
-static int launch(rt_context* c, rt_kparams& K, hipStream_t s, unsigned first, int samples) {
+static rt_context::SkyKey sky_key_of(const rt_context* c, const rt_kparams& K) {
+    rt_context::SkyKey k;
+    k.gen = c->sky_gen;
+    k.width = K.width;
+    k.height = K.height;
+    k.rows = K.rows;
+    k.row_offset = K.row_offset;
+    k.row_stride = K.row_stride;
+    k.tile_w = K.tile_w;
+    k.tile_sq = K.tile_sq;
+    k.spp_inner = K.spp_inner;
+    k.jitter = K.jitter;
+    return k;
+}
+
+void sky_table(rt_context* c, const rt_kparams& K) {
+    const rt_context::SkyKey k = sky_key_of(c, K);
+    if (k == c->sky_key) return;
+    if (c->sky_uploaded && c->sky_ev) (void)hipEventSynchronize(c->sky_ev);
+    rt_sky_build(K, c->sky_prims, c->sky_bits);
+    c->sky_key = k;
+    c->sky_builds++;
+    c->sky_uploaded = false;
+    c->sky_any = false;
+    for (const uint32_t w : c->sky_bits) c->sky_any = c->sky_any || w != 0u;
+}
+
+void policy_tiles(const rt_context* c, rt_kparams& K) {
     const bool small = (long)K.rows * K.width <= (long)c->num_cus * 1024;
     K.tile_w = c->tile_w >= 0 ? c->tile_w : K.bvh_nodes ? (small ? 4 : 8) : (small ? 32 : 8);
     K.tile_sq = c->tile_sq;
+}
+
+static int launch(rt_context* c, rt_kparams& K, hipStream_t s, unsigned first, int samples) {
+    policy_tiles(c, K);
+    const bool small = (long)K.rows * K.width <= (long)c->num_cus * 1024;
     K.leaf_batch = c->leaf_batch > 0 ? c->leaf_batch : small ? RT_LEAF_BATCH_SMALL : RT_LEAF_BATCH;
     K.refill = c->refill > 0 ? c->refill : small ? RT_REFILL_SMALL : RT_REFILL;
     K.rec = nullptr;
@@ -192,6 +224,27 @@
     if (const int rc = moments_prepare(c, first, samples, MA, track)) return rc;
     int orc = order_after_all(c, s);
     if (orc) return orc;
+    bool sky = c->sky_on && (fast ? rt_fast::rt_render_takes_sorted(K, c->num_cus, c->simple, c->block, c->spread)
+                                  : rt_render_takes_sorted(K, c->num_cus, c->simple, c->block, c->spread));
+    if (sky && !c->sky_eager) {
+        const rt_context::SkyKey k = sky_key_of(c, K);
+        if (!(k == c->sky_key) && !(k == c->sky_seen)) {
+            c->sky_seen = k;
+            sky = false;
+        }
+    }
+    if (sky) {
+        sky_table(c, K);
+        if (c->sky_any && !c->sky_uploaded) {
+            const size_t bytes = c->sky_bits.size() * sizeof(uint32_t);
+            if (const int rc = ensure_buf(c, c->sky_buf, bytes)) return rc;
+            if (!c->sky_ev) HIP_TRY(c, hipEventCreateWithFlags(&c->sky_ev, hipEventDisableTiming));
+            HIP_TRY(c, hipMemcpyAsync(c->sky_buf.p, c->sky_bits.data(), bytes, hipMemcpyHostToDevice, s));
+            HIP_TRY(c, hipEventRecord(c->sky_ev, s));
+            c->sky_uploaded = true;
+        }
+        if (c->sky_any) K.sky = c->sky_buf.as<unsigned>();
+    }
     rt_order_groups_last = 0;
     rt_launched_kernel[0] = 0;
     HIP_TRY(c, c->render.begin(s, c->ktiming));
@@ -364,6 +417,31 @@
     return RT_OK;
 }
 
+int rt_sky_table(rt_context* c, const rt_render_params* p, int tile_w, int tile_sq, uint32_t* bits, size_t words,
+                 long long* tiles_out, unsigned long long* builds_out) {
+    const HostFpEnv fp;
+    if (!c || !p) return fail(c, RT_ERR_INVALID_ARGUMENT, "null argument");
+    if (!c->has_scene) return fail(c, RT_ERR_NO_SCENE, "rt_set_scene() not called");
+    const int stride = p->row_stride == 0 ? 1 : p->row_stride;
+    if (const int rc = shard_check(c, p->width, p->height, p->row_offset, stride)) return rc;
+    if (tile_w > 64 || (tile_w > 0 && (tile_w & (tile_w - 1))))
+        return fail(c, RT_ERR_INVALID_ARGUMENT, "rt_sky_table: tile_w %d is not a power of two up to 64", tile_w);
+    if (words && !bits) return fail(c, RT_ERR_INVALID_ARGUMENT, "rt_sky_table: null bits");
+    rt_kparams K;
+    fill_view(c, p->width, p->height, p->row_offset, stride, shard_rows(p->height, p->row_offset, stride), K);
+    if (tile_w < 0) {
+        policy_tiles(c, K);
+    } else {
+        K.tile_w = tile_w;
+        K.tile_sq = tile_sq != 0;
+    }
+    sky_table(c, K);
+    for (size_t i = 0; i < words; i++) bits[i] = i < c->sky_bits.size() ? c->sky_bits[i] : 0u;
+    if (tiles_out) *tiles_out = rt_sky_tiles(K);
+    if (builds_out) *builds_out = c->sky_builds;
+    return RT_OK;
+}
+
 int rt_render_cpu(rt_context* c, const rt_render_params* p, int threads, uint8_t* rgba_out, float* accum_out) {
     if (!c) return RT_ERR_INVALID_ARGUMENT;
     if (!c->cpu) return fail(c, RT_ERR_INVALID_ARGUMENT, "rt_render_cpu: not a CPU context (rt_create_cpu)");
diff --git a/bwidman-raytracer_amd/csrc/rt_sky.cpp b/bwidman-raytracer_amd/csrc/rt_sky.cpp
--- /dev/null
+++ b/bwidman-raytracer_amd/csrc/rt_sky.cpp
@@ -0,0 +1,253 @@
+#include <algorithm>
+#include <cmath>
+
+#include "rt_scene.h"
+#include "rt_sky.h"
+
+struct float4;
+struct float2;
+#include "rt_layout.h"
+
+namespace {
+
+const double kAbs = 9.5367431640625e-07;
+const double kRel = 6.103515625e-05;
+const double kSign = 3.814697265625e-06;
+const double kSlackAngle = 1e-5;
+const double kScaleMax = 1e9;
+
+struct D3 {
+    double x, y, z;
+};
+D3 sub(D3 a, D3 b) { return {a.x - b.x, a.y - b.y, a.z - b.z}; }
+double dot(D3 a, D3 b) { return a.x * b.x + a.y * b.y + a.z * b.z; }
+D3 cross(D3 a, D3 b) { return {a.y * b.z - a.z * b.y, a.z * b.x - a.x * b.z, a.x * b.y - a.y * b.x}; }
+double len(D3 a) { return std::sqrt(dot(a, a)); }
+D3 mul(double k, D3 a) { return {k * a.x, k * a.y, k * a.z}; }
+D3 d3(const rt_vec3& v) { return {v.x, v.y, v.z}; }
+
+bool quad_sphere(const rt_vec3* verts, double scale, double* out) {
+    const int nv = 4;
+    D3 v[nv], p[nv];
+    for (int k = 0; k < nv; k++) v[k] = d3(verts[k]);
+    const D3 n = cross(sub(v[1], v[0]), sub(v[2], v[1]));
+    const double nl = len(n);
+    if (!(nl > 0.0) || !std::isfinite(nl)) return false;
+    const D3 nh = mul(1.0 / nl, n);
+    double extent = 0.0;
+    for (int k = 1; k < nv; k++) extent = std::max(extent, len(sub(v[k], v[0])));
+    if (!(extent > 0.0) || !std::isfinite(extent)) return false;
+    const double tol = std::ldexp(extent, -10);
+    D3 c = {0.0, 0.0, 0.0};
+    for (int k = 0; k < nv; k++) {
+        const double off = dot(nh, sub(v[k], v[0]));
+        if (!(std::fabs(off) <= tol)) return false;
+        p[k] = sub(v[k], mul(off, nh));
+        c = {c.x + 0.25 * p[k].x, c.y + 0.25 * p[k].y, c.z + 0.25 * p[k].z};
+    }
+    double r = 0.0, min_sin = 1.0;
+    for (int k = 0; k < nv; k++) {
+        const D3 e = sub(p[(k + 1) % nv], p[k]), in = cross(nh, e);
+        const double el = len(e);
+        if (!(el > 0.0)) return false;
+        for (int j = 0; j < nv; j++)
+            if (j != k && j != (k + 1) % nv && !(dot(in, sub(p[j], p[k])) > tol * el)) return false;
+        const D3 b = sub(p[(k + nv - 1) % nv], p[k]);
+        const double bl = len(b);
+        if (!(bl > 0.0)) return false;
+        const double cosang = dot(e, b) / (el * bl);
+        min_sin = std::min(min_sin, std::sqrt(std::max(0.0, 1.0 - cosang * cosang)));
+        r = std::max(r, len(sub(p[k], c)));
+    }
+    if (!(min_sin >= 1.0 / 1024.0) || !std::isfinite(r) || !std::isfinite(scale)) return false;
+    const double rc = r * (1.0 + std::ldexp(1.0, -20)) + std::ldexp(1.0, -14) * scale / (0.25 * min_sin);
+    const double rc2 = rc * rc * (1.0 + std::ldexp(1.0, -20));
+    if (!(rc2 < 1e30)) return false;
+    out[0] = c.x, out[1] = c.y, out[2] = c.z, out[3] = rc2;
+    return true;
+}
+
+struct TileGrid {
+    int tw = 0, th = 0;
+    long tiles_x = 0, tiles_y = 0;
+    long px = 0, py = 0;
+};
+TileGrid tile_grid(const rt_kparams& K) {
+    TileGrid g;
+    if (K.tile_w <= 0 || K.tile_w > 64 || (K.tile_w & (K.tile_w - 1)) || K.width <= 0 || K.rows <= 0) return g;
+    g.tw = K.tile_w;
+    g.th = 64 / K.tile_w;
+    g.tiles_x = g.px = ((long)K.width + g.tw - 1) / g.tw;
+    g.tiles_y = g.py = ((long)K.rows + g.th - 1) / g.th;
+    if (K.tile_sq) {
+        g.px += g.px & 1;
+        g.py += g.py & 1;
+    }
+    return g;
+}
+
+}
+
+void rt_sky_collect(const rt_scene& s, const rt_compiled_scene& r, rt_sky_prims& out) {
+    rt_sky_prims P;
+    P.scale = r.cull_omax;
+    P.cull_dmax = r.cull_dmax;
+    bool ok = r.off_bvh == 0 && r.cull_omax > 0.0f && std::isfinite(r.cull_omax);
+    const float* h = r.data.data();
+    auto put = [&](std::vector<double>& to, const float* q) {
+        for (int a = 0; a < 4; a++) {
+            if (!std::isfinite(q[a])) ok = false;
+            to.push_back(q[a]);
+        }
+    };
+    for (int i = 0; ok && i < r.n_sph; i++) {
+        put(P.sph, h + (size_t)i * RT_SPH_FLOATS);
+        if (!(P.sph.back() >= 0.0)) ok = false;
+    }
+    for (int i = 0; ok && i < r.n_pln; i++) put(P.pln, h + r.off_pln + (size_t)i * RT_PLN_FLOATS);
+    for (int i = 0; ok && i < r.n_tri; i++) {
+        const float* q = h + r.off_tri + (size_t)i * RT_TRI_FLOATS;
+        for (int a = 0; a < 4; a++) P.poly.push_back(q[RT_TRI_CULL + a]);
+        put(P.poly, q);
+    }
+    for (int i = 0; ok && i < r.n_quad; i++) {
+        double q[4] = {0.0, 0.0, 0.0, INFINITY};
+        (void)quad_sphere(s.quads[i].vertices, P.scale, q);
+        P.poly.insert(P.poly.end(), q, q + 4);
+        put(P.poly, h + r.off_quad + (size_t)i * RT_QUAD_FLOATS);
+    }
+    P.ok = ok;
+    if (!ok) {
+        P.sph.clear();
+        P.pln.clear();
+        P.poly.clear();
+    }
+    out = std::move(P);
+}
+
+long rt_sky_tiles(const rt_kparams& K) {
+    const TileGrid g = tile_grid(K);
+    return g.px * g.py;
+}
+
+void rt_sky_build(const rt_kparams& K, const rt_sky_prims& P, std::vector<uint32_t>& bits) {
+    const TileGrid g = tile_grid(K);
+    const long tiles = g.px * g.py;
+    bits.assign(rt_sky_words(tiles), 0u);
+    if (tiles == 0 || !P.ok || K.spp_inner > 1) return;
+    const double S = P.scale;
+    if (!(S > 0.0 && S <= kScaleMax) || !(P.cull_dmax >= 2.0)) return;
+    const double jit = K.jitter;
+    if (!(jit >= 0.0 && jit < 0.25)) return;
+    const D3 cam = {K.cam_pos[0], K.cam_pos[1], K.cam_pos[2]};
+    double R[9];
+    for (int a = 0; a < 9; a++) R[a] = K.rot[a];
+    const double sz = K.screen_z;
+    bool finite = std::isfinite(cam.x) && std::isfinite(cam.y) && std::isfinite(cam.z) && std::isfinite(sz);
+    for (int a = 0; a < 9; a++) finite = finite && std::isfinite(R[a]);
+    if (!finite || !(std::fabs(cam.x) <= S && std::fabs(cam.y) <= S && std::fabs(cam.z) <= S)) return;
+
+    struct Sph {
+        D3 w;
+        double wl, lim2;
+    };
+    struct Pln {
+        D3 m;
+    };
+    struct Poly {
+        Sph s;
+        Pln p;
+        bool s_ok, p_ok;
+    };
+    std::vector<Sph> sph(P.sph.size() / 4);
+    std::vector<Pln> pln(P.pln.size() / 4);
+    std::vector<Poly> poly(P.poly.size() / 8);
+    const double abs_slack = kAbs * S;
+    auto sphere_of = [&](const double* q, Sph& s) {
+        s.w = sub({q[0], q[1], q[2]}, cam);
+        const double l2 = dot(s.w, s.w);
+        s.wl = std::sqrt(l2);
+        s.lim2 = q[3] + kRel * l2;
+        return std::isfinite(s.lim2) && s.wl > abs_slack && (s.wl - abs_slack) * (s.wl - abs_slack) > s.lim2;
+    };
+    auto plane_of = [&](const double* q, Pln& p) {
+        const D3 n = {q[0], q[1], q[2]};
+        const double nl = len(n), s0 = dot(n, cam) + q[3];
+        if (!(nl > 0.0) || !(nl < 1e18) || !(std::fabs(q[3]) < 1e18)) return false;
+        if (!(std::fabs(s0) > kSign * (nl * len(cam) * 1.7320508075688772 + std::fabs(q[3])))) return false;
+        p.m = mul((s0 > 0.0 ? 1.0 : -1.0) / nl, n);
+        return true;
+    };
+    for (size_t i = 0; i < sph.size(); i++)
+        if (!sphere_of(&P.sph[4 * i], sph[i])) return;
+    for (size_t i = 0; i < pln.size(); i++)
+        if (!plane_of(&P.pln[4 * i], pln[i])) return;
+    for (size_t i = 0; i < poly.size(); i++) {
+        poly[i].s_ok = sphere_of(&P.poly[8 * i], poly[i].s);
+        poly[i].p_ok = plane_of(&P.poly[8 * i + 4], poly[i].p);
+        if (!poly[i].s_ok && !poly[i].p_ok) return;
+    }
+
+    const long gx = g.tiles_x + 1, gy = g.tiles_y + 1;
+    std::vector<D3> dir((size_t)(gx * gy));
+    for (long iy = 0; iy < gy; iy++) {
+        const long j = std::min(iy * g.th, (long)K.rows - 1);
+        const double py = (double)((long)K.row_offset + j * K.row_stride - K.height / 2);
+        for (long ix = 0; ix < gx; ix++) {
+            const double px = (double)(std::min(ix * g.tw, (long)K.width - 1) - K.width / 2);
+            const D3 pr = {R[0] * px + R[1] * py + R[2] * sz, R[3] * px + R[4] * py + R[5] * sz,
+                           R[6] * px + R[7] * py + R[8] * sz};
+            const double l = len(pr);
+            dir[(size_t)(iy * gx + ix)] = mul(1.0 / l, pr);
+        }
+    }
+    const double delta = std::asin(jit * 1.00001) + kSlackAngle;
+    const double cd = std::cos(delta), sd = std::sin(delta), cos1 = std::cos(1.0);
+
+    auto rect_is_sky = [&](long tx0, long ty0, long tx1, long ty1) -> int {
+        const D3 c00 = dir[(size_t)(ty0 * gx + tx0)], c10 = dir[(size_t)(ty0 * gx + tx1)];
+        const D3 c01 = dir[(size_t)(ty1 * gx + tx0)], c11 = dir[(size_t)(ty1 * gx + tx1)];
+        const D3 sum = {c00.x + c10.x + c01.x + c11.x, c00.y + c10.y + c01.y + c11.y, c00.z + c10.z + c01.z + c11.z};
+        const double sl = len(sum);
+        if (!(sl > 1.0)) return 0;
+        const D3 A = mul(1.0 / sl, sum);
+        const double ct = std::min(std::min(dot(A, c00), dot(A, c10)), std::min(dot(A, c01), dot(A, c11)));
+        if (!(ct > 0.0)) return 0;
+        const double st = std::sqrt(std::max(0.0, 1.0 - ct * ct));
+        const double cth = ct * cd - st * sd, sth = st * cd + ct * sd;
+        if (!(cth > cos1)) return 0;
+        auto plane_clears = [&](const Pln& p, double& far_side) {
+            const double cp = dot(p.m, A), sp = std::sqrt(std::max(0.0, 1.0 - cp * cp));
+            far_side = cp * cth + sp * sth;
+            return cp * cth - sp * sth > kSign;
+        };
+        auto sphere_clears = [&](const Sph& s) {
+            const double cphi = dot(A, s.w), sphi = len(cross(A, s.w));
+            const double lo = sphi * cth - cphi * sth, hi = sphi * cth + cphi * sth;
+            const double dist = std::min(lo, hi) - abs_slack;
+            return dist > 0.0 && dist * dist > s.lim2;
+        };
+        double far_side;
+        for (const Pln& p : pln)
+            if (!plane_clears(p, far_side)) return far_side < 0.0 ? -1 : 0;
+        for (const Sph& s : sph)
+            if (!sphere_clears(s)) return 0;
+        for (const Poly& q : poly)
+            if (!(q.p_ok && plane_clears(q.p, far_side)) && !(q.s_ok && sphere_clears(q.s))) return 0;
+        return 1;
+    };
+    auto set_bit = [&](long tx, long ty) {
+        const long t = K.tile_sq ? ((ty >> 1) * (g.px >> 1) + (tx >> 1)) * 4 + (ty & 1) * 2 + (tx & 1) : ty * g.px + tx;
+        bits[(size_t)(t >> 5)] |= 1u << (t & 31);
+    };
+    const long kB = 8;
+    for (long by = 0; by < g.tiles_y; by += kB)
+        for (long bx = 0; bx < g.tiles_x; bx += kB) {
+            const long ex = std::min(bx + kB, g.tiles_x), ey = std::min(by + kB, g.tiles_y);
+            const int whole = rect_is_sky(bx, by, ex, ey);
+            if (whole < 0) continue;
+            for (long ty = by; ty < ey; ty++)
+                for (long tx = bx; tx < ex; tx++)
+                    if (whole > 0 || rect_is_sky(tx, ty, tx + 1, ty + 1) > 0) set_bit(tx, ty);
+        }
+}
diff --git a/bwidman-raytracer_amd/csrc/rt_sky.h b/bwidman-raytracer_amd/csrc/rt_sky.h
--- /dev/null
+++ b/bwidman-raytracer_amd/csrc/rt_sky.h
@@ -0,0 +1,25 @@
+#pragma once
+
+#include <cstdint>
+#include <vector>
+
+#include "../../include/rt_abi.h"
+
+struct rt_kparams;
+struct rt_compiled_scene;
+
+struct rt_sky_prims {
+    bool ok = false;
+    double scale = 0.0;
+    double cull_dmax = -1.0;
+    std::vector<double> sph;
+    std::vector<double> pln;
+    std::vector<double> poly;
+};
+
+void rt_sky_collect(const rt_scene& s, const rt_compiled_scene& r, rt_sky_prims& out);
+
+long rt_sky_tiles(const rt_kparams& K);
+inline size_t rt_sky_words(long tiles) { return (size_t)(tiles / 32 + 2); }
+
+void rt_sky_build(const rt_kparams& K, const rt_sky_prims& P, std::vector<uint32_t>& bits);
diff --git a/include/rt_abi.h b/include/rt_abi.h
--- a/include/rt_abi.h
+++ b/include/rt_abi.h
@@ -176,6 +176,10 @@
 
 RT_API int rt_set_kernel_timing(rt_context* ctx, int enable);
 
+RT_API int rt_sky_table(rt_context* ctx, const rt_render_params* p, int tile_w, int tile_sq,
+                        uint32_t* bits, size_t words, long long* tiles_out,
+                        unsigned long long* builds_out);
+
 RT_API int rt_shard_rows(int height, int row_offset, int row_stride);
 
 RT_API int rt_deinterleave_rows_device(rt_context* ctx, const void* gathered,
```

Result: faster. 92130 Msamples/s (median of 6 runs) (+2.3%).
